# BlueFisher/Advanced-Soft-Actor-Critic

Hardware: AMD Instinct MI355X
Metric: SAC train steps/sec (PER sample + grad step), batch 256 (higher is better)
Workload: dtype f32; 1 GPU; cfg2: TEST vector obs(6) c_action(2) stock MLP, PER capacity 524288, n_step=4 V-trace; per_gpu_batch=256, global_batch=256, rows_resident=262144, replay_capacity=524288, n_step=4, burn_in_step=0, parallelism=single, ranks=1, hipgraph=True

## Files before the change

### advanced-soft-actor-critic_amd/algorithm/fused_mlp.py

```python
import contextlib
import os
import weakref

import torch
from torch import nn

from asac_amd import native

from .nn_models.layers.linear_layers import LinearLayers, ResBlock

__all__ = ['StockMLP', 'describe_q', 'describe_policy', 'describe_dense', 'fused_dense', 'gauss_head']

MAX_WIDTH, MAX_HEAD = 64, 16
MAX_INPUT = 128
FUSED_DENSE = True

_direct_depth = 0
_direct_only = []


@contextlib.contextmanager
def direct_param_grads(only=None):
    global _direct_depth
    if _direct_depth == 0:
# ... 340 lines not shown
        self._anchor = torch.zeros(1, device=device, requires_grad=True)
        self.accumulate = True
        self._workspace = None
        self._start, self._deferred_rows = start, None
        self.device = device

    @staticmethod
    def _rows(x, width):
        assert x.shape[-1] == width
        if x.dim() == 2 and x.stride(-1) == 1:
            return x
        return x.reshape(-1, width) if x.is_contiguous() else x.contiguous().view(-1, width)

    @staticmethod
    def _rows_in_place(x, width):
        assert x.shape[-1] == width
        if x.dim() == 3 and not x.is_contiguous() and x.stride(2) == 1 and x.stride(0) != x.stride(1) * x.shape[1]:
            return native.WindowRows(x)
        return StockMLP._rows(x, width)

    def _launch_forward(self, x0, x1, out=None):
        if isinstance(x0, native.WindowRows):
            job, out = self.job(x0, x1, out)
            native.mlp_forward_multi([job])
            return out
        N = x0.shape[-2]
        if out is None:
            out = torch.empty((self.E, N, self.out_cols), dtype=torch.float32, device=self.device)
        assert out.shape == (self.E, N, self.out_cols) and out.is_contiguous()
        native.mlp_forward(self.desc, self.params, self.member_stride, self.E, x0, x1, N, out)
        return out

    def _workspace_for(self, N):
        need = native.mlp_backward_workspace(self.member_stride, self.E, N)
        if self._workspace is None or self._workspace.numel() < need:
            self._workspace = torch.zeros(need, dtype=torch.float32, device=self.device)
        return self._workspace

    def _reduce_mode(self, defer):
        if defer:
            return native.MLP_REDUCE_DEFER
        return native.MLP_REDUCE_ACCUMULATE if self.accumulate else native.MLP_REDUCE_OVERWRITE

    def backward_qloss(self, x0, x1, target_q, y, weights, clip_eps, loss_out, defer=False, state_grads=False):
        N = x0.shape[-2]
        g0 = torch.empty((self.E, N, self.in0), dtype=torch.float32, device=self.device) if state_grads else None
        native.mlp_backward_qloss(self.desc, self.params, self.member_stride, self.E, x0, x1, N, target_q, y, weights,
                                  clip_eps, loss_out, self.grad_params, self._workspace_for(N), self._reduce_mode(defer),
                                  grad_x0=g0)
        self._deferred_rows = N if defer else None
        return g0

    def backward_qloss_return_ok(self, N: int, ret) -> bool:
        return native.mlp_backward_qloss_return_ok(self.desc, self.params, self.member_stride, self.E, N, ret)

    def backward_qloss_return(self, x0, x1, target_q, ret, weights, clip_eps, loss_out, defer=False, state_grads=False):
        N = x0.shape[-2]
        g0 = torch.empty((self.E, N, self.in0), dtype=torch.float32, device=self.device) if state_grads else None
        native.mlp_backward_qloss_return(self.desc, self.params, self.member_stride, self.E, x0, x1, N, target_q, ret,
                                         weights, clip_eps, loss_out, self.grad_params, self._workspace_for(N),
                                         self._reduce_mode(defer), grad_x0=g0)
        self._deferred_rows = N if defer else None
        return g0

    def backward_policy_q(self, x0, x1, q_table, subset, E_sample):
        N = x0.shape[-2]
        g1 = torch.empty((self.E, N, self.in1), dtype=torch.float32, device=self.device)
        native.mlp_backward_policy_q(self.desc, self.params, self.member_stride, self.E, x0, x1, N, q_table, subset,
                                     E_sample, g1)
        return g1

    def backward_policy_sample(self, x0, eps, grad_a, log_alpha, defer=False):
        N = x0.shape[-2]
        native.mlp_backward_policy_sample(self.desc, self.params, self.member_stride, x0, N, eps, grad_a, log_alpha,
                                          self.grad_params, self._workspace_for(N), self._reduce_mode(defer))
        self._deferred_rows = N if defer else None

    def policy_step_fused_ok(self, critics: 'StockMLP', N: int) -> bool:
        return (self.E == 1 and critics.E >= 2 and self.grad_params is not None and
                native.policy_step_fused_ok(critics.desc, critics.params, critics.member_stride, self.desc, self.params,
                                            self.member_stride, N))

    def policy_step_fused(self, critics: 'StockMLP', x0, action, eps, log_alpha, q_out=None, defer=False, subset=None,
                          sample_out=None):
        N = x0.shape[-2]
        assert subset is not None or critics.E == 2
        a_out, logp_out, ls_out = sample_out if action is None else (None, None, None)
        native.policy_step_fused(critics.desc, critics.params, critics.member_stride, self.desc, self.params,
                                 self.member_stride, x0, N, action, eps, log_alpha, q_out, self.grad_params,
                                 self._workspace_for(N), self._reduce_mode(defer), subset=subset, a_out=a_out,
                                 logp_out=logp_out, ls_out=ls_out)
        self._deferred_rows = N if defer else None

    def adam_partials(self, opt, loss_out=None):
        N = self._deferred_rows
        assert N is not None, 'no deferred backward pending'
        tiles = native.mlp_backward_tiles(N, self.E)
        s0 = self._start
        s1 = s0 + self.E * self.member_stride
        native.adam_step_partials(self.params, self.grad_params, opt.exp_avg[s0:s1], opt.exp_avg_sq[s0:s1], opt.lr,
                                  opt.betas[0], opt.betas[1], opt.eps, opt.steps_done, self._workspace, tiles,
                                  self.E, self.member_stride, native.mlp_param_extent(self.desc),
                                  self.accumulate, loss_out, N if loss_out is not None else 0)
        self._deferred_rows = None

    def job(self, x0, x1, out=None):
        N = x0.shape[0] if isinstance(x0, native.WindowRows) else x0.shape[-2]
        if self.wide and isinstance(x0, native.WindowRows):
            x0 = x0.t.reshape(N, x0.t.shape[-1])
        if out is None:
            out = torch.empty((self.E, N, self.out_cols), dtype=torch.float32, device=self.device)
        assert out.shape == (self.E, N, self.out_cols) and out.is_contiguous()
        return native.mlp_job(self.desc, self.params, self.member_stride, self.E, x0, x1, N, out), out

    def _launch_backward(self, x0, x1, grad_out, need0, need1, param_grads, reduce_members=True, defer=False,
                         grad_target=None, later=None):
        N = x0.shape[-2]
        E = self.E
        g0 = torch.empty((E, N, self.in0), dtype=torch.float32, device=self.device) if need0 else None
        g1 = torch.empty((E, N, self.in1), dtype=torch.float32, device=self.device) if need1 else None
        gp = ws = None
        mode = self._reduce_mode(defer and param_grads)
        if param_grads:
            gp = self.grad_params
            self._deferred_rows = N if defer else None
            if grad_target is not None:
                assert not defer
                gp, mode = grad_target, native.MLP_REDUCE_OVERWRITE
            if later is None or defer:
                ws = self._workspace_for(N)
            if later is not None and not defer:
                ws = torch.empty(native.mlp_backward_workspace(self.member_stride, E, N), dtype=torch.float32,
                                 device=self.device)
                tiles, used = native.mlp_backward_tiles(N, E), native.mlp_param_extent(self.desc)
                for e in range(E):
                    later.add(ws[e * self.member_stride:], tiles, 16 if tiles >= 64 else 1, E * self.member_stride, used,
                              gp[e * self.member_stride:], accumulate=mode == native.MLP_REDUCE_ACCUMULATE)
                mode = native.MLP_REDUCE_DEFER
        native.mlp_backward(self.desc, self.params, self.member_stride, E, x0, x1, N, grad_out, g0, g1, gp, ws,
                            reduce_mode=mode)
        if reduce_members:
            if g0 is not None and x0.dim() == 2:
                g0 = g0.sum(0) if E > 1 else g0[0]
            if g1 is not None and x1.dim() == 2:
                g1 = g1.sum(0) if E > 1 else g1[0]
        return g0, g1

    def call_select(self, base, t, x1=None, param_grads=True):
        if torch.is_grad_enabled() and (param_grads or base.requires_grad or (x1 is not None and x1.requires_grad)):
            pg = param_grads and self.grad_params is not None
            return _MlpSelectFn.apply(self._anchor, base, t, x1, self, pg, *(self.param_tensors if pg else ()))
        return self._launch_forward(base[:, t], x1)

    def __call__(self, x0, x1=None, param_grads=True):
        if isinstance(x0, native.WindowRows):
            assert not (torch.is_grad_enabled() and (param_grads or x0.t.requires_grad))
            return self._launch_forward(x0, x1)
        if torch.is_grad_enabled() and (param_grads or x0.requires_grad or (x1 is not None and x1.requires_grad)):
            pg = param_grads and self.grad_params is not None
            return _MlpFn.apply(self._anchor, x0, x1, self, pg, *(self.param_tensors if pg else ()))
        return self._launch_forward(x0, x1)


class _GaussHeadFn(torch.autograd.Function):
    @staticmethod
    def forward(ctx, raw, A):
        raw = raw.contiguous()
        loc = torch.empty((*raw.shape[:-1], A), dtype=raw.dtype, device=raw.device)
        scale = torch.empty_like(loc)
        native.gauss_head_fwd(raw, A, loc, scale)
        ctx.save_for_backward(raw)
        ctx.A = A
        return loc, scale

# ... 12 lines not shown
```

### advanced-soft-actor-critic_amd/algorithm/oc/option_base.py

```python
import inspect
import logging
import os

import torch
from torch.nn import functional

from asac_amd import native

from ..fused import FlatParamGroup
from ..fused_mlp import DeferredPartialSums, direct_param_grads
from ..imitation_base import SpanAdam
from ..sac_base import SAC_Base
from ..utils.enums import SEQ_ENCODER
from ..utils.operators import get_last_false_indexes

_UNSUPPORTED = "OptionBase does not support {what}: {why}"


def _reject_unsupported(args, kwargs) -> None:
    bound = inspect.signature(SAC_Base.__init__).bind_partial(None, *args, **kwargs).arguments
    if bound.get('siamese') is not None:
        raise ValueError(_UNSUPPORTED.format(
            what='siamese', why='the siamese representation loss inside compute_rep_q_grads is not built for an option'))
    if bound.get('use_prediction'):
# ... 212 lines not shown

    def _target_terminations(self, nx_target_states, nx_target_obses_list):
        with torch.no_grad():
            beta = self.model_target_termination(nx_target_states[:, :-1], [o[:, :-1] for o in nx_target_obses_list])
        return beta.squeeze(-1)

    def compute_rep_q_grads(self, next_n_vs_over_options, n_indexes, n_last_masks, n_padding_masks, nx_obses_list,
                            nx_target_obses_list, nx_states, nx_target_states, n_actions, n_pre_actions, n_rewards,
                            n_dones, n_mu_probs, n_pre_seq_hidden_states, priority_is=None):
        self._check_batch(n_rewards.shape[0])
        E, dsum = self.ensemble_q_num, self.d_action_summed_size
        n_target_terminations = self._target_terminations(nx_target_states, nx_target_obses_list)
        obs_list = [o[:, 0] for o in nx_obses_list]
        state, action = nx_states[:, 0], n_actions[:, 0]
        d_action, c_action = action[..., :dsum], action[..., dsum:]
        B = state.shape[0]
        q_list = None
        if self.d_action_sizes:
            q_list = [q(state, c_action, obs_list) for q in self.model_q_list]
            c_q = torch.stack([q[1] for q in q_list]).squeeze(-1) if self.c_action_size else None
        else:
            c_q = self._c_q_values(False, state, c_action, obs_list)
        d_y, c_y = self._get_y(next_n_vs_over_options, n_target_terminations, n_last_masks, n_padding_masks,
                               nx_target_obses_list, nx_target_states.detach(), n_actions, n_rewards, n_dones,
                               n_mu_probs if self.use_n_step_is else None,
                               eps_buf=self._eps_y, subset_prefix='y')

        start, stop = self._params.span('rep', f'q_{E - 1}')
        self._params.grad[start:stop].zero_()
        losses = roots = None
        if self.d_action_sizes:
            qs = torch.stack([torch.sum(d_action * q[0], dim=-1, keepdim=True) / self.d_action_branch_size
                              for q in q_list])
            losses = functional.mse_loss(qs, d_y.expand_as(qs), reduction='none')
        if self.c_action_size:
            yv = c_y.reshape(1, -1)
            if self.clip_epsilon > 0:
                with torch.no_grad():
                    t_q = self._c_q_values(True, state.detach(), c_action, obs_list)
                if losses is None and B == self._grad_q.shape[1]:
                    w = priority_is.reshape(-1).contiguous() if priority_is is not None else None
                    native.q_loss_fwd_bwd(c_q.detach().contiguous(), t_q.contiguous(), c_y.reshape(-1), w,
                                          self.clip_epsilon, self._loss_q_e, self._grad_q)
                    roots = ([c_q], [self._grad_q])
                else:
                    clipped = t_q + torch.clamp(c_q - t_q, -self.clip_epsilon, self.clip_epsilon)
                    c_loss = torch.maximum((clipped - yv) ** 2, (c_q - yv) ** 2).unsqueeze(-1)
            else:
                c_loss = functional.mse_loss(c_q, yv.expand_as(c_q), reduction='none').unsqueeze(-1)
            if roots is None:
                losses = c_loss if losses is None else losses + c_loss
        if roots is None:
            if priority_is is not None:
                losses = losses * priority_is.unsqueeze(0)
            loss_q_list = losses.mean(dim=(1, 2))
            self._loss_q_e.copy_(loss_q_list.detach())
            roots = ([loss_q_list.sum()], [None])
        with direct_param_grads(), DeferredPartialSums() as sums_later:
            torch.autograd.backward(*roots, retain_graph=True)
        sums_later.flush()
        self._write_option_summary({'loss/q': self._stats['loss_q']})
        return d_y, c_y

    def train_rep_q(self):
        start, stop = self._params.span('rep', f'q_{self.ensemble_q_num - 1}')
        if self.fix_policy or self.optimizer_rep is None:
            start = self._params.span('q_0')[0]
        self.optimizer_q_list[0].step(start, stop)
        self._steps_rep_q.add_(1)

    def train_policy_alpha(self, n_padding_masks, n_obses_list, nx_states, n_actions, n_mu_probs) -> None:
        if self.fix_policy:
            return
        self._check_batch(n_actions.shape[0])
        obs_list = [o[:, 0] for o in n_obses_list]
        n_states = nx_states[:, :-1]
        state, action = n_states[:, 0], n_actions[:, 0]
        mu_d_policy_probs = n_mu_probs[:, 0, :self.d_action_summed_size]
        for name in ('policy', 'alpha', 'curiosity', 'rnd'):
            if name in self._params.segments:
                s, e = self._params.span(name)
                self._params.grad[s:e].zero_()
        self._counter_advanced = False
        self._pi_sampled = False
        self._train_policy(obs_list=obs_list, state=state, action=action, mu_d_policy_probs=mu_d_policy_probs)
        if self._auto_alpha():
            self._train_alpha(obs_list, state)
        if self.curiosity is not None:
            self._train_curiosity(n_padding_masks=n_padding_masks, nx_states=nx_states, n_actions=n_actions)
        if self.use_rnd:
            self._train_rnd(n_padding_masks=n_padding_masks, n_states=n_states, n_actions=n_actions)
        if not self._counter_advanced:
            self._steps_pi.add_(1)
        if self._summary_due():
            self._refresh_policy_stats()
            tags = {}
            if self.d_action_sizes and not self.discrete_dqn_like:
                tags['loss/d_entropy'] = self._stats['d_entropy']
                if self.use_auto_alpha:
                    tags['loss/d_alpha'] = torch.exp(self.log_d_alpha.detach())
            if self.c_action_size:
                tags['loss/c_entropy'] = self._stats['c_entropy']
                if self.use_auto_alpha:
                    tags['loss/c_alpha'] = torch.exp(self.log_c_alpha.detach())
            if self.curiosity is not None:
                tags['loss/curiosity'] = self._stats['loss_curiosity']
            self._write_option_summary(tags)

    def compute_termination_grads(self, terminal_entropy, obs_list, state, y, v_over_options, done, priority_is):
        termination = self.model_termination(state.detach(), obs_list)
        B = termination.shape[0]
        dbeta = torch.empty(B, dtype=torch.float32, device=self.device)
        with torch.no_grad():
            native.termination_loss_grad(termination.detach(), y.detach(), v_over_options, done.contiguous(),
                                         priority_is, terminal_entropy, self._loss_termination, dbeta,
                                         workspace=self._termination_ws)
        self.optimizer_termination.zero_grad()
        with direct_param_grads(), DeferredPartialSums() as sums_later:
            torch.autograd.backward([termination], [dbeta.view_as(termination)])
        sums_later.flush()
        if self._summary_due():
            self._stats['termination'].copy_(torch.mean(termination.detach()))
            self._write_option_summary({'loss/termination': self._stats['loss_termination'],
                                        'metric/termination': self._stats['termination']})

    def train_termination(self):
        self.optimizer_termination.step()

    @torch.no_grad()
    def _get_td_error(self, next_n_vs_over_options, n_last_masks, n_padding_masks, nx_obses_list, nx_target_obses_list,
                      state, nx_target_states, n_actions, n_rewards, n_dones, n_mu_probs):
        self._check_batch(n_rewards.shape[0])
        dsum = self.d_action_summed_size
        n_target_terminations = self._target_terminations(nx_target_states, nx_target_obses_list)
        obs_list = [o[:, 0] for o in nx_obses_list]
        action = n_actions[:, 0]
        d_action, c_action = action[..., :dsum], action[..., dsum:]
        B = state.shape[0]
        q_list = None
        if self.d_action_sizes:
            q_list = [q(state, c_action, obs_list) for q in self.model_q_list]
            c_q = torch.stack([q[1] for q in q_list]).squeeze(-1).contiguous() if self.c_action_size else None
        else:
            c_q = self._c_q_values(False, state, c_action, obs_list).contiguous()
        fused_td = bool(self.c_action_size) and not self.d_action_sizes
        td = torch.empty(B, dtype=torch.float32, device=self.device)
        d_y, c_y = self._get_y(next_n_vs_over_options, n_target_terminations, n_last_masks, n_padding_masks,
                               nx_obses_list, nx_target_states, n_actions, n_rewards, n_dones,
                               n_mu_probs if self.use_n_step_is else None,
                               eps_buf=self._eps_td, subset_prefix='td',
                               q_online=c_q if fused_td else None, td_out=td)
        if fused_td:
            return td.unsqueeze(-1)
        err = torch.zeros((self.ensemble_q_num, B, 1), device=self.device)
        if self.d_action_sizes:
            d_q = torch.stack([torch.sum(d_action * q[0], dim=-1, keepdim=True) / self.d_action_branch_size
                               for q in q_list])
            err = err + torch.abs(d_q - d_y)
        if self.c_action_size:
            err = err + torch.abs(c_q.unsqueeze(-1) - c_y)
        return err.mean(dim=0)

    def _check_batch(self, rows: int) -> None:
        if rows != self.batch_size:
            raise ValueError(f'OptionBase was built with batch_size={self.batch_size} and takes batches of that size, '
                             f'got {rows} rows')

# ... 12 lines not shown
```

### advanced-soft-actor-critic_amd/algorithm/sac_base.py

```python
import contextlib
import logging
import random
from collections import defaultdict, namedtuple
from pathlib import Path

import numpy as np
import torch
from torch import distributions, nn
from torch.nn import functional

from asac_amd import native

from . import fused_gru, fused_linear
from .fused import DeviceNoise, FlatAdam, FlatParamGroup, squash_sample, squash_sample_ls, time_slice
from .fused_mlp import DeferredPartialSums, StockMLP, describe_policy, describe_q, direct_param_grads
from .nn_models import *
from .nn_models.layers.seq_layers import step_mask_cache
from .nn_models.representation import ModelSimpleRep
from .batch_buffer import BatchBuffer
from .captured_step import CapturedStep
from .replay_buffer import PrioritizedReplayBuffer
from .sac_aux import AuxHeadsMixin
from .utils import *
from .utils.enums import CURIOSITY, SEQ_ENCODER, SIAMESE
# ... 347 lines not shown
        tnamed += [(f'q_{i}', list(q.parameters())) for i, q in enumerate(self.model_target_q_list)]
        self._target_params = FlatParamGroup(tnamed, dev, with_grad=False)
        self._polyak_len = self._params.span('rep', f'q_{self.ensemble_q_num - 1}')[1]
        assert self._polyak_len == self._target_params.numel
        if self._dist is not None:
            self._dist.broadcast_(self._params.flat)

        self._opt_steps = torch.zeros(1, dtype=torch.int64, device=dev)
        self._exp_avg = torch.zeros_like(self._params.flat)
        self._exp_avg_sq = torch.zeros_like(self._params.flat)

        def adam(names):
            if all(len(self._params.params[n]) == 0 for n in names):
                return None
            return FlatAdam(self._params, names, learning_rate, self._opt_steps, self._exp_avg, self._exp_avg_sq)

        self.optimizer_rep = adam(['rep'])
        self.optimizer_q_list = [adam([f'q_{i}']) for i in range(self.ensemble_q_num)]
        self.optimizer_policy = adam(['policy'])
        if self.use_auto_alpha:
            self.optimizer_alpha = adam(['alpha'])
        if cur is not None:
            self.optimizer_curiosity = adam(['curiosity'])
        if self.siamese is not None:
            self.optimizer_siamese = adam(['siamese'])
        if self.use_prediction:
            self.optimizer_prediction = adam(['prediction'])
        if self.use_rnd:
            self.optimizer_rnd = adam(['rnd'])

        self._fq = self._ftq = self._fpi = None
        if self._use_fused_mlp and self.c_action_size and not self.d_action_sizes:
            dq = [describe_q(q) for q in self.model_q_list + self.model_target_q_list]
            seg = self._params.segments
            stride = seg['q_0'][1] - seg['q_0'][0]
            consecutive = all(seg[f'q_{i}'][0] == seg['q_0'][0] + i * stride for i in range(self.ensemble_q_num))
            if all(d is not None for d in dq) and consecutive:
                tseg = self._target_params.segments
                self._fq = StockMLP(dq[0], self._params.flat, self._params.grad, seg['q_0'][0], stride,
                                    self.ensemble_q_num, dev, [p for q in self.model_q_list for p in q.parameters()])
                self._ftq = StockMLP(dq[0], self._target_params.flat, None, tseg['q_0'][0], stride,
                                     self.ensemble_q_num, dev)
            dp = describe_policy(self.model_policy)
            if dp is not None:
                self._fpi = StockMLP(dp, self._params.flat, self._params.grad, seg['policy'][0],
                                     seg['policy'][1] - seg['policy'][0], 1, dev, list(self.model_policy.parameters()))
        self._wide_critics = self._fq is not None and self._fq.wide
        if self._wide_critics:
            self._la_gather_sidecar = False
        self._logger.info(f'fused stock MLP path: Q={self._fq is not None} policy={self._fpi is not None}')
        stock_only = {f'q_{i}' for i in range(self.ensemble_q_num)} | {'policy', 'alpha'}
        self._grads_overwrite = (self._fq is not None and self._fpi is not None and not self.offline_enabled
                                 and all(stop == start or name in stock_only
                                         for name, (start, stop) in self._params.segments.items()))
        if self._grads_overwrite:
            self._fq.accumulate = self._fpi.accumulate = False

        n, A, E, Es = self.n_step, self.c_action_size, self.ensemble_q_num, self.ensemble_q_sample
        f32 = dict(dtype=torch.float32, device=dev)
        A1 = max(A, 1)
        sizes = [B * (n + 1) * A1, B * A1, B * A1, B * (n + 1) * A1]
        self._eps_all = torch.zeros(sum(sizes), **f32)
        o = np.cumsum([0] + sizes)
        self._eps_y = self._eps_all[o[0]:o[1]].view(B, n + 1, A1)
        self._eps_pi = self._eps_all[o[1]:o[2]].view(B, A1)
        self._eps_alpha = self._eps_all[o[2]:o[3]].view(B, A1)
        self._eps_td = self._eps_all[o[3]:o[4]].view(B, n + 1, A1)
        names = ('y_dn', 'y_dnext', 'y_cn', 'y_cnext', 'pi_d', 'pi_c', 'td_dn', 'td_dnext', 'td_cn', 'td_cnext')
        self._subsets_all = torch.arange(Es, dtype=torch.int32, device=dev).repeat(len(names), 1).contiguous()
        self._subsets = {k: self._subsets_all[i] for i, k in enumerate(names)}
        self._y_buf = torch.zeros(B, **f32)
        self._y_td_buf = torch.zeros(B, **f32)
        self._td_error = torch.zeros(B, **f32)
        self._stats = {k: torch.zeros((), **f32) for k in ('d_entropy', 'c_entropy', 'loss_curiosity', 'loss_policy')}
        self._loss_q_e = torch.zeros(E, **f32)
        self._stats['loss_q'] = self._loss_q_e[0]
        self._grad_q = torch.zeros(E, B, **f32)
        self._mse_big_ws = torch.zeros(native.mse_mean_grad_workspace(), **f32) if self.use_prediction else None
        self._grad_logp = torch.zeros(B, **f32)
        self._ls_y = None
        self._cq_buf, self._tq_buf, self._cq_td_buf = (torch.zeros(E, B, 1, **f32) for _ in range(3))
        self._pi_q, self._pi_stats_src = torch.zeros(E, B, 1, **f32), None
        self._pi_a, self._pi_logp, self._pi_sampled = torch.zeros(B, A1, **f32), torch.zeros(B, **f32), False
        self._rep_twin = None
        if self._twin_rep and type(self.model_rep) is not ModelSimpleRep:
            from .fused_gru import TwinPass
            self._rep_twin = TwinPass(self.model_rep, self.model_target_rep)

    def _build_ckpt(self) -> None:
        ck = self.ckpt_dict = {'global_step': self.global_step}
        if self.optimizer_rep is not None:
            ck['model_rep'], ck['model_target_rep'], ck['optimizer_rep'] = \
                self.model_rep, self.model_target_rep, self.optimizer_rep
        for i in range(self.ensemble_q_num):
            ck[f'model_q_{i}'] = self.model_q_list[i]
            ck[f'model_target_q_{i}'] = self.model_target_q_list[i]
            ck[f'optimizer_q_{i}'] = self.optimizer_q_list[i]
        ck['model_policy'], ck['optimizer_policy'] = self.model_policy, self.optimizer_policy
        ck['log_d_alpha'], ck['log_c_alpha'] = self.log_d_alpha, self.log_c_alpha
        if self.use_auto_alpha:
            ck['optimizer_alpha'] = self.optimizer_alpha
        if self.curiosity == CURIOSITY.FORWARD:
            ck['model_forward_dynamic'] = self.model_forward_dynamic
        elif self.curiosity == CURIOSITY.INVERSE:
            ck['model_inverse_dynamic'] = self.model_inverse_dynamic
        if self.curiosity is not None:
            ck['optimizer_curiosity'] = self.optimizer_curiosity
        self._aux_ckpt(ck)
        total = sum(p.numel() for m in ck.values() if isinstance(m, nn.Module) for p in m.parameters())
        self._logger.info(f'Parameters: {total}')

    def _init_or_restore(self, last_ckpt: int | None) -> None:
        self.ckpt_dir = None
        if not self.model_abs_dir:
            self._update_target_variables()
            return
        self.ckpt_dir = ckpt_dir = Path(self.model_abs_dir).joinpath('model')
        ckpts = sorted(int(p.stem) for p in ckpt_dir.glob('*.pth')) if ckpt_dir.exists() else []
        ckpt_dir.mkdir(parents=True, exist_ok=True)
        if not ckpts:
            self._logger.info('Initializing from scratch')
            self._update_target_variables()
            return
        if last_ckpt is None or last_ckpt not in ckpts:
            if last_ckpt is not None:
                self._logger.warning(f'{last_ckpt} NOT IN {ckpts}, using {ckpts[-1]}')
            last_ckpt = ckpts[-1]
        path = ckpt_dir.joinpath(f'{last_ckpt}.pth')
        restored = torch.load(path, map_location=self.device, weights_only=True)
        failed = False
        for name, obj in self.ckpt_dict.items():
            if name not in restored:
                self._logger.warning(f'{name} not in {last_ckpt}.pth')
                continue
            if isinstance(obj, torch.Tensor):
                if name == 'global_step':
                    self.global_step.copy_(restored[name].to('cpu'))
                else:
                    with torch.no_grad():
                        obj.copy_(restored[name])
                continue
            try:
                if failed and name.startswith('optimizer'):
                    continue
                obj.load_state_dict(restored[name])
            except RuntimeError as e:
                failed = True
                self._logger.error(e)
            if isinstance(obj, nn.Module):
                obj.train(self.train_mode)
        self._params.rebind()
        self._target_params.rebind()
        self._logger.info(f'Restored from {path}')
        if self.train_mode and self.use_replay_buffer:
            self.replay_buffer.load(ckpt_dir, last_ckpt)
            self._logger.info('Replay buffer restored')

    def _init_replay_buffer(self, replay_config: dict | None = None) -> None:
        if not self.train_mode:
            return
        if not self.use_replay_buffer:
            self.batch_buffer = BatchBuffer(burn_in_step=self.burn_in_step,
                                            n_step=self.n_step,
                                            padding_action=self._padding_action,
                                            batch_size=self.batch_size,
                                            device=self.device,
# ... 265 lines not shown
        return bnx_indexes, bnx_padding_masks, gen_n_pre_actions(bn_actions, keep_last_action=True)

    def get_l_states(self, l_indexes, l_padding_masks, l_obses_list, l_pre_actions, l_pre_seq_hidden_states,
                     is_target=False):
        rep = self.model_target_rep if is_target else self.model_rep
        if self.seq_encoder == SEQ_ENCODER.ATTN:
            st, attn, _ = rep(l_indexes.shape[1], l_indexes, l_obses_list, l_pre_actions,
                              l_pre_seq_hidden_states[:, :1], is_prev_hidden_state=True,
                              padding_mask=l_padding_masks)
            return _real(st), _real(attn)
        out = rep(l_obses_list, l_pre_actions, l_pre_seq_hidden_states, padding_mask=l_padding_masks)
        return tuple(_real(o) for o in out) if isinstance(out, tuple) else _real(out)

    def _c_q_values(self, target: bool, state, c_action, obs_list, param_grads=True, select=None):
        fused = self._ftq if target else self._fq
        if fused is not None:
            lead = state.shape[:-1]
            a_rows = StockMLP._rows(c_action, self.c_action_size)
            if select is not None and not target and select[0].dim() == 3 and select[0].is_contiguous():
                out = fused.call_select(select[0], select[1], a_rows, param_grads=param_grads)
            else:
                rows = StockMLP._rows if torch.is_grad_enabled() else StockMLP._rows_in_place
                out = fused(rows(state, self.state_size), a_rows, param_grads=param_grads and not target)
            return out.view(self.ensemble_q_num, *lead)
        models = self.model_target_q_list if target else self.model_q_list
        return torch.stack([q(state, c_action, obs_list)[1] for q in models]).squeeze(-1)

    def _policy(self, state, obs_list):
        if self._fpi is not None:
            lead, A = state.shape[:-1], self.c_action_size
            rows = StockMLP._rows if torch.is_grad_enabled() else StockMLP._rows_in_place
            self._ls = self._fpi(rows(state, self.state_size))[0].view(*lead, 2 * A)
            return None, None, self._ls[..., :A], self._ls[..., A:], True
        self._ls = None
        d_policy, c_policy = self.model_policy(state, obs_list)
        if c_policy is None:
            return d_policy, None, None, None, False
        plain = type(c_policy) is distributions.Normal
        return d_policy, c_policy, c_policy.loc, c_policy.scale, plain

    @staticmethod
    def _rsample(c_policy, eps):
        if hasattr(c_policy, 'padding_mask'):
            keep = ~c_policy.padding_mask
            return c_policy.loc * keep + eps * (c_policy.scale * keep)
        return c_policy.loc + eps * c_policy.scale

    @torch.no_grad()
    def get_l_probs(self, l_obses_list, l_states, l_actions):
        d_policy, c_policy, loc, scale, plain = self._policy(l_states, l_obses_list)
        A_all = self.d_action_summed_size + self.c_action_size
        probs = torch.empty((*l_states.shape[:2], A_all), dtype=torch.float32, device=self.device)
        if self.d_action_sizes:
            probs[..., :self.d_action_summed_size] = d_policy.probs
        if self.c_action_size:
            if plain and l_actions.stride(-1) == 1:
                native.squash_prob(loc, scale, l_actions, self.d_action_summed_size, probs,
                                   self.d_action_summed_size)
            else:
                c_act = l_actions[..., self.d_action_summed_size:]
                probs[..., self.d_action_summed_size:] = squash_correction_prob(
                    c_policy, torch.atanh(torch.clamp(c_act, -0.999, 0.999)))
        return probs

    def _return_sample_epilogue(self, jobs, k, ls, nx_actions, eps_buf, policy_sample):
        A = self.c_action_size
        if not (native.SAMPLE_EPILOGUE and A and 2 * A <= 16 and ls.dim() == 3 and nx_actions.stride(-1) == 1):
            return None
        f32 = dict(dtype=torch.float32, device=self.device)
        a_tanh, logp = torch.empty((*ls.shape[:2], A), **f32), torch.empty(ls.shape[:2], **f32)
        c_pi = torch.empty((*ls.shape[:2], A), **f32) if self.use_n_step_is else None
        epis = [native.sample_epilogue() for _ in jobs]
        epis[k] = native.sample_epilogue(jobs[k], eps_buf, a_tanh, logp, ls.shape[1],
                                         action=nx_actions if self.use_n_step_is else None,
                                         action_offset=self.d_action_summed_size, prob_out=c_pi,
                                         eps2=self._eps_pi if policy_sample else None, t2=0,
                                         a2_out=self._pi_a if policy_sample else None,
                                         logp2_out=self._pi_logp if policy_sample else None)
        if not native.mlp_forward_multi_sampled_ok(jobs, epis):
            return None
        self.noise.normal_(eps_buf)
        if policy_sample:
            self.noise.normal_(self._eps_pi)
            self._pi_sampled = True
        native.mlp_forward_multi_sampled(jobs, epis)
        return (a_tanh, logp), c_pi

    def _vtrace_args(self, n_rewards, n_dones, n_last, n_pad, y_out):
        a = native.VtraceArgs()
        a.reward, a.reward_stride = n_rewards.data_ptr(), n_rewards.stride(0)
        a.done, a.last_mask, a.padding_mask = n_dones.data_ptr(), n_last.data_ptr(), n_pad.data_ptr()
        assert n_dones.stride(0) == n_last.stride(0) == n_pad.stride(0)
        a.mask_stride = n_dones.stride(0)
        a.gamma_ratio, a.lambda_ratio = self._gamma_ratio.data_ptr(), self._lambda_ratio.data_ptr()
        a.gamma, a.v_rho, a.v_c = self.gamma, self._v_rho_f, self._v_c_f
        a.use_n_step_is, a.B, a.n = int(self.use_n_step_is), n_rewards.shape[0], self.n_step
        a.y_out = y_out.data_ptr()
        return a

    def _window_sample(self, loc, scale, plain, c_policy, eps_buf, nx_actions, t0_ls=None):
        dsum, A = self.d_action_summed_size, self.c_action_size
        self.noise.normal_(eps_buf)
        if not plain:
            sampled = self._rsample(c_policy, eps_buf)
            c_pi = None
            if self.use_n_step_is:
                c_pi = squash_correction_prob(
                    c_policy, torch.atanh(torch.clamp(nx_actions[..., dsum:], -0.999, 0.999))).contiguous()
            return torch.tanh(sampled), sum_log_prob(squash_correction_log_prob(c_policy, sampled)), c_pi
        f32 = dict(dtype=torch.float32, device=self.device)
        a_tanh, logp = torch.empty(loc.shape, **f32), torch.empty(loc.shape[:-1], **f32)
        c_pi = torch.empty(loc.shape, **f32) if self.use_n_step_is else None
        stored = dict(action=nx_actions, action_offset=dsum, prob_out=c_pi) if self.use_n_step_is else {}
        if t0_ls is not None:
            self.noise.normal_(self._eps_pi)
            native.squash_multi([
                native.squash_job(loc, scale, eps_buf, a_tanh, logp, **stored),
                native.squash_job(t0_ls[:, 0, :A], t0_ls[:, 0, A:], self._eps_pi, self._pi_a, self._pi_logp)])
            self._pi_sampled = True
        else:
            native.squash_sample_fwd(loc, scale, eps_buf, a_tanh, logp, **stored)
        return a_tanh, logp, c_pi

    def _stored_action_ratios(self, d_policy, n_mu_probs, nx_actions):
        dsum = self.d_action_summed_size
        mu = n_mu_probs[..., :dsum] * nx_actions[:, :-1, :dsum]
        mu = torch.where(mu == 0., torch.ones_like(mu), mu).prod(-1).contiguous()
        pi = torch.exp(d_policy.log_prob(nx_actions[..., :dsum]).sum(-1))[:, :-1].contiguous()
        return pi, mu

    def _c_return(self, q_tab, logp, c_pi, n_mu_probs, sub_n, sub_next, n_rewards, n_dones, n_last, n_pad, y_out,
                  q_online=None, td_out=None):
        E, Es = self.ensemble_q_num, self.ensemble_q_sample
        args = self._vtrace_args(n_rewards, n_dones, n_last, n_pad, y_out)
        args.q = q_tab.data_ptr()
        args.q_stride_e, args.q_stride_b, args.q_stride_t = q_tab.stride(0), q_tab.stride(1), q_tab.stride(2)
        args.subset_n, args.subset_next, args.E_sample = (sub_n.data_ptr(), sub_next.data_ptr(), Es) if Es != E else (None, None, Es)
        logp = logp.contiguous()
        args.logp, args.log_alpha = logp.data_ptr(), self.log_c_alpha.data_ptr()
        if self.use_n_step_is:
            args.pi_prob, args.pi_stride_b, args.pi_stride_t = c_pi.data_ptr(), c_pi.stride(0), c_pi.stride(1)
            args.mu_prob, args.mu_stride_b, args.mu_stride_t = \
                n_mu_probs.data_ptr(), n_mu_probs.stride(0), n_mu_probs.stride(1)
            args.mu_offset, args.A = self.d_action_summed_size, self.c_action_size
        if q_online is not None and not self.d_action_sizes:
            q_online = q_online.contiguous()
            args.q_online, args.E_online, args.td_error_out = q_online.data_ptr(), q_online.shape[0], td_out.data_ptr()
        return _Return(args, (q_tab, logp, c_pi, n_mu_probs, sub_n, sub_next, q_online))

    @staticmethod
    def _launch_return(ret, *, sidecars=None, pending_alpha=None, td_update=None) -> bool:
        if td_update is not None and ret.args.td_error_out:
            rb, ids = td_update
            rb.td_update(ret.args, ids, sidecars=sidecars, alpha_step=pending_alpha)
            return True
        native.vtrace_return_min(ret.args, sidecars=sidecars, pending_alpha=pending_alpha)
        return False

    @torch.no_grad()
    def _get_y(self, n_last_masks, n_padding_masks, nx_obses_list, nx_states, nx_actions, n_rewards,
               n_dones, n_mu_probs, *, eps_buf, subset_prefix, y_out, q_online=None, td_out=None, ls=None,
               sample=None, stored_pi=None, policy_sample=False, q_table=None, launch=True):
        n_actions = nx_actions[:, :-1]
        if ls is None and sample is None and self._fpi is not None and self.c_action_size and nx_states.dim() == 3:
            job_pi, ls_out = self._fpi.job(StockMLP._rows_in_place(nx_states, self.state_size), None)
            ls_try = ls_out[0].view(*nx_states.shape[:2], 2 * self.c_action_size)
            pre = self._return_sample_epilogue([job_pi], 0, ls_try, nx_actions, eps_buf, policy_sample)
            if pre is not None:
                ls, (sample, stored_pi) = ls_try, pre
        if ls is not None:
            d_policy = c_policy = None
            loc, scale, plain = ls[..., :self.c_action_size], ls[..., self.c_action_size:], True
        else:
            d_policy, c_policy, loc, scale, plain = self._policy(nx_states, nx_obses_list)
            ls = self._ls
        self._ls_y = ls

        if self.curiosity is not None:
            n_states, next_n_states = nx_states[:, :-1], nx_states[:, 1:]
            if self.curiosity == CURIOSITY.FORWARD:
                approx, actual = self.model_forward_dynamic(n_states, n_actions), next_n_states
            else:
                approx, actual = self.model_inverse_dynamic(n_states, next_n_states), n_actions
            if (self._fused_curiosity and approx.is_cuda and approx.dim() == 3 and approx.dtype == torch.float32
                    and actual.stride(-1) == 1 and n_rewards.dim() == 2 and n_rewards.dtype == torch.float32
                    and (n_rewards.stride(1) == 1 or n_rewards.shape[1] == 1) and not torch.is_grad_enabled()):
                native.curiosity_bonus(approx.contiguous(), actual, n_rewards, self.curiosity_strength)
            else:
                d = approx - actual
                bonus = torch.sum(d.mul_(d), dim=-1).mul_(0.5)
                n_rewards.add_(bonus, alpha=self.curiosity_strength)

        logp = c_pi = None
        if self.c_action_size and sample is not None:
            (a_tanh, logp), c_pi = sample, stored_pi
        elif self.c_action_size:
            a_tanh, logp, c_pi = self._window_sample(
                loc, scale, plain, c_policy, eps_buf, nx_actions,
                t0_ls=ls if plain and policy_sample and ls is not None and ls.dim() == 3 else None)
        else:
            a_tanh = torch.zeros(0, device=self.device)

# ... 13 lines not shown
            self.noise.subset_(sub_eval, E)
            d_y = self.get_dqn_like_d_y(n_last_masks, n_padding_masks, n_rewards, n_dones,
                                        eval_next.index_select(0, sub_eval.long()), target_next)
        elif self.d_action_sizes:
            sub_next, sub_n = self._subsets[subset_prefix + '_dnext'], self._subsets[subset_prefix + '_dn']
            self.noise.subset_(sub_next, E)
            self.noise.subset_(sub_n, E)
            stacked = torch.stack([q[0] for q in nx_qs])
            mean_next = stacked[:, :, 1:].index_select(0, sub_next.long()).mean(0)
            mean_n = stacked[:, :, :-1].index_select(0, sub_n.long()).mean(0)
            probs = d_policy.probs
            n_p, next_p = probs[:, :-1], probs[:, 1:]
            d_alpha = torch.exp(self.log_d_alpha)
            v_n = torch.sum(n_p * (mean_n - d_alpha * torch.log(n_p.clamp(min=1e-8))), -1) / self.d_action_branch_size
            v_next = torch.sum(next_p * (mean_next - d_alpha * torch.log(next_p.clamp(min=1e-8))), -1) \
                / self.d_action_branch_size
            pi, mu = self._stored_action_ratios(d_policy, n_mu_probs, nx_actions) if self.use_n_step_is else (None, None)
            d_y = torch.empty(n_rewards.shape[0], dtype=torch.float32, device=self.device)
            args = self._vtrace_args(n_rewards, n_dones, n_last_masks, n_padding_masks, d_y)
            native.vtrace_return_direct(args, v_n.contiguous(), v_next.contiguous(), pi, mu)
            d_y = d_y.unsqueeze(-1)

        if self.c_action_size:
            sub_n, sub_next = self._subsets[subset_prefix + '_cn'], self._subsets[subset_prefix + '_cnext']
            self.noise.subset_(sub_n, E)
            self.noise.subset_(sub_next, E)
            if q_table is not None:
                q_tab = q_table
            elif nx_qs is not None:
                q_tab = torch.stack([q[1] for q in nx_qs]).squeeze(-1)
            else:
                q_tab = self._c_q_values(True, nx_states, a_tanh, nx_obses_list)
            ret = self._c_return(q_tab, logp, c_pi, n_mu_probs, sub_n, sub_next, n_rewards, n_dones, n_last_masks,
                                 n_padding_masks, y_out, q_online, td_out)
            if launch:
                self._launch_return(ret)
            c_y = y_out.unsqueeze(-1)
        return (d_y, c_y) if launch else (d_y, c_y, ret)

    def _stock_q_targets(self, job_tq, job_pi, ls, window, policy_sample):
        nx_states, nx_actions = window[3], window[4]
        ls = ls[0].view(*nx_states.shape[:2], 2 * self.c_action_size)
        pre = self._return_sample_epilogue([job_tq, job_pi], 1, ls, nx_actions, self._eps_y, policy_sample)
        if pre is None:
            native.mlp_forward_multi([job_tq, job_pi])
        sample, stored_pi = pre or (None, None)
        _, c_y, ret = self._get_y(*window, eps_buf=self._eps_y, subset_prefix='y', y_out=self._y_buf, ls=ls,
                                  sample=sample, stored_pi=stored_pi, policy_sample=policy_sample and pre is None,
                                  launch=False)
        return c_y, ret

    def _stock_q_backward(self, x0, a0, ret, c_y, priority_is, fold, fused_return, state_grads=False):
        w = priority_is.reshape(-1).contiguous() if priority_is is not None else None
        t_q = self._tq_buf.view(self.ensemble_q_num, -1)
        if fused_return and self._fq.backward_qloss_return_ok(x0.shape[-2], ret.args):
            g0 = self._fq.backward_qloss_return(x0, a0, t_q, ret.args, w, self.clip_epsilon, self._loss_q_e,
                                                defer=fold, state_grads=state_grads)
        else:
            self._launch_return(ret)
            g0 = self._fq.backward_qloss(x0, a0, t_q, c_y.reshape(-1), w, self.clip_epsilon, self._loss_q_e,
                                         defer=fold, state_grads=state_grads)
        if fold:
            self._fq.adam_partials(self.optimizer_q_list[0], loss_out=self._loss_q_e)
        return g0

    @torch.no_grad()
    def _train_rep_q_stock(self, n_last_masks, n_padding_masks, nx_obses_list, nx_states, nx_actions, n_rewards,
                           n_dones, n_mu_probs, priority_is, policy_sample):
        E, B = self.ensemble_q_num, nx_states.shape[0]
        x0 = StockMLP._rows(nx_states[:, 0], self.state_size)
        a0 = StockMLP._rows(nx_actions[:, 0], self.c_action_size)
        xs = StockMLP._rows(nx_states, self.state_size)
        job_tq, _ = self._ftq.job(x0, a0, out=self._tq_buf)
        job_pi, ls = self._fpi.job(xs, None)
        T, A = nx_states.shape[1], self.c_action_size
        window = (n_last_masks, n_padding_masks, nx_obses_list, nx_states, nx_actions, n_rewards, n_dones,
                  n_mu_probs if self.use_n_step_is else None)
        fused = None
        if self._fused_forward_chain and self.curiosity is None:
            f32 = dict(dtype=torch.float32, device=self.device)
            a_y, logp_y = torch.empty((B, T, A), **f32), torch.empty((B, T), **f32)
            c_pi = torch.empty((B, T, A), **f32) if self.use_n_step_is else None
            job_q, q_tab = self._ftq.job(xs, a_y.view(-1, A))
            fused = native.pi_q_job(job_pi, job_q, self._eps_y, a_y, logp_y, T,
                                    action=nx_actions if self.use_n_step_is else None,
                                    action_offset=self.d_action_summed_size, prob_out=c_pi,
                                    eps2=self._eps_pi if policy_sample else None, t2=0,
                                    a2_out=self._pi_a, logp2_out=self._pi_logp)
            if not native.policy_sample_q_forward_ok(fused):
                fused = None
        if fused is not None:
            self.noise.normal_(self._eps_y)
            if policy_sample:
                self.noise.normal_(self._eps_pi)
                self._pi_sampled = True
            native.policy_sample_q_forward(fused, [job_tq], sidecars=self._take_la_gather())
            _, c_y, ret = self._get_y(*window, eps_buf=self._eps_y, subset_prefix='y', y_out=self._y_buf,
                                      ls=ls[0].view(B, T, 2 * A), sample=(a_y, logp_y), stored_pi=c_pi,
                                      q_table=q_tab.view(E, B, T), launch=False)
        else:
            c_y, ret = self._stock_q_targets(job_tq, job_pi, ls, window, policy_sample)
        opt = self.optimizer_q_list[0]
        fold = self._dist is None and opt.start == self._fq._start and self._params.span('rep')[0] == self._params.span('rep')[1]
        self._stock_q_backward(x0, a0, ret, c_y, priority_is, fold, fused_return=fused is not None and self._fused_q_return)
        if not fold:
            self._finish_rep_q(None, None)

    def _train_rep_q(self, n_last_masks, n_padding_masks, nx_obses_list, nx_states, nx_actions, n_rewards,
                     n_dones, n_mu_probs, priority_is, aux=None, policy_sample=False, state_base=None):
        if (self._stock_c_only() and aux is None and self.clip_epsilon > 0 and not nx_states.requires_grad
                and self.optimizer_rep is None):
            return self._train_rep_q_stock(n_last_masks, n_padding_masks, nx_obses_list, nx_states, nx_actions,
                                           n_rewards, n_dones, n_mu_probs, priority_is, policy_sample)
        dsum = self.d_action_summed_size
        obs_list = [o[:, 0] for o in nx_obses_list]
        state, action = nx_states[:, 0], nx_actions[:, 0]
        if state_base is not None and not nx_states.requires_grad:
            state = state_base[0][:, state_base[1]]
        d_action, c_action = action[..., :dsum], action[..., dsum:]

        if (self._fused_q_state_grads and self._fq is not None and self._ftq is not None and not self.d_action_sizes
                and self.c_action_size and self.clip_epsilon > 0 and aux is None and state_base is not None
                and state_base[0].dim() == 3 and state.requires_grad):
            base, t = state_base
            with torch.no_grad():
                x0 = StockMLP._rows(base.detach()[:, t], self.state_size)
                a0 = StockMLP._rows(c_action, self.c_action_size)
                states_y = nx_states.detach()
                job_tq, _ = self._ftq.job(x0, a0, out=self._tq_buf)
                job_pi, ls_y = self._fpi.job(StockMLP._rows_in_place(states_y, self.state_size), None)
                c_y, ret = self._stock_q_targets(
                    job_tq, job_pi, ls_y, (n_last_masks, n_padding_masks, nx_obses_list, states_y, nx_actions, n_rewards,
                                           n_dones, n_mu_probs if self.use_n_step_is else None), policy_sample)
                fold = self._dist is None and self._fold_rep_q_adam and self._rep_q_adam_alike()
                g0 = self._stock_q_backward(x0, a0, ret, c_y, priority_is, fold, fused_return=self._fused_q_return,
                                            state_grads=True)
                g_base = self._g_state_base
                if g_base is None or g_base.shape != base.shape:
                    g_base = self._g_state_base = torch.zeros_like(base)
                at_position = self._gru_backward_at and fused_gru.is_fused_top(base)
                from_head = not at_position and self._head_sums_members and fused_linear.is_fused_head_output(base)
                if not (at_position or from_head):
                    torch.sum(g0, dim=0, out=g_base[:, t])
            rep_stepped = False
            with direct_param_grads(), DeferredPartialSums() as sums_later:
                if at_position:
                    rep_stepped = fused_gru.backward_from_position(base, g0, t, g_base,
                                                                   adam=self._rep_adam_epilogue() if fold else None)
                elif from_head:
                    fused_linear.backward_from_members(base, g0, t, g_base)
                else:
                    torch.autograd.backward([base], [g_base])
            sums_later.flush()
            if fold:
                if not rep_stepped:
                    self.optimizer_q_list[0].step(*self._params.span('rep'))
                return
            return self._finish_rep_q(None, None)
        q_list = None
        if self.d_action_sizes:
            q_list = [q(state, c_action, obs_list) for q in self.model_q_list]
            c_q = torch.stack([q[1] for q in q_list]).squeeze(-1) if self.c_action_size else None
        else:
            c_q = self._c_q_values(False, state, c_action, obs_list, select=state_base)
        d_y, c_y = self._get_y(n_last_masks, n_padding_masks, nx_obses_list, nx_states.detach(), nx_actions,
                               n_rewards, n_dones, n_mu_probs if self.use_n_step_is else None,
                               eps_buf=self._eps_y, subset_prefix='y', y_out=self._y_buf,
                               policy_sample=policy_sample)

        losses = None
        if self.d_action_sizes:
            qs = torch.stack([torch.sum(d_action * q[0], dim=-1, keepdim=True) / self.d_action_branch_size
                              for q in q_list])
            losses = functional.mse_loss(qs, d_y.expand_as(qs), reduction='none')
        if self.c_action_size:
            if self.clip_epsilon > 0:
                with torch.no_grad():
                    t_q = self._c_q_values(True, state.detach(), c_action, obs_list)
# ... 4 lines not shown
                    with direct_param_grads(), DeferredPartialSums() as sums_later:
                        torch.autograd.backward([c_q], [self._grad_q],
                                                retain_graph=aux is not None and self.use_prediction)
                    sums_later.flush()
                    if aux is None:
                        return self._finish_rep_q(None, None)
                    return self._finish_rep_q(None, None, aux,
                                              dict(n_padding_masks=n_padding_masks, nx_obses_list=nx_obses_list,
                                                   nx_states=nx_states, nx_actions=nx_actions, n_rewards=n_rewards))
                clipped = t_q + torch.clamp(c_q - t_q, -self.clip_epsilon, self.clip_epsilon)
                yv = c_y.reshape(1, -1)
                c_loss = torch.maximum((clipped - yv) ** 2, (c_q - yv) ** 2).unsqueeze(-1)
            else:
                c_loss = functional.mse_loss(c_q, c_y.reshape(1, -1).expand_as(c_q), reduction='none').unsqueeze(-1)
                losses = losses * 2 if losses is not None else None
            losses = c_loss if losses is None else losses + c_loss
        if priority_is is not None:
            losses = losses * priority_is.unsqueeze(0)
        loss_q_list = losses.mean(dim=(1, 2))
        return self._finish_rep_q(loss_q_list.sum(), loss_q_list[0], aux,
                                  dict(n_padding_masks=n_padding_masks, nx_obses_list=nx_obses_list,
                                       nx_states=nx_states, nx_actions=nx_actions, n_rewards=n_rewards))

    def _rep_q_adam_alike(self) -> bool:
        a, b = self.optimizer_rep, self.optimizer_q_list[0]
        return a is None or (a.lr, tuple(a.betas), a.eps) == (b.lr, tuple(b.betas), b.eps)

    def _rep_adam_epilogue(self):
        hp = (self.optimizer_rep.lr, *self.optimizer_rep.betas, self.optimizer_rep.eps) if self.optimizer_rep is not None else None
        if self._rep_epilogue is False or self._rep_epilogue_hp != hp:
            self._rep_epilogue, self._rep_epilogue_hp = None, hp
            from .nn_models.layers.seq_layers import GRU
            grus = [m for m in self.model_rep.modules() if isinstance(m, GRU)]
            opt, (s, e) = self.optimizer_q_list[0], self._params.span('rep')
            if (len(grus) == 1 and grus[0]._fusable and self.optimizer_rep is not None and e > s
                    and {id(p) for p in grus[0].parameters()} == {id(p) for p in self.model_rep.parameters()}):
                g = self._params
                self._rep_epilogue = native.adam_epilogue(g.flat[s:e], g.grad[s:e], opt.exp_avg[s:e], opt.exp_avg_sq[s:e],
                                                          self.optimizer_rep.lr, *self.optimizer_rep.betas,
                                                          self.optimizer_rep.eps, opt.steps_done)
        return self._rep_epilogue

    def _finish_rep_q(self, total_loss, loss_q0, aux=None, ctx=None):
        if total_loss is not None:
            with direct_param_grads(), DeferredPartialSums() as sums_later:
                total_loss.backward(retain_graph=aux is not None and self.use_prediction)
            sums_later.flush()
            self._stats['loss_q'].copy_(loss_q0.detach())
        start, stop = self._params.span('rep', f'q_{self.ensemble_q_num - 1}')
        if aux is None:
            if self._dist is not None:
                self._dist.all_reduce_grads(self._params.grad, start, stop)
            self.optimizer_q_list[0].step(start, stop)
            return
        grads_rep_main = [p.grad.detach() for p in self.model_rep.parameters()]
        grads_q_main = [[p.grad.detach() for p in q.parameters()] for q in self.model_q_list]
        if self.siamese is not None:
            n_obs = [o[:, :-1] for o in ctx['nx_obses_list']]
            self._train_siamese_representation_learning(grads_rep_main, grads_q_main, aux['n_indexes'],
                                                        ctx['n_padding_masks'], n_obs, aux['n_pre_actions'],
                                                        aux['n_pre_seq_hidden_states'])
        q_start = self._params.span('q_0')[0]
        if self._dist is not None:
            self._dist.all_reduce_grads(self._params.grad, q_start, stop)
        self.optimizer_q_list[0].step(q_start, stop)
        if self.use_prediction:
            self._train_rpm(grads_rep_main, ctx['nx_obses_list'], ctx['nx_states'], aux['nx_target_states'],
                            ctx['nx_actions'][:, :-1], ctx['n_rewards'])
        if self.optimizer_rep is not None:
            if self._dist is not None:
                self._dist.all_reduce_grads(self._params.grad, *self._params.span('rep'))
            self.optimizer_rep.step()

    def _stock_c_only(self) -> bool:
        return (self._fpi is not None and self._fq is not None and bool(self.c_action_size)
                and not self.d_action_sizes and not (self.offline_enabled and self.offline_loss))

    @torch.no_grad()
    def _train_policy_stock(self, state, ls=None):
        A, E = self.c_action_size, self.ensemble_q_num
        x = StockMLP._rows(state, self.state_size)
        B = x.shape[0]
        fusable = (self._fused_policy_step and self.ensemble_q_sample == 2 and self._fpi.policy_step_fused_ok(self._fq, B))
        sample_out = None
        if ls is None and not self._pi_sampled and fusable:
            f32 = dict(dtype=torch.float32, device=self.device)
            self.noise.normal_(self._eps_pi)
            sample_out = (torch.empty((B, A), **f32), torch.empty(B, **f32), torch.empty((B, 2 * A), **f32))
            a_tanh, logp, scale = sample_out[0], sample_out[1], sample_out[2][:, A:]
        else:
            if ls is None:
                ls = self._fpi._launch_forward(x, None)[0]
            loc, scale = ls[..., :A], ls[..., A:]
            if self._pi_sampled:
                a_tanh, logp, self._pi_sampled = self._pi_a, self._pi_logp, False
            else:
                self.noise.normal_(self._eps_pi)
                a_tanh = torch.empty((B, A), dtype=torch.float32, device=self.device)
                logp = torch.empty(B, dtype=torch.float32, device=self.device)
                native.squash_sample_fwd(loc, scale, self._eps_pi, a_tanh, logp)
        sub = self._subsets['pi_c']
        self.noise.subset_(sub, E)
        self._pi_stats_src = (logp, scale)
        opt = self.optimizer_policy
        fold = self._dist is None and (opt.start, opt.stop) == (self._fpi._start, self._fpi._start + self._fpi.member_stride)
        if fusable and a_tanh.is_contiguous():
            self._fpi.policy_step_fused(self._fq, x, None if sample_out is not None else a_tanh, self._eps_pi,
                                        self.log_c_alpha, q_out=self._pi_q, defer=fold, subset=sub if E != 2 else None,
                                        sample_out=sample_out)
        else:
            c_qs = self._fq._launch_forward(x, a_tanh, out=self._pi_q)
            g_a = self._fq.backward_policy_q(x, a_tanh, c_qs.view(E, B), sub if self.ensemble_q_sample != E else None,
                                             self.ensemble_q_sample)
            self._fpi.backward_policy_sample(x, self._eps_pi, g_a, self.log_c_alpha, defer=fold)
        if fold:
            self._fpi.adam_partials(opt)
            return
        if self._dist is not None:
            self._dist.all_reduce_grads(self._params.grad, *self._params.span('policy'))
        opt.step()

    def _train_policy(self, obs_list, state, action, mu_d_policy_probs, ls=None):
        if self._stock_c_only():
            return self._train_policy_stock(state, ls)
        dsum, E = self.d_action_summed_size, self.ensemble_q_num
        d_policy, c_policy, loc, scale, plain = self._policy(state, obs_list)
        loss_d = loss_c = None
        with torch.no_grad():
            d_alpha = torch.exp(self.log_d_alpha) if self.d_action_sizes else None
            c_alpha = torch.exp(self.log_c_alpha) if self.c_action_size else None

        if self.d_action_sizes and self.discrete_dqn_like and not self.c_action_size:
            with torch.no_grad():
                self._stats['d_entropy'].copy_(torch.mean(d_policy.entropy().sum(-1) / self.d_action_branch_size))
            return
        if self.d_action_sizes and not self.discrete_dqn_like:
            probs = d_policy.probs
            c_action = action[..., dsum:]
            d_qs = torch.stack([q(state, c_action, obs_list)[0] for q in self.model_q_list])
            sub = self._subsets['pi_d']
            self.noise.subset_(sub, E)
            mean_q = d_qs.index_select(0, sub.long()).mean(0)
            inner = d_alpha * torch.log(probs.clamp(min=1e-8)) - mean_q.detach()
            loss_d = torch.sum(probs * inner, dim=1, keepdim=True) / self.d_action_branch_size
            mu_ent = -torch.sum(mu_d_policy_probs * torch.log(mu_d_policy_probs.clamp(min=1e-8)), dim=-1) \
                / self.d_action_branch_size
            pi_ent = d_policy.entropy().sum(-1) / self.d_action_branch_size
            loss_d = loss_d + self.d_policy_entropy_penalty * (torch.pow(mu_ent - pi_ent, 2.) / 2.).unsqueeze(-1)

        pi_inputs = list(self.model_policy.parameters()) + ([self._fpi._anchor] if self._fpi is not None else [])
        if self.c_action_size and not self.d_action_sizes and plain and not (self.offline_enabled and self.offline_loss):
            self.noise.normal_(self._eps_pi)
            if self._ls is not None:
                a_tanh, logp = squash_sample_ls(self._ls, self._eps_pi)
            else:
                a_tanh, logp = squash_sample(loc, scale, self._eps_pi)
            c_qs = self._c_q_values(False, state, a_tanh, obs_list, param_grads=False)
            sub = self._subsets['pi_c']
            self.noise.subset_(sub, E)
            native.policy_loss_fwd_bwd(logp.detach(), c_qs.detach().contiguous(),
                                       sub if self.ensemble_q_sample != E else None, self.ensemble_q_sample,
                                       self.log_c_alpha, scale.detach(), self._stats['loss_policy'],
                                       self._grad_logp, self._grad_q, self._stats['c_entropy'])
            with direct_param_grads(only=pi_inputs):
                torch.autograd.backward([logp, c_qs], [self._grad_logp, self._grad_q], inputs=pi_inputs)
            if self._dist is not None:
                self._dist.all_reduce_grads(self._params.grad, *self._params.span('policy'))
            self.optimizer_policy.step()
            return

        if self.c_action_size:
            self.noise.normal_(self._eps_pi)
            if plain:
                a_tanh, logp = squash_sample(loc, scale, self._eps_pi)
                logp = logp.unsqueeze(-1)
            else:
                sampled = self._rsample(c_policy, self._eps_pi)
                a_tanh = torch.tanh(sampled)
                logp = sum_log_prob(squash_correction_log_prob(c_policy, sampled), keepdim=True)
            if self.d_action_sizes:
                c_qs = torch.stack([q(state, a_tanh, obs_list)[1] for q in self.model_q_list])
            else:
                c_qs = self._c_q_values(False, state, a_tanh, obs_list, param_grads=False).unsqueeze(-1)
            sub = self._subsets['pi_c']
            self.noise.subset_(sub, E)
            if self.ensemble_q_sample != E:
                c_qs = c_qs.index_select(0, sub.long())
            loss_c = c_alpha * logp - c_qs.min(dim=0)[0]
            if self.offline_enabled and self.offline_loss:
                loss_c = loss_c + functional.mse_loss(torch.atanh(a_tanh.clamp(-0.999999, 0.999999)), action[..., dsum:],
                                                      reduction='none').sum(-1, keepdim=True)

# ... 697 lines not shown
```

### advanced-soft-actor-critic_amd/csrc/mlp.hip

```cpp
#include "asac_common.h"
#include "asac_gelu.h"
#include "asac_sidecar.h"
#include "asac_squash.h"
#include "asac_vtrace.h"

#include <cmath>

namespace asac {

constexpr int kP = 66;
constexpr int kMaxW = 64;
constexpr int kMaxB = ASAC_MLP_MAX_BLOCKS;
constexpr int kHeadPad = 16;
#ifndef ASAC_PS_WAVES
#define ASAC_PS_WAVES 16
#endif
#ifndef ASAC_PIQ_WAVES
#define ASAC_PIQ_WAVES 8
#endif
constexpr int kPiQThreads = 64 * ASAC_PIQ_WAVES;
template <int TM> constexpr int threads_of() { return TM * 16; }

inline int mlp_tile_rows(int64_t N, int E) { return ((N + 15) / 16) * (int64_t)(E > 0 ? E : 1) <= 256 ? 16 : 32; }

using f32x4 = __attribute__((ext_vector_type(4))) float;

#ifdef ASAC_MLP_STAMPS
__device__ unsigned long long g_mlp_stamps[32];
#define MLP_STAMP(i)                                                                             \
    do {                                                                                         \
        if (blockIdx.x == 0 && blockIdx.y == 0 && threadIdx.x == 0) g_mlp_stamps[i] = wall_clock64(); \
    } while (0)
#else
#define MLP_STAMP(i)
#endif

__device__ __forceinline__ int round4(int v) { return (v + 3) & ~3; }

template <int THREADS>
__device__ __forceinline__ void stage_matrix(float* dst, const float* __restrict__ src, int rows, int cols) {
    if (rows == kMaxW && cols == kMaxW && (reinterpret_cast<uintptr_t>(src) & 15) == 0) {
        constexpr int U = 1024 / THREADS;
        const float4* s4 = reinterpret_cast<const float4*>(src);
        float4 v[U];
#pragma unroll
        for (int u = 0; u < U; ++u) v[u] = s4[threadIdx.x + u * THREADS];
#pragma unroll
        for (int u = 0; u < U; ++u) {
            const int q = threadIdx.x + u * THREADS;
            float2* d = reinterpret_cast<float2*>(dst + (q >> 4) * kP + ((q & 15) << 2));
            d[0] = make_float2(v[u].x, v[u].y);
            d[1] = make_float2(v[u].z, v[u].w);
        }
        return;
    }
    constexpr int U = 4096 / THREADS;
    float v[U];
#pragma unroll
    for (int u = 0; u < U; ++u) {
        const int i = threadIdx.x + u * THREADS;
        const int r = i >> 6, c = i & 63;
        v[u] = (r < rows && c < cols) ? src[r * cols + c] : 0.f;
    }
#pragma unroll
    for (int u = 0; u < U; ++u) {
        const int i = threadIdx.x + u * THREADS;
        dst[(i >> 6) * kP + (i & 63)] = v[u];
    }
}

template <int THREADS>
__device__ __forceinline__ void stage_matrix_part(float* dst, const float* __restrict__ src, int rows, int cols, int c0,
                                                  int ncols) {
    constexpr int U = 4096 / THREADS;
    float v[U];
#pragma unroll
    for (int u = 0; u < U; ++u) {
        const int i = threadIdx.x + u * THREADS;
        const int r = i >> 6, c = i & 63;
        v[u] = (r < rows && c < ncols) ? src[r * cols + c0 + c] : 0.f;
    }
#pragma unroll
    for (int u = 0; u < U; ++u) {
        const int i = threadIdx.x + u * THREADS;
        dst[(i >> 6) * kP + (i & 63)] = v[u];
    }
}

template <int THREADS>
__device__ __forceinline__ void stage_heads(const asac_mlp_desc_t& d, const float* __restrict__ P, int K,
                                            float* head, float* head_bias) {
    constexpr int U = 1024 / THREADS;
    float v[U];
#pragma unroll
    for (int u = 0; u < U; ++u) {
        const int i = threadIdx.x + u * THREADS;
        const int o = i >> 6, c = i & 63;
        float x = 0.f;
        if (c < K) {
            if (o < d.head_cols[0]) x = P[d.head_w_off[0] + o * K + c];
            else if (o < d.head_cols[0] + d.head_cols[1]) x = P[d.head_w_off[1] + (o - d.head_cols[0]) * K + c];
        }
        v[u] = x;
// ... 969 lines not shown
            }
            __syncthreads();
            if (l == 2) MLP_STAMP(16);
            if (part) {
                if (l == 0 && wide) {
                    grad_weight<TM>(L.delta, 0, L.x[0], W, kMaxW, part + a.d.w_off[0], K0);
                    grad_weight<TM>(L.delta, 0, x_hi, W, K0 - kMaxW, part + a.d.w_off[0] + kMaxW, K0);
                } else if constexpr (W8 != 0) {
                    grad_weight_tiles(L.delta, 0, L.x[l], W, Kin, part + a.d.w_off[l], wave - 4, W8 - 4);
                } else {
                    grad_weight<TM>(L.delta, 0, L.x[l], W, Kin, part + a.d.w_off[l]);
                }
                if (l == 2) MLP_STAMP(17);
                grad_bias<TM>(L.delta, 0, W, part + a.d.b_off[l]);
                if (l == 2) MLP_STAMP(18);
            }
            if (l == 0 && wide && (a.gx0 || a.gx1)) g_hi = gemm_tile_nt(L.delta, w_hi, round4(W), rt, ct);
            if (comp) {
                f32x4 gin = gemm_tile_nt(L.delta, L.w[l], fixed ? kMaxW : round4(W), rt, ct);
                if (a.d.residual[l]) gin += g;
                g = gin;
            }
            MLP_STAMP(5 + (kMaxB - 1 - l));
        }
    }
    if (comp && (a.gx0 || a.gx1)) {
#pragma unroll
        for (int r = 0; r < 4; ++r) {
            const int64_t row = row0 + rt * 16 + 4 * (lane >> 4) + r;
            if (row >= a.N) continue;
            if (col < a.d.in0) {
                if (a.gx0) a.gx0[((int64_t)e * a.N + row) * a.d.in0 + col] = g[r];
            } else if (col < K0) {
                if (a.gx1) a.gx1[((int64_t)e * a.N + row) * a.d.in1 + (col - a.d.in0)] = g[r];
            }
            const int ch = col + kMaxW;
            if (wide && ch < K0) {
                if (ch < a.d.in0) {
                    if (a.gx0) a.gx0[((int64_t)e * a.N + row) * a.d.in0 + ch] = g_hi[r];
                } else if (a.gx1) {
                    a.gx1[((int64_t)e * a.N + row) * a.d.in1 + (ch - a.d.in0)] = g_hi[r];
                }
            }
        }
    }
    MLP_STAMP(10);
}

constexpr int kPsWaves = ASAC_PS_WAVES;
constexpr int kPsThreads = 64 * kPsWaves;
constexpr int kPsSlots = 1024 / kPsThreads;
constexpr int kPsRows = 16;

struct PsQLds {
    float w[3][kMaxW * kP];
    float head[kHeadPad * kP];
    float bias[3][kMaxW];
    float head_bias[kHeadPad];
    float xs[2][kPsRows * kP];
};
struct PsPiLds {
    float w[3][kMaxW * kP];
    float head[kHeadPad * kP];
    float bias[3][kMaxW];
    float head_bias[kHeadPad];
    float x[4][kPsRows * kP];
    float delta[kPsRows * kP];
};
struct PsLds {
    PsQLds q[2];
    float ga[2][kPsRows * kHeadPad];
    float qv[2][kPsRows];
    float ls[kPsRows * 2 * kHeadPad];
    float act[kPsRows * kHeadPad];
};
static_assert(sizeof(PsPiLds) <= 2 * sizeof(PsQLds), "the policy phase reuses the critics' LDS");

struct PolicyStepArgs {
    MlpArgs q, pi;
    float* q_out;
    float* a_out;
    float* logp_out;
    float* ls_out;
};

__device__ __forceinline__ void ps_fetch_tile(const StageScalars& q, int64_t row0, float (&v)[kPsSlots]) {
    const int in0 = q.in0, in1 = q.in1;
    const rsrc_t r0 = make_rsrc(q.x0);
    const rsrc_t r1 = make_rsrc(q.x1, in1 > 0 ? 0x7fffffffu : 0u);
#pragma unroll
    for (int u = 0; u < kPsSlots; ++u) {
        const int i = threadIdx.x + u * kPsThreads;
        const int r = i >> 6, c = i & 63;
        const uint32_t row = (uint32_t)row0 + (uint32_t)r;
        const bool live = (int64_t)row0 + r < q.N;
        const unsigned o0 = (live && c < in0) ? (row * (uint32_t)q.x0_rs + (uint32_t)c) * 4u : kOob;
        const unsigned o1 = (live && c >= in0 && c < in0 + in1) ? (row * (uint32_t)q.x1_rs + (uint32_t)(c - in0)) * 4u : kOob;
        v[u] = __builtin_bit_cast(float, buf_ld(r0, o0) | buf_ld(r1, o1));
    }
}
__device__ __forceinline__ void ps_put_tile(const float (&v)[kPsSlots], float* xs) {
#pragma unroll
    for (int u = 0; u < kPsSlots; ++u) {
        const int i = threadIdx.x + u * kPsThreads;
        xs[(i >> 6) * kP + (i & 63)] = v[u];
    }
}

__global__ __launch_bounds__(kPsThreads) void k_policy_step(const PolicyStepArgs a_by_value) {
    extern __shared__ __attribute__((aligned(16))) unsigned char smem_raw[];
    const ASAC_KARG PolicyStepArgs& a = *static_cast<const ASAC_KARG PolicyStepArgs*>(kernarg_base());
    PsLds& L = *reinterpret_cast<PsLds*>(smem_raw);
    PsPiLds& P = *reinterpret_cast<PsPiLds*>(smem_raw);
    const int wave = threadIdx.x >> 6, lane = threadIdx.x & 63;
    const int m = wave >> 2, ct = wave & 3;
    const int col = ct * 16 + (lane & 15);
    const int64_t row0 = (int64_t)blockIdx.x * kPsRows;
    const int64_t N = a.pi.N;
    const int A = a.pi.d.head_cols[0];
    const int S = a.q.d.in0, K0q = a.q.d.in0 + a.q.d.in1, K0p = a.pi.d.in0;
    MLP_STAMP(0);

    const int e0 = a.q.subset ? a.q.subset[0] : 0, e1 = a.q.subset ? a.q.subset[1] : 1;
    const StageScalars s0 = stage_scalars<3>(a.q, e0), s1 = stage_scalars<3>(a.q, e1), sp = stage_scalars<3>(a.pi, 0);
    const bool sample_here = a.q.x1 == nullptr;
    float in_q[kPsSlots] = {}, in_pi[kPsSlots];
    if (!sample_here) ps_fetch_tile(s0, row0, in_q);
    ps_fetch_tile(sp, row0, in_pi);
    StagedNet<kPsThreads> r0, r1, rp;
    net_fetch_fixed<kPsThreads, 3>(s0, r0);
    net_fetch_fixed<kPsThreads, 3>(s1, r1);
    net_fetch_fixed<kPsThreads, 3>(sp, rp);
    float ev = 0.f, gl = 0.f;
    {
        const int lrow = threadIdx.x / (A > 0 ? A : 1), d = threadIdx.x - lrow * A;
        if ((int)threadIdx.x < kPsRows * A && row0 + lrow < N) ev = a.pi.eps[(row0 + lrow) * A + d];
        gl = expf(*a.pi.log_alpha) * (1.f / (float)N);
    }
    if (sample_here) {
        net_put_fixed<kPsThreads, 3>(rp, P);
        ps_put_tile(in_pi, P.x[0]);
        __syncthreads();
#pragma unroll
        for (int l = 0; l < 3; ++l) {
            if (wave < 4) {
                const float* xin = P.x[l & 1];
                float* xout = P.x[(l & 1) ^ 1];
                const f32x4 acc = l > 0 ? gemm_tile(xin, P.w[l], kMaxW, 0, wave) : gemm_tile(xin, P.w[l], round4(K0p), 0, wave);
                const int pc = wave * 16 + (lane & 15);
                const float bias = P.bias[l][pc];
                const bool res = a.pi.d.residual[l] != 0;
                f32x2_g ya, yb, unused;
                gelu_parts2((f32x2_g){acc[0] + bias, acc[1] + bias}, ya, unused);
                gelu_parts2((f32x2_g){acc[2] + bias, acc[3] + bias}, yb, unused);
                const float yv[4] = {ya.x, ya.y, yb.x, yb.y};
#pragma unroll
                for (int r = 0; r < 4; ++r) {
                    const int row = 4 * (lane >> 4) + r;
                    float y = yv[r];
                    if (res) y += xin[row * kP + pc];
                    xout[row * kP + pc] = y;
                }
            }
            __syncthreads();
        }
        if (wave < 4) {
            const f32x4 acc = gemm_tile(P.x[1], P.head, kMaxW, 0, 0);
            const int hc = lane & 15;
            const float mine = wave == 0 ? acc[0] : wave == 1 ? acc[1] : wave == 2 ? acc[2] : acc[3];
            const int lrow = 4 * (lane >> 4) + wave;
            const float v = head_value(a.pi.d, hc, mine + P.head_bias[hc]);
            L.ls[lrow * 2 * kHeadPad + hc] = v;
            if (a.ls_out && row0 + lrow < N && hc < 2 * A) a.ls_out[(row0 + lrow) * (2 * A) + hc] = v;
        }
        __syncthreads();
        if (threadIdx.x < kPsRows) {
            const int lrow = threadIdx.x;
            const int64_t r = row0 + lrow;
            float* arow = L.act + lrow * kHeadPad;
            if (r < N) {
                float lp;
                squash_sample_at(L.ls + lrow * 2 * kHeadPad, L.ls + lrow * 2 * kHeadPad + A, a.pi.eps + r * A, A, arow, &lp, nullptr);
                for (int d = 0; d < A; ++d) a.a_out[r * A + d] = arow[d];
                a.logp_out[r] = lp;
            } else {
                for (int d = 0; d < A; ++d) arow[d] = 0.f;
            }
        }
        __syncthreads();
        ps_put_tile(in_pi, L.q[0].xs[0]);
        ps_put_tile(in_pi, L.q[1].xs[0]);
    } else {
        ps_put_tile(in_q, L.q[0].xs[0]);
        ps_put_tile(in_q, L.q[1].xs[0]);
    }
    net_put_fixed<kPsThreads, 3>(r0, L.q[0]);
    net_put_fixed<kPsThreads, 3>(r1, L.q[1]);
    __syncthreads();
    if (sample_here) {
        if ((int)threadIdx.x < kPsRows * A) {
            const int lrow = threadIdx.x / A, d = threadIdx.x - lrow * A;
            const float v = L.act[lrow * kHeadPad + d];
            L.q[0].xs[0][lrow * kP + S + d] = v;
            L.q[1].xs[0][lrow * kP + S + d] = v;
        }
        __syncthreads();
    }
    MLP_STAMP(1);

    const bool qwave = wave < 8;
    PsQLds& Q = L.q[qwave ? m : 0];
    f32x4 z[3];
    int cur = 0;
#pragma unroll
    for (int l = 0; l < 3; ++l) {
        if (qwave) {
        const float* xin = Q.xs[cur];
        float* xout = Q.xs[cur ^ 1];
        const f32x4 acc = l > 0 ? gemm_tile(xin, Q.w[l], kMaxW, 0, ct) : gemm_tile(xin, Q.w[l], round4(K0q), 0, ct);
        const float bias = Q.bias[l][col];
        const bool res = a.q.d.residual[l] != 0;
        f32x2_g ya, yb, da, db;
        gelu_parts2((f32x2_g){acc[0] + bias, acc[1] + bias}, ya, da);
        gelu_parts2((f32x2_g){acc[2] + bias, acc[3] + bias}, yb, db);
        const float yv[4] = {ya.x, ya.y, yb.x, yb.y};
        z[l] = f32x4{da.x, da.y, db.x, db.y};
#pragma unroll
        for (int r = 0; r < 4; ++r) {
            const int row = 4 * (lane >> 4) + r;
            float y = yv[r];
            if (res) y += xin[row * kP + col];
            xout[row * kP + col] = y;
        }
        }
        __syncthreads();
        cur ^= 1;
    }
    MLP_STAMP(2);
    if (qwave && ct == 0) {
        const f32x4 raw = gemm_tile(Q.xs[cur], Q.head, kMaxW, 0, 0);
        if ((lane & 15) == 0) {
#pragma unroll
            for (int r = 0; r < 4; ++r) {
                const int lrow = 4 * (lane >> 4) + r;
                const float qv = raw[r] + Q.head_bias[0];
                L.qv[m][lrow] = qv;
                if (a.q_out && row0 + lrow < N) a.q_out[(int64_t)(m ? e1 : e0) * N + row0 + lrow] = qv;
            }
        }
    }
    __syncthreads();
    MLP_STAMP(3);
    float* qdelta = Q.xs[cur ^ 1];
    if (qwave) {
        const int t = threadIdx.x & 255;
        const int r = t >> 4, c = t & 15;
        float g = 0.f;
        if (c == 0 && row0 + r < N) {
            const int best = L.qv[1][r] < L.qv[0][r] ? 1 : 0;
            if (best == m) g = -1.f / (float)N;
        }
        qdelta[r * kP + c] = g;
    }
    __syncthreads();
    MLP_STAMP(4);
    f32x4 g = {0.f, 0.f, 0.f, 0.f};
    if (qwave) g = gemm_tile_nt(qdelta, Q.head, kHeadPad, 0, ct);
#pragma unroll
    for (int l = 2; l >= 0; --l) {
        __syncthreads();
        if (qwave) {
#pragma unroll
            for (int r = 0; r < 4; ++r) qdelta[(4 * (lane >> 4) + r) * kP + col] = g[r] * z[l][r];
        }
        __syncthreads();
        if (qwave) {
            f32x4 gin = gemm_tile_nt(qdelta, Q.w[l], kMaxW, 0, ct);
            if (a.q.d.residual[l]) gin += g;
            g = gin;
        }
    }
    if (qwave && col >= S && col < K0q) {
#pragma unroll
        for (int r = 0; r < 4; ++r) L.ga[m][(4 * (lane >> 4) + r) * kHeadPad + (col - S)] = g[r];
    }
    __syncthreads();
    MLP_STAMP(5);

    net_put_fixed<kPsThreads, 3>(rp, P);
    ps_put_tile(in_pi, P.x[0]);
    if (threadIdx.x < kPsRows * kHeadPad) P.delta[(threadIdx.x >> 4) * kP + (threadIdx.x & 15)] = 0.f;
    __syncthreads();
    MLP_STAMP(6);
    f32x4 zp[3];
#pragma unroll
    for (int l = 0; l < 3; ++l) {
        if (wave < 4) {
            const float* xin = P.x[l];
            float* xout = P.x[l + 1];
            const f32x4 acc = l > 0 ? gemm_tile(xin, P.w[l], kMaxW, 0, wave) : gemm_tile(xin, P.w[l], round4(K0p), 0, wave);
            const int pc = wave * 16 + (lane & 15);
            const float bias = P.bias[l][pc];
            const bool res = a.pi.d.residual[l] != 0;
            f32x2_g ya, yb, da, db;
            gelu_parts2((f32x2_g){acc[0] + bias, acc[1] + bias}, ya, da);
            gelu_parts2((f32x2_g){acc[2] + bias, acc[3] + bias}, yb, db);
            const float yv[4] = {ya.x, ya.y, yb.x, yb.y};
            zp[l] = f32x4{da.x, da.y, db.x, db.y};
#pragma unroll
            for (int r = 0; r < 4; ++r) {
                const int row = 4 * (lane >> 4) + r;
                float y = yv[r];
                if (res) y += xin[row * kP + pc];
                xout[row * kP + pc] = y;
            }
        }
        __syncthreads();
    }
    MLP_STAMP(7);
    if (wave == 0) {
        const f32x4 raw = gemm_tile(P.x[3], P.head, kMaxW, 0, 0);
        const int hc = lane & 15;
#pragma unroll
        for (int r = 0; r < 4; ++r) P.delta[(4 * (lane >> 4) + r) * kP + hc] = raw[r] + P.head_bias[hc];
    }
    __syncthreads();
    MLP_STAMP(8);
    if ((int)threadIdx.x < kPsRows * A) {
        const int lrow = threadIdx.x / A, d = threadIdx.x - lrow * A;
        const int64_t row = row0 + lrow;
        float g_loc = 0.f, g_scale = 0.f;
        const float raw_l = P.delta[lrow * kP + d], raw_s = P.delta[lrow * kP + A + d];
        if (row < N) {
            const float loc = head_value(a.pi.d, d, raw_l), sc = head_value(a.pi.d, A + d, raw_s);
            const float t = tanhf(loc + ev * sc);
            const float one_m = 1.f - t * t;
            float ga = 0.f;
            ga += L.ga[0][lrow * kHeadPad + d];
            ga += L.ga[1][lrow * kHeadPad + d];
            float gx = ga * one_m;
            if (one_m > 1e-2f) gx += gl * ((float)A * 2.f * t);
            g_loc = gx * head_deriv(a.pi.d, d, raw_l);
            g_scale = (gx * ev - gl / sc) * head_deriv(a.pi.d, A + d, raw_s);
        }
        P.delta[lrow * kP + d] = g_loc;
        P.delta[lrow * kP + A + d] = g_scale;
    }
    __syncthreads();
    MLP_STAMP(9);
    float* part = a.pi.partial + (int64_t)blockIdx.x * a.pi.member_stride;
    ps_grad_weight(P.delta, 0, P.x[3], A, kMaxW, part + a.pi.d.head_w_off[0]);
    ps_grad_weight(P.delta, A, P.x[3], A, kMaxW, part + a.pi.d.head_w_off[1], 4);
    if (wave == 7) {
        const int c = lane & 15, rq = (lane >> 4) * 4;
        float sb = 0.f;
#pragma unroll
        for (int r = 0; r < 4; ++r) sb += P.delta[(rq + r) * kP + c];
        sb += __shfl_xor(sb, 16, 64);
        sb += __shfl_xor(sb, 32, 64);
        if (lane < 16) {
            if (c < A) part[a.pi.d.head_b_off[0] + c] = sb;
            else if (c < 2 * A) part[a.pi.d.head_b_off[1] + c - A] = sb;
        }
    }
    f32x4 gp = {0.f, 0.f, 0.f, 0.f};
    if (wave < 4) gp = gemm_tile_nt(P.delta, P.head, kHeadPad, 0, wave);
    MLP_STAMP(10);
#pragma unroll
    for (int l = 2; l >= 0; --l) {
        const int Kin = l == 0 ? K0p : kMaxW;
        __syncthreads();
        if (wave < 4) {
            const int pc = wave * 16 + (lane & 15);
#pragma unroll
            for (int r = 0; r < 4; ++r) P.delta[(4 * (lane >> 4) + r) * kP + pc] = gp[r] * zp[l][r];
        }
        __syncthreads();
        ps_grad_weight(P.delta, 0, P.x[l], kMaxW, Kin, part + a.pi.d.w_off[l]);
        grad_bias<kPsRows>(P.delta, 0, kMaxW, part + a.pi.d.b_off[l]);
        if (l > 0 && wave < 4) {
            f32x4 gin = gemm_tile_nt(P.delta, P.w[l], kMaxW, 0, wave);
            if (a.pi.d.residual[l]) gin += gp;
            gp = gin;
        }
        MLP_STAMP(11 + (2 - l));
    }
}

struct StockJobArg {
    const float *P, *x0, *x1;
    float* out;
    int32_t member_stride, N, x0_rs, x0_ms, x1_rs, x1_ms, x0_sb, x0_T;
    int32_t in0, in1, h0, h1, hw0, hw1, hb0, hb1;
    int32_t w_off[3], b_off[3];
    int32_t residual_bits, head_transform;
};
static_assert(sizeof(StockJobArg) == 128, "StockJobArg");

template <typename JOB>
__device__ __forceinline__ MlpFwdArgs expand_stock(const JOB& j) {
    MlpFwdArgs a;
    a.d.in0 = j.in0, a.d.in1 = j.in1, a.d.n_blocks = 3;
#pragma unroll
    for (int l = 0; l < kMaxB; ++l) {
        a.d.width[l] = l < 3 ? kMaxW : 0;
        a.d.residual[l] = l < 3 ? (j.residual_bits >> l) & 1 : 0;
        a.d.w_off[l] = l < 3 ? j.w_off[l] : 0;
        a.d.b_off[l] = l < 3 ? j.b_off[l] : 0;
    }
    a.d.head_cols[0] = j.h0, a.d.head_cols[1] = j.h1;
    a.d.head_w_off[0] = j.hw0, a.d.head_w_off[1] = j.hw1;
    a.d.head_b_off[0] = j.hb0, a.d.head_b_off[1] = j.hb1;
    a.d.head_transform = j.head_transform, a.d.reserved_ = 0;
    a.params = j.P, a.member_stride = j.member_stride;
    a.x0 = j.x0, a.x0_rs = j.x0_rs, a.x0_ms = j.x0_ms;
    a.x1 = j.x1, a.x1_rs = j.x1_rs, a.x1_ms = j.x1_ms;
    a.x0_sb = j.x0_sb, a.x0_T = j.x0_T, a.pad_ = 0;
    a.N = j.N, a.out = j.out;
    return a;
}

struct PiQLds {
    float head[kHeadPad * kP];
    float bias[kMaxB][kMaxW];
    float head_bias[kHeadPad];
    float xs[2][16 * kP];
    float w[3][kMaxW * kP];
    float qw[3][kMaxW * kP];
    float qhead[kHeadPad * kP];
    float qbias[3][kMaxW];
    float qhead_bias[kHeadPad];
    float ls[16 * 2 * kHeadPad];
    float act[16 * kHeadPad];
};
static_assert(offsetof(PiQLds, w) == offsetof(MlpLds<16>, w), "PiQLds starts like MlpLds<16>");

struct PiQCritic {
    float (&w)[3][kMaxW * kP];
    float (&head)[kHeadPad * kP];
    float (&bias)[3][kMaxW];
    float (&head_bias)[kHeadPad];
};

struct StoredProbArg {
    const float* action;
    float* out;
    int32_t T, a_sb, a_st, a_off, p_sb, p_st, p_off, pad_;
};
struct PiQLaunch {
    StockJobArg pi, q;
    const float *eps, *eps2;
    float *a_out, *logp_out, *a2_out, *logp2_out;
    StoredProbArg sp;
    int32_t E, tile_groups, blocks, T, t2;
    int32_t x_n, x_blocks;
    int32_t x_E[ASAC_MLP_MAX_JOBS], x_first_block[ASAC_MLP_MAX_JOBS], x_tile_stride[ASAC_MLP_MAX_JOBS];
    StockJobArg x_job[ASAC_MLP_MAX_JOBS];
};


__device__ __forceinline__ StageScalars stage_scalars_stock(const ASAC_KARG StockJobArg& j, int e) {
    StageScalars q;
    q.P = j.P + e * j.member_stride;
    q.x0 = j.x0, q.x1 = j.in1 > 0 ? j.x1 : j.x0;
    q.N = j.N, q.x0_rs = j.x0_rs, q.x0_ms = j.x0_ms, q.x1_rs = j.x1_rs, q.x1_ms = j.x1_ms, q.x0_sb = j.x0_sb;
    q.in0 = j.in0, q.in1 = j.in1, q.x0_T = j.x0_T;
    q.h0 = j.h0, q.h1 = j.h1;
    q.hw0 = j.hw0, q.hw1 = j.hw1, q.hb0 = j.hb0, q.hb1 = j.hb1;
#pragma unroll
    for (int l = 0; l < 3; ++l) q.w_off[l] = j.w_off[l], q.b_off[l] = j.b_off[l];
    ASAC_PIN(q.P); ASAC_PIN(q.x0); ASAC_PIN(q.x1);
    ASAC_PIN(q.N); ASAC_PIN(q.x0_rs); ASAC_PIN(q.x0_ms); ASAC_PIN(q.x1_rs); ASAC_PIN(q.x1_ms); ASAC_PIN(q.x0_sb);
    ASAC_PIN(q.in0); ASAC_PIN(q.in1); ASAC_PIN(q.x0_T); ASAC_PIN(q.h0); ASAC_PIN(q.h1);
    ASAC_PIN(q.hw0); ASAC_PIN(q.hw1); ASAC_PIN(q.hb0); ASAC_PIN(q.hb1);
#pragma unroll
    for (int l = 0; l < 3; ++l) { ASAC_PIN(q.w_off[l]); ASAC_PIN(q.b_off[l]); }
    return q;
}

__device__ __forceinline__ StageScalars stage_scalars_stock_like(const ASAC_KARG StockJobArg& j, int e, const StageScalars& rows) {
    StageScalars q = rows;
    q.P = j.P + e * j.member_stride;
    q.in1 = j.in1;
    q.h0 = j.h0, q.h1 = j.h1;
    q.hw0 = j.hw0, q.hw1 = j.hw1, q.hb0 = j.hb0, q.hb1 = j.hb1;
#pragma unroll
    for (int l = 0; l < 3; ++l) q.w_off[l] = j.w_off[l], q.b_off[l] = j.b_off[l];
    ASAC_PIN(q.P); ASAC_PIN(q.in1); ASAC_PIN(q.h0); ASAC_PIN(q.h1);
    ASAC_PIN(q.hw0); ASAC_PIN(q.hw1); ASAC_PIN(q.hb0); ASAC_PIN(q.hb1);
#pragma unroll
    for (int l = 0; l < 3; ++l) { ASAC_PIN(q.w_off[l]); ASAC_PIN(q.b_off[l]); }
    return q;
}

__device__ __forceinline__ float gauss_head_value(bool location, float raw) {
    return location ? tanhf(raw / 5.f) * 5.f : expf(fminf(fmaxf(raw, -20.f), 0.5f));
}

template <bool WINDOW>
__device__ __forceinline__ void pi_q_tiles(const ASAC_KARG PiQLaunch& a, PiQLds& L) {
    constexpr int THREADS = kPiQThreads;
    constexpr int SLOTS = 1024 / kPiQThreads;
    const bool comp = (threadIdx.x >> 6) < 4;
    const int e = (int)blockIdx.x % a.E, group = (int)blockIdx.x / a.E;
    const int wave = threadIdx.x >> 6, lane = threadIdx.x & 63;
    const int col = wave * 16 + (lane & 15);
    const int A = a.pi.h0, S = a.q.in0;
    const int K0p = a.pi.in0, K0q = a.q.in0 + a.q.in1;
    const int N = a.pi.N;
    const int n_tiles = (int)((N + 15) / 16);
    const bool writer = e == 0;
    MLP_STAMP(0);

    const StageScalars sp = stage_scalars_stock(a.pi, 0);
    const StageScalars sq = stage_scalars_stock_like(a.q, e, sp);
    float in_lo[SLOTS];
    fetch_input_tile_fixed<THREADS, WINDOW, SLOTS>(sp, 0, (int64_t)group * 16, in_lo);
    StagedNet<THREADS> rp, rq;
    net_fetch_fixed<THREADS, 3>(sp, rp);
    net_fetch_fixed<THREADS, 3>(sq, rq);
    put_input_tile<THREADS, SLOTS>(in_lo, L.xs[0]);
    net_put_fixed<THREADS, 3>(rp, L);
    PiQCritic C{L.qw, L.qhead, L.qbias, L.qhead_bias};
    __syncthreads();
    MLP_STAMP(1);

    for (int tile = group; tile < n_tiles; tile += a.tile_groups) {
        const int row0 = tile * 16;
        if (tile != group) {
            fetch_input_tile_fixed<THREADS, WINDOW, SLOTS>(sp, 0, row0, in_lo);
            __syncthreads();
            put_input_tile<THREADS, SLOTS>(in_lo, L.xs[0]);
            __syncthreads();
        }
        int cur = 0;
#pragma unroll
        for (int l = 0; l < 3; ++l) {
            if (comp) {
                const float* xin = L.xs[cur];
                float* xout = L.xs[cur ^ 1];
                const f32x4 acc = l > 0 ? gemm_tile(xin, L.w[l], kMaxW, 0, wave) : gemm_tile(xin, L.w[l], round4(K0p), 0, wave);
                const float bias = L.bias[l][col];
                const bool res = (a.pi.residual_bits >> l) & 1;
                f32x2_g ya, yb, unused;
                gelu_parts2((f32x2_g){acc[0] + bias, acc[1] + bias}, ya, unused);
                gelu_parts2((f32x2_g){acc[2] + bias, acc[3] + bias}, yb, unused);
                const float yv[4] = {ya.x, ya.y, yb.x, yb.y};
#pragma unroll
                for (int r = 0; r < 4; ++r) {
                    const int row = 4 * (lane >> 4) + r;
                    float y = yv[r];
                    if (res) y += xin[row * kP + col];
                    xout[row * kP + col] = y;
                }
            }
            __syncthreads();
            cur ^= 1;
        }
        MLP_STAMP(2);
        if (comp) {
            const f32x4 acc = gemm_tile(L.xs[cur], L.head, kMaxW, 0, 0);
            const int hc = lane & 15;
            const float mine = wave == 0 ? acc[0] : wave == 1 ? acc[1] : wave == 2 ? acc[2] : acc[3];
            const int lrow = 4 * (lane >> 4) + wave;
            const float v = gauss_head_value(hc < A, mine + L.head_bias[hc]);
            L.ls[lrow * 2 * kHeadPad + hc] = v;
            if (writer && a.pi.out && row0 + lrow < N && hc < 2 * A) a.pi.out[(row0 + lrow) * (2 * A) + hc] = v;
        }
        __syncthreads();
        MLP_STAMP(3);
        {
            float* scr = L.xs[1];
            const int job = wave;
            const bool job_on = job == 0 || (writer && ((job == 1 && a.sp.action) || (job == 2 && a.eps2)));
            float* s0 = scr + job * 256;
            float* s1 = s0 + 128;
            if (job < 3 && job_on) {
                for (int it = lane; it < 16 * A; it += 64) {
                    const int lrow = it / A, d = it - lrow * A;
                    const int r = row0 + lrow;
                    if (r >= N) continue;
                    const float l = L.ls[lrow * 2 * kHeadPad + d], sc = L.ls[lrow * 2 * kHeadPad + A + d];
                    if (job == 1) {
                        const int spT = a.sp.T;
                        const int sb = (int)((unsigned)r / (unsigned)spT), st = r - sb * spT;
                        const float av = a.sp.action[sb * a.sp.a_sb + st * a.sp.a_st + a.sp.a_off + d];
                        const float x = atanhf(fminf(fmaxf(av, -0.999f), 0.999f));
                        s0[lrow * 8 + d] = squash_jac(x);
                        s1[lrow * 8 + d] = expf(normal_log_prob(x, l, sc));
                    } else {
                        float ev;
                        const int smp = (int)((unsigned)r / (unsigned)a.T);
                        if (job == 0) {
                            ev = a.eps[r * A + d];
                        } else {
                            if (r - smp * a.T != a.t2) continue;
                            ev = a.eps2[smp * A + d];
                        }
                        const float x = l + ev * sc;
                        const float t = tanhf(x);
                        s0[lrow * 8 + d] = logf(fmaxf(1.f - t * t, kSquashFloor));
                        s1[lrow * 8 + d] = normal_log_prob(x, l, sc);
                        if (job == 0) {
                            L.act[lrow * kHeadPad + d] = t;
                            if (writer) a.a_out[r * A + d] = t;
                        } else {
                            a.a2_out[smp * A + d] = t;
                        }
                    }
                }
                __builtin_amdgcn_fence(__ATOMIC_RELEASE, "wavefront");
                __builtin_amdgcn_wave_barrier();
                __builtin_amdgcn_fence(__ATOMIC_ACQUIRE, "wavefront");
                if (lane < 16) {
                    const int lrow = lane;
                    const int r = row0 + lrow;
                    if (r < N) {
                        if (job == 1) {
                            float jac = 1.f;
                            for (int d = 0; d < A; ++d) jac *= s0[lrow * 8 + d];
                            const int spT = a.sp.T;
                            const int sb = (int)((unsigned)r / (unsigned)spT), st = r - sb * spT;
                            float* out = a.sp.out + (sb * a.sp.p_sb + st * a.sp.p_st + a.sp.p_off);
                            for (int d = 0; d < A; ++d) out[d] = s1[lrow * 8 + d] / jac;
                        } else {
                            const int smp = (int)((unsigned)r / (unsigned)a.T);
                            if (job == 0 || r - smp * a.T == a.t2) {
                                float corr = 0.f;
                                for (int d = 0; d < A; ++d) corr += s0[lrow * 8 + d];
                                float lp = 0.f;
                                for (int d = 0; d < A; ++d) {
                                    float v = s1[lrow * 8 + d] - corr;
                                    if (v == INFINITY) v = 0.f;
                                    lp += v;
                                }
                                if (job == 2) a.logp2_out[smp] = lp;
                                else if (writer) a.logp_out[r] = lp;
                            }
                        }
                    }
                }
            }
            if (job == 0 && lane < 16 && row0 + lane >= N)
                for (int d = 0; d < A; ++d) L.act[lane * kHeadPad + d] = 0.f;
        }
        if (tile == group) net_put_fixed<THREADS, 3>(rq, C);
        put_input_tile<THREADS, SLOTS>(in_lo, L.xs[0]);
        __syncthreads();
// ... 469 lines not shown
        const int64_t be = desc->b_off[l] + desc->width[l];
        used = we > used ? we : used;
        used = be > used ? be : used;
    }
    for (int h = 0; h < 2; ++h) {
        if (desc->head_cols[h] <= 0) continue;
        const int64_t we = desc->head_w_off[h] + (int64_t)desc->head_cols[h] * H;
        const int64_t be = desc->head_b_off[h] + desc->head_cols[h];
        used = we > used ? we : used;
        used = be > used ? be : used;
    }
    return used;
}

int asac_mlp_backward(const asac_mlp_desc_t* desc, const float* params, int64_t member_stride, int E,
                      const float* x0, int64_t x0_row_stride, int64_t x0_member_stride,
                      const float* x1, int64_t x1_row_stride, int64_t x1_member_stride, int64_t N,
                      const float* grad_out, float* grad_x0, float* grad_x1, float* grad_params,
                      float* workspace, int reduce_mode, void* stream) {
    if (!desc || !desc_ok(*desc) || E <= 0 || N <= 0 || !x0 || (desc->in1 > 0 && !x1) || !grad_out)
        return bad_arg("asac_mlp_backward");
    if (grad_params && !workspace) return bad_arg("asac_mlp_backward: workspace");
    MlpArgs a = make_args(desc, params, member_stride, x0, x0_row_stride, x0_member_stride, x1, x1_row_stride,
                          x1_member_stride, N);
    a.gout = grad_out;
    a.gx0 = grad_x0;
    a.gx1 = grad_x1;
    return mlp_backward_common("asac_mlp_backward", desc, a, E, N, member_stride, grad_params, workspace,
                               reduce_mode, nullptr, as_stream(stream));
}

int asac_mlp_backward_policy_q(const asac_mlp_desc_t* desc, const float* params, int64_t member_stride, int E,
                               const float* x0, int64_t x0_row_stride, int64_t x0_member_stride,
                               const float* x1, int64_t x1_row_stride, int64_t x1_member_stride, int64_t N,
                               const float* q_table, const int32_t* subset, int E_sample, float* grad_x1,
                               void* stream) {
    if (!desc || !desc_ok(*desc) || E <= 0 || N <= 0 || !x0 || desc->in1 <= 0 || !x1 || !q_table || !grad_x1 ||
        E_sample < 1 || E_sample > E)
        return bad_arg("asac_mlp_backward_policy_q");
    if (desc->head_cols[0] != 1 || desc->head_cols[1] != 0 || desc->head_transform != 0)
        return bad_arg("asac_mlp_backward_policy_q: not a scalar-head network");
    MlpArgs a = make_args(desc, params, member_stride, x0, x0_row_stride, x0_member_stride, x1, x1_row_stride,
                          x1_member_stride, N);
    a.q_table = q_table;
    a.subset = subset;
    a.E_sample = E_sample;
    a.gx1 = grad_x1;
    return mlp_backward_common("asac_mlp_backward_policy_q", desc, a, E, N, member_stride, nullptr, nullptr,
                               ASAC_MLP_REDUCE_OVERWRITE, nullptr, as_stream(stream));
}

int asac_mlp_backward_policy_sample(const asac_mlp_desc_t* desc, const float* params, int64_t member_stride,
                                    const float* x0, int64_t x0_row_stride, int64_t N, const float* eps,
                                    const float* grad_a, int grad_a_members, const float* log_alpha,
                                    float* grad_params, float* workspace, int reduce_mode, void* stream) {
    if (!desc || !desc_ok(*desc) || N <= 0 || !x0 || desc->in1 != 0 || !eps || !grad_a || grad_a_members < 1 ||
        !log_alpha || !grad_params || !workspace)
        return bad_arg("asac_mlp_backward_policy_sample");
    if (desc->head_transform != 1 || desc->head_cols[0] != desc->head_cols[1] || desc->head_cols[0] > 16)
        return bad_arg("asac_mlp_backward_policy_sample: not a Gaussian-head policy");
    MlpArgs a = make_args(desc, params, member_stride, x0, x0_row_stride, 0, nullptr, 0, 0, N);
    a.eps = eps;
    a.grad_a = grad_a;
    a.grad_a_members = grad_a_members;
    a.log_alpha = log_alpha;
    return mlp_backward_common("asac_mlp_backward_policy_sample", desc, a, 1, N, member_stride, grad_params,
                               workspace, reduce_mode, nullptr, as_stream(stream));
}

int asac_policy_step_fused_ok(const asac_mlp_desc_t* q_desc, const float* q_params, int64_t q_member_stride,
                              const asac_mlp_desc_t* pi_desc, const float* pi_params, int64_t pi_member_stride, int64_t N) {
    if (!q_desc || !pi_desc || !desc_ok(*q_desc) || !desc_ok(*pi_desc) || N <= 0) return 0;
    if (!stock3(*q_desc, q_params, q_member_stride) || !stock3(*pi_desc, pi_params, pi_member_stride)) return 0;
    if (q_desc->head_cols[0] != 1 || q_desc->head_cols[1] != 0 || q_desc->head_transform != 0) return 0;
    if (pi_desc->head_transform != 1 || pi_desc->head_cols[0] != pi_desc->head_cols[1] || pi_desc->in1 != 0) return 0;
    if (q_desc->in0 != pi_desc->in0 || q_desc->in1 != pi_desc->head_cols[0] || 2 * pi_desc->head_cols[0] > kHeadPad) return 0;
    return mlp_tile_rows(N, 1) == kPsRows ? 1 : 0;
}

int asac_policy_step_fused(const asac_mlp_desc_t* q_desc, const float* q_params, int64_t q_member_stride,
                           const asac_mlp_desc_t* pi_desc, const float* pi_params, int64_t pi_member_stride,
                           const float* x, int64_t x_row_stride, int64_t N, const float* action, const float* eps,
                           const float* log_alpha, const int32_t* subset, float* q_out, float* a_tanh_out,
                           float* logp_out, float* ls_out, float* pi_grad_params, float* workspace, int reduce_mode,
                           void* stream) {
    if (!asac_policy_step_fused_ok(q_desc, q_params, q_member_stride, pi_desc, pi_params, pi_member_stride, N) ||
        !x || !eps || !log_alpha || !pi_grad_params || !workspace || (!action && (!a_tanh_out || !logp_out)))
        return bad_arg("asac_policy_step_fused");
    PolicyStepArgs a{};
    const int A = pi_desc->head_cols[0];
    a.q = make_args(q_desc, q_params, q_member_stride, x, x_row_stride, 0, action, A, 0, N);
    a.pi = make_args(pi_desc, pi_params, pi_member_stride, x, x_row_stride, 0, nullptr, 0, 0, N);
    if (!offsets32(a.q) || !offsets32(a.pi)) return bad_arg("asac_policy_step_fused: offsets");
    a.q.subset = subset;
    a.a_out = a_tanh_out;
    a.logp_out = logp_out;
    a.ls_out = ls_out;
    a.pi.eps = eps;
    a.pi.log_alpha = log_alpha;
    a.pi.partial = workspace;
    a.q_out = q_out;
    static bool attr_done = false;
    if (int rc = set_lds_limit(reinterpret_cast<const void*>(k_policy_step), sizeof(PsLds), attr_done,
                               "asac_policy_step_fused: hipFuncSetAttribute"))
        return rc;
    const int tiles = (int)((N + kPsRows - 1) / kPsRows);
    hipStream_t s = as_stream(stream);
    ASAC_LAUNCH(k_policy_step, dim3((unsigned)tiles), dim3(kPsThreads), sizeof(PsLds), s, a);
    if (reduce_mode != ASAC_MLP_REDUCE_DEFER) {
        const int64_t used = asac_mlp_param_extent(pi_desc);
        if (tiles >= kSlicedFrom)
            hipLaunchKernelGGL(k_mlp_reduce_partials_sliced, dim3((unsigned)((used + 63) / 64), 1u), dim3(64 * kReduceSlices),
                               0, s, workspace, tiles, 1, pi_member_stride, used, pi_grad_params,
                               reduce_mode == ASAC_MLP_REDUCE_ACCUMULATE ? 1 : 0, nullptr, nullptr, 0.f);
        else
            hipLaunchKernelGGL(k_mlp_reduce_partials, dim3((unsigned)((used + 255) / 256), 1u), dim3(256), 0, s, workspace,
                               tiles, 1, pi_member_stride, used, pi_grad_params,
                               reduce_mode == ASAC_MLP_REDUCE_ACCUMULATE ? 1 : 0, nullptr, nullptr, 0.f);
    }
    return finish_launch("asac_policy_step_fused");
}

static bool fits32(int64_t v) { return v >= 0 && v < 0x1fffffffLL; }

static StockJobArg stock_job_arg(const asac_mlp_desc_t* d, const float* params, int64_t member_stride, const float* x0,
                                 int64_t x0_rs, int64_t x0_ms, const float* x1, int64_t x1_rs, int64_t x1_ms, int64_t N,
                                 int64_t x0_T, int64_t x0_sb, float* out) {
    StockJobArg j{};
    j.P = params, j.x0 = x0, j.x1 = x1, j.out = out;
    j.member_stride = (int32_t)member_stride, j.N = (int32_t)N;
    j.x0_rs = (int32_t)x0_rs, j.x0_ms = (int32_t)x0_ms, j.x1_rs = (int32_t)x1_rs, j.x1_ms = (int32_t)x1_ms;
    j.x0_sb = (int32_t)x0_sb, j.x0_T = (int32_t)x0_T;
    j.in0 = d->in0, j.in1 = d->in1, j.h0 = d->head_cols[0], j.h1 = d->head_cols[1];
    j.hw0 = (int32_t)d->head_w_off[0], j.hw1 = (int32_t)d->head_w_off[1];
    j.hb0 = (int32_t)d->head_b_off[0], j.hb1 = (int32_t)d->head_b_off[1];
    for (int l = 0; l < 3; ++l) {
        j.w_off[l] = (int32_t)d->w_off[l], j.b_off[l] = (int32_t)d->b_off[l];
        j.residual_bits |= (d->residual[l] ? 1 : 0) << l;
    }
    j.head_transform = d->head_transform;
    return j;
}

static bool pi_q_job_ok(const asac_pi_q_job_t& j) {
    const asac_mlp_job_t &p = j.pi, &q = j.q;
    if (!p.desc || !q.desc || !desc_ok(*p.desc) || !desc_ok(*q.desc) || p.N <= 0 || q.N != p.N || p.E != 1 || q.E < 1) return false;
    if (!stock3(*p.desc, p.params, p.member_stride) || !stock3(*q.desc, q.params, q.member_stride)) return false;
    if (q.desc->head_cols[0] != 1 || q.desc->head_cols[1] != 0 || q.desc->head_transform != 0) return false;
    if (p.desc->head_transform != 1 || p.desc->head_cols[0] != p.desc->head_cols[1] || p.desc->in1 != 0) return false;
    const int A = p.desc->head_cols[0];
    if (q.desc->in0 != p.desc->in0 || q.desc->in1 != A || 2 * A > kHeadPad || A > 8) return false;
    if (!p.x0 || q.x0 != p.x0 || q.x0_row_stride != p.x0_row_stride || q.x0_window_T != p.x0_window_T ||
        q.x0_sample_stride != p.x0_sample_stride || p.x0_member_stride != 0 || q.x0_member_stride != 0 || !q.out)
        return false;
    const asac_squash_job_t& s = j.sample;
    if (!s.eps || !s.a_tanh_out || !s.logp_out || s.A != A || s.rows != p.N) return false;
    if (s.action && (!s.prob_out || s.T <= 0)) return false;
    if (j.eps2 && (!j.a2_out || !j.logp2_out || s.T <= 0 || j.t2 < 0 || j.t2 >= s.T)) return false;
    if (!fits32(p.member_stride) || !fits32(q.member_stride * q.E)) return false;
    if (s.action && (!fits32((p.N / s.T + 1) * s.action_stride_b) || !fits32((p.N / s.T + 1) * s.prob_stride_b) ||
                     !fits32(s.T * s.action_stride_t) || !fits32(s.T * s.prob_stride_t)))
        return false;
    return p.N * (p.x0_row_stride + 1) < 0x1fffffffLL &&
           (p.x0_window_T == 0 || (p.N / p.x0_window_T + 1) * p.x0_sample_stride < 0x1fffffffLL);
}

int asac_policy_sample_q_forward_ok(const asac_pi_q_job_t* job) { return job && pi_q_job_ok(*job) ? 1 : 0; }

int asac_policy_sample_q_forward(const asac_pi_q_job_t* job, const asac_mlp_job_t* extra_jobs, int n_extra,
                                 const asac_sidecar_t* sidecars_host, int n_sidecars, void* stream) {
    if (!job || !pi_q_job_ok(*job) || n_extra < 0 || n_extra > ASAC_MLP_MAX_JOBS || (n_extra > 0 && !extra_jobs))
        return bad_arg("asac_policy_sample_q_forward");
    SidecarsDev sc{};
    if (sidecars_prepare(sidecars_host, n_sidecars, sc)) return bad_arg("asac_policy_sample_q_forward: sidecar");
    PiQLaunch m{};
    const asac_mlp_job_t &p = job->pi, &q = job->q;
    m.pi = stock_job_arg(p.desc, p.params, p.member_stride, p.x0, p.x0_row_stride, 0, nullptr, 0, 0, p.N, p.x0_window_T,
                         p.x0_sample_stride, p.out);
    m.q = stock_job_arg(q.desc, q.params, q.member_stride, p.x0, p.x0_row_stride, 0, p.x0, 0, 0, p.N, p.x0_window_T,
                        p.x0_sample_stride, q.out);
    m.E = q.E;
    const int tiles = (int)((p.N + 15) / 16);
    const int cap = 256 / q.E > 0 ? 256 / q.E : 1;
    m.tile_groups = tiles <= cap ? tiles : cap;
    m.blocks = m.tile_groups * q.E;
    const asac_squash_job_t& sj = job->sample;
    m.eps = sj.eps;
    m.a_out = sj.a_tanh_out;
    m.logp_out = sj.logp_out;
    m.sp = StoredProbArg{sj.action, sj.prob_out, sj.T, (int32_t)sj.action_stride_b, (int32_t)sj.action_stride_t, sj.action_offset,
                         (int32_t)sj.prob_stride_b, (int32_t)sj.prob_stride_t, sj.prob_offset, 0};
    m.eps2 = job->eps2;
    m.T = sj.T > 0 ? sj.T : 1;
    m.t2 = job->t2;
    m.a2_out = job->a2_out;
    m.logp2_out = job->logp2_out;
    m.x_n = n_extra;
    int blocks = 0;
    for (int k = 0; k < n_extra; ++k) {
        const asac_mlp_job_t& j = extra_jobs[k];
        if (!j.desc || !desc_ok(*j.desc) || !stock3(*j.desc, j.params, j.member_stride) || j.E <= 0 || j.N <= 0 || !j.x0 ||
            (j.desc->in1 > 0 && !j.x1) || !j.out || j.x0_window_T < 0 ||
            j.N * (j.x0_row_stride + j.x1_row_stride + 1) >= 0x1fffffffLL ||
            (j.x0_window_T > 0 && (j.N / j.x0_window_T + 1) * j.x0_sample_stride >= 0x1fffffffLL) ||
            !fits32(j.member_stride) || !fits32(j.x0_member_stride) || !fits32(j.x1_member_stride))
            return bad_arg("asac_policy_sample_q_forward: extra job");
        m.x_job[k] = stock_job_arg(j.desc, j.params, j.member_stride, j.x0, j.x0_row_stride, j.x0_member_stride, j.x1,
                                   j.x1_row_stride, j.x1_member_stride, j.N, j.x0_window_T, j.x0_sample_stride, j.out);
        m.x_E[k] = j.E;
        m.x_first_block[k] = blocks;
        m.x_tile_stride[k] = mlp_tile_groups(j.N, j.E, 1, 16);
        blocks += m.x_tile_stride[k] * j.E;
    }
    m.x_blocks = blocks;
    static bool attr_done = false;
    static bool attr_done1 = false;
    if (int rc = set_lds_limit(reinterpret_cast<const void*>(k_pi_sample_q<ASAC_MAX_SIDECARS>), sizeof(PiQLds), attr_done,
                               "asac_policy_sample_q_forward: hipFuncSetAttribute"))
        return rc;
    if (int rc = set_lds_limit(reinterpret_cast<const void*>(k_pi_sample_q<1>), sizeof(PiQLds), attr_done1,
                               "asac_policy_sample_q_forward: hipFuncSetAttribute"))
        return rc;
    const SidecarsDev none{};
    for (int rep = 0; rep < g_launch_repeat; ++rep) {
        const bool last = rep == g_launch_repeat - 1;
        const dim3 grid((unsigned)(m.blocks + blocks + (last ? sc.blocks : 0)));
        if (sc.n <= 1)
            hipLaunchKernelGGL(k_pi_sample_q<1>, grid, dim3(kPiQThreads), sizeof(PiQLds), as_stream(stream), m,
                               sidecars_first<1>(last ? sc : none));
        else
            hipLaunchKernelGGL(k_pi_sample_q<ASAC_MAX_SIDECARS>, grid, dim3(kPiQThreads), sizeof(PiQLds), as_stream(stream), m,
                               last ? sc : none);
    }
    return finish_launch("asac_policy_sample_q_forward");
}

int asac_mlp_backward_qloss(const asac_mlp_desc_t* desc, const float* params, int64_t member_stride, int E,
                            const float* x0, int64_t x0_row_stride, int64_t x0_member_stride,
                            const float* x1, int64_t x1_row_stride, int64_t x1_member_stride, int64_t N,
                            const float* target_q, const float* y, const float* weights, float clip_eps,
                            float* loss_out, float* grad_params, float* workspace, int reduce_mode,
                            void* stream) {
    return asac_mlp_backward_qloss_gx(desc, params, member_stride, E, x0, x0_row_stride, x0_member_stride, x1, x1_row_stride,
                                      x1_member_stride, N, target_q, y, weights, clip_eps, loss_out, nullptr, grad_params,
                                      workspace, reduce_mode, stream);
}

int asac_mlp_backward_qloss_return_ok(const asac_mlp_desc_t* desc, const float* params, int64_t member_stride, int E,
                                      int64_t N, const asac_vtrace_args_t* ret) {
    if (!desc || !desc_ok(*desc) || !ret || E <= 0 || N <= 0 || ret->B != N || ret->n <= 0 || !ret->q || !ret->y_out ||
        ret->E_sample <= 0 || ret->E_sample > ASAC_MAX_ENSEMBLE || ret->td_error_out)
        return 0;
    if (desc->in0 + desc->in1 > kMaxW || !stock3(*desc, params, member_stride)) return 0;
    const int tm = mlp_tile_rows(N, E);
    const size_t lds = (tm == 16 ? sizeof(MlpBwdLds<16>) : sizeof(MlpBwdLds<32>)) +
                       (size_t)(2 * ((ret->n + 1) | 1) + 2) * tm * sizeof(float);
    const int threads = tm == 16 ? 64 * ASAC_BWD_WAVES : 32 * 16;
    return tm * ret->n <= threads && lds <= 128 * 1024;
}

int asac_mlp_backward_qloss_return(const asac_mlp_desc_t* desc, const float* params, int64_t member_stride, int E,
                                   const float* x0, int64_t x0_row_stride, int64_t x0_member_stride,
                                   const float* x1, int64_t x1_row_stride, int64_t x1_member_stride, int64_t N,
                                   const float* target_q, const asac_vtrace_args_t* ret, const float* weights,
                                   float clip_eps, float* loss_out, float* grad_x0, float* grad_params, float* workspace,
                                   int reduce_mode, void* stream) {
    if (!desc || !desc_ok(*desc) || E <= 0 || N <= 0 || !x0 || (desc->in1 > 0 && !x1) || !target_q || !ret ||
        !grad_params || !workspace || clip_eps <= 0.f)
        return bad_arg("asac_mlp_backward_qloss_return");
    if (desc->head_cols[0] != 1 || desc->head_cols[1] != 0 || desc->head_transform != 0)
        return bad_arg("asac_mlp_backward_qloss_return: not a scalar-head network");
    if (reduce_mode != ASAC_MLP_REDUCE_DEFER && !loss_out) return bad_arg("asac_mlp_backward_qloss_return: loss_out");
    if (!asac_mlp_backward_qloss_return_ok(desc, params, member_stride, E, N, ret) ||
        (ret->use_n_step_is && (!ret->mu_prob || !ret->pi_prob || ret->A <= 0)))
        return bad_arg("asac_mlp_backward_qloss_return: return arguments");
    MlpArgs a = make_args(desc, params, member_stride, x0, x0_row_stride, x0_member_stride, x1, x1_row_stride,
                          x1_member_stride, N);
    if (!offsets32(a)) return bad_arg("asac_mlp_backward_qloss_return: offsets");
    a.tq = target_q;
// ... 34 lines not shown
```

### advanced-soft-actor-critic_amd/native.py

```python
import ctypes as C
from pathlib import Path

import torch

PKG_DIR = Path(__file__).resolve().parent
import os as _os

LIB_PATH = Path(_os.environ.get('ASAC_HIP_LIB', PKG_DIR / 'lib' / 'libasac_hip.so'))
ABI_VERSION = 84

MAX_GATHER_KEYS = 16
PAD_KEEP, PAD_WORD, PAD_BYTE, PAD_ROW, PAD_EMIT_MASK = 0, 1, 2, 3, 4
CVT_NONE, CVT_U8_TO_F32_UNIT, CVT_BOOL_TO_F32 = 0, 1, 2


class AsacNativeError(RuntimeError):
    pass


class GatherKey(C.Structure):
    _fields_ = [('src', C.c_void_p), ('dst', C.c_void_p), ('pad_row', C.c_void_p),
                ('row_bytes', C.c_int32), ('pad_mode', C.c_int32), ('pad_word', C.c_uint32),
                ('convert', C.c_int32), ('dst_row_pitch', C.c_int32), ('derive', C.c_int32)]


class AdamEpilogue(C.Structure):
    _fields_ = [('param_base', C.c_void_p), ('grad_base', C.c_void_p), ('exp_avg_base', C.c_void_p),
                ('exp_avg_sq_base', C.c_void_p), ('lr', C.c_float), ('beta1', C.c_float), ('beta2', C.c_float),
                ('eps', C.c_float), ('steps_done', C.c_void_p)]


def adam_epilogue(param_flat, grad_flat, exp_avg, exp_avg_sq, lr, beta1, beta2, eps, steps_done) -> AdamEpilogue:
    for t in (param_flat, grad_flat, exp_avg, exp_avg_sq):
        assert t.is_cuda and t.is_contiguous() and t.dtype == torch.float32 and t.numel() == param_flat.numel()
    assert steps_done.dtype == torch.int64 and steps_done.is_cuda
    ep = AdamEpilogue(param_flat.data_ptr(), grad_flat.data_ptr(), exp_avg.data_ptr(), exp_avg_sq.data_ptr(),
                      float(lr), float(beta1), float(beta2), float(eps), steps_done.data_ptr())
    ep._keep = (param_flat, grad_flat, exp_avg, exp_avg_sq, steps_done)
    ep._span = (grad_flat.data_ptr(), grad_flat.data_ptr() + 4 * grad_flat.numel())
    return ep


ROW_ITEM, ROW_SLOT, ROW_SLOT_ROW, ROW_BROADCAST = 0, 1, 2, 3
DERIVE_NONE, DERIVE_PREVIOUS, DERIVE_HOLD_LAST, DERIVE_HOLD_LAST_NEXT = 0, 1, 2, 3


class RowMove(C.Structure):
    _fields_ = [('src', C.c_void_p), ('dst', C.c_void_p),
                ('src_stride0', C.c_int64), ('src_stride1', C.c_int64),
                ('dst_stride0', C.c_int64), ('dst_stride1', C.c_int64),
                ('row_bytes', C.c_int32), ('src_mode', C.c_int32), ('dst_mode', C.c_int32),
                ('src_row_offset', C.c_int32), ('pad_word', C.c_uint32), ('reserved_', C.c_int32)]


class BatchPutKey(C.Structure):
    _fields_ = [('src', C.c_void_p), ('pool', C.c_void_p), ('pad_row', C.c_void_p), ('src_stride', C.c_int64),
                ('row_bytes', C.c_int32), ('pad_mode', C.c_int32), ('pad_word', C.c_uint32), ('reserved_', C.c_int32)]


class BatchGatherKey(C.Structure):
    _fields_ = [('pool', C.c_void_p), ('dst', C.c_void_p), ('row_bytes', C.c_int32), ('convert', C.c_int32)]


class VtraceArgs(C.Structure):
    _fields_ = [
        ('q', C.c_void_p), ('q_stride_e', C.c_int64), ('q_stride_b', C.c_int64), ('q_stride_t', C.c_int64),
        ('subset_n', C.c_void_p), ('subset_next', C.c_void_p), ('E_sample', C.c_int32),
        ('logp', C.c_void_p), ('log_alpha', C.c_void_p),
        ('reward', C.c_void_p), ('reward_stride', C.c_int64),
        ('done', C.c_void_p), ('last_mask', C.c_void_p), ('padding_mask', C.c_void_p), ('mask_stride', C.c_int64),
        ('mu_prob', C.c_void_p), ('mu_stride_b', C.c_int64), ('mu_stride_t', C.c_int64), ('mu_offset', C.c_int32),
        ('pi_prob', C.c_void_p), ('pi_stride_b', C.c_int64), ('pi_stride_t', C.c_int64), ('A', C.c_int32),
        ('gamma_ratio', C.c_void_p), ('lambda_ratio', C.c_void_p),
        ('gamma', C.c_float), ('v_rho', C.c_float), ('v_c', C.c_float),
        ('use_n_step_is', C.c_int32), ('B', C.c_int32), ('n', C.c_int32),
        ('q_online', C.c_void_p), ('E_online', C.c_int32),
        ('td_error_out', C.c_void_p), ('y_out', C.c_void_p)]


class MlpDesc(C.Structure):
    _fields_ = [('in0', C.c_int32), ('in1', C.c_int32), ('n_blocks', C.c_int32),
                ('width', C.c_int32 * 4), ('residual', C.c_int32 * 4), ('head_cols', C.c_int32 * 2),
                ('w_off', C.c_int64 * 4), ('b_off', C.c_int64 * 4),
                ('head_w_off', C.c_int64 * 2), ('head_b_off', C.c_int64 * 2),
                ('head_transform', C.c_int32), ('reserved_', C.c_int32)]


class MlpJob(C.Structure):
    _fields_ = [('desc', C.POINTER(MlpDesc)), ('params', C.c_void_p), ('member_stride', C.c_int64),
                ('x0', C.c_void_p), ('x0_row_stride', C.c_int64), ('x0_member_stride', C.c_int64),
                ('x1', C.c_void_p), ('x1_row_stride', C.c_int64), ('x1_member_stride', C.c_int64),
                ('N', C.c_int64), ('out', C.c_void_p), ('E', C.c_int32), ('x0_window_T', C.c_int32),
                ('x0_sample_stride', C.c_int64)]


MLP_MAX_JOBS = 2
SAMPLE_EPILOGUE = _os.environ.get('ASAC_SAMPLE_EPILOGUE', '1') != '0'


class Sidecar(C.Structure):
    _fields_ = [('kind', C.c_int32),
                ('logp', C.c_void_p), ('B', C.c_int32), ('target', C.c_float), ('slot', C.c_int32),
                ('param', C.c_void_p), ('grad', C.c_void_p), ('exp_avg', C.c_void_p), ('exp_avg_sq', C.c_void_p),
                ('n', C.c_int32), ('lr', C.c_float), ('beta1', C.c_float), ('beta2', C.c_float), ('eps', C.c_float),
                ('steps_done', C.c_void_p), ('advance_counter', C.c_int32),
                ('ring', C.c_void_p), ('row_bytes', C.c_int32), ('capacity', C.c_int32), ('ids', C.c_void_p),
                ('batch', C.c_int32), ('first_off', C.c_int32), ('count', C.c_int32), ('slot_ids', C.c_void_p),
                ('padding_mask', C.c_void_p), ('mask_sample_stride', C.c_int32), ('rows', C.c_void_p),
                ('rows_sample_stride_bytes', C.c_int64), ('rows_row_stride_bytes', C.c_int64), ('winner', C.c_void_p),
                ('gather_plan', C.c_void_p), ('gather_blocks', C.c_int32)]


SIDECAR_ALPHA_ADAM, SIDECAR_SCATTER_ELECT, SIDECAR_SCATTER_WRITE, SIDECAR_WINDOW_GATHER, MAX_SIDECARS = 1, 2, 3, 4, 4


class SquashJob(C.Structure):
    _fields_ = [('loc', C.c_void_p), ('scale', C.c_void_p), ('ls_row_stride', C.c_int64), ('eps', C.c_void_p),
                ('rows', C.c_int64), ('A', C.c_int32), ('T', C.c_int32), ('a_tanh_out', C.c_void_p),
                ('logp_out', C.c_void_p), ('x_out', C.c_void_p), ('action', C.c_void_p),
                ('action_stride_b', C.c_int64), ('action_stride_t', C.c_int64), ('prob_out', C.c_void_p),
                ('prob_stride_b', C.c_int64), ('prob_stride_t', C.c_int64), ('action_offset', C.c_int32),
                ('prob_offset', C.c_int32)]


SQUASH_MAX_JOBS = 4


class PiQJob(C.Structure):
    _fields_ = [('pi', MlpJob), ('sample', SquashJob), ('eps2', C.c_void_p), ('t2', C.c_int32), ('reserved_', C.c_int32),
                ('a2_out', C.c_void_p), ('logp2_out', C.c_void_p), ('q', MlpJob)]


class SampleEpilogue(C.Structure):
    _fields_ = [('sample', SquashJob), ('eps2', C.c_void_p), ('t2', C.c_int32), ('reserved_', C.c_int32),
                ('a2_out', C.c_void_p), ('logp2_out', C.c_void_p)]


class PartialSum(C.Structure):
    _fields_ = [('partial', C.c_void_p), ('out', C.c_void_p), ('slab_stride', C.c_int64), ('n', C.c_int64),
                ('slabs', C.c_int32), ('slices', C.c_int32), ('accumulate', C.c_int32), ('pad_', C.c_int32)]


class GruDesc(C.Structure):
    _fields_ = [('input', C.c_int32), ('hidden', C.c_int32), ('hidden_pow2', C.c_int32), ('layers', C.c_int32)]


class Conv2Desc(C.Structure):
    _fields_ = [(n, C.c_int32) for n in ('channels', 'height', 'width', 'out1', 'kernel1', 'stride1',
                                         'out2', 'kernel2', 'stride2')]


GRU_MAX_LAYERS, GRU_MAX_DIM = 2, 16
_PtrArray = C.c_void_p * GRU_MAX_LAYERS

class ObsDecoderParams(C.Structure):
    _fields_ = [(n, C.c_void_p) for n in ('dense1_w', 'dense1_b', 'dense2_w', 'dense2_b', 'ct1_w', 'ct1_b', 'ct2_w',
                                          'ct2_b', 'ct3_w', 'ct3_b')]


_SIGNATURES = {
    'asac_version': (C.c_int, []),
    'asac_last_error': (C.c_char_p, []),
    'asac_set_launch_repeat': (C.c_int, [C.c_int]),
    'asac_sumtree_sample': (C.c_int, [C.c_void_p, C.c_int, C.c_int, C.c_void_p, C.c_void_p, C.c_void_p,
                                      C.c_double, C.c_void_p, C.c_void_p, C.c_void_p, C.c_void_p,
                                      C.c_void_p, C.c_void_p]),
    'asac_per_is_weights': (C.c_int, [C.c_void_p, C.c_int, C.c_void_p, C.c_void_p, C.c_void_p, C.c_double,
                                      C.c_void_p, C.c_void_p]),
    'asac_sumtree_update': (C.c_int, [C.c_void_p, C.c_int, C.c_int, C.c_void_p, C.c_void_p, C.c_void_p,
                                      C.c_float, C.c_float, C.c_float, C.c_int, C.c_void_p, C.c_void_p,
                                      C.c_void_p]),
    'asac_per_add': (C.c_int, [C.c_void_p, C.c_int, C.c_int64, C.c_int, C.c_int, C.c_void_p, C.c_float,
                               C.c_void_p, C.c_void_p]),
    'asac_sumtree_leaf_max': (C.c_int, [C.c_void_p, C.c_int, C.c_void_p, C.c_void_p]),
    'asac_sumtree_check': (C.c_int, [C.c_void_p, C.c_int, C.c_void_p, C.c_void_p]),
    'asac_gelu_eval': (C.c_int, [C.c_void_p, C.c_void_p, C.c_void_p, C.c_int64, C.c_void_p]),
    'asac_sumtree_plan_top': (C.c_int, [C.c_void_p, C.c_int, C.c_int, C.c_void_p, C.c_void_p, C.c_void_p, C.c_void_p, C.c_void_p]),
    'asac_sumtree_descend_owned': (C.c_int, [C.c_void_p, C.c_int, C.c_int, C.c_void_p, C.c_void_p, C.c_int, C.c_void_p,
                                             C.c_void_p, C.c_void_p, C.c_void_p, C.c_void_p]),
    'asac_per_is_weights_slice': (C.c_int, [C.c_void_p, C.c_int, C.c_int, C.c_int, C.c_void_p, C.c_void_p, C.c_double,
                                            C.c_void_p, C.c_void_p]),
    'asac_window_gather_pad': (C.c_int, [C.POINTER(GatherKey), C.c_int, C.c_void_p, C.c_int, C.c_int,
                                         C.c_int, C.c_int, C.c_void_p, C.c_void_p]),
    'asac_window_gather_plan_bytes': (C.c_int64, []),
    'asac_window_gather_plan': (C.c_int, [C.POINTER(GatherKey), C.c_int, C.c_void_p, C.c_int, C.c_int, C.c_int, C.c_int,
                                          C.c_void_p, C.c_void_p, C.POINTER(C.c_int)]),
    'asac_sumtree_descend': (C.c_int, [C.c_void_p, C.c_int, C.c_int, C.c_void_p, C.c_void_p, C.c_void_p, C.c_void_p,
                                       C.c_void_p, C.c_void_p]),
    'asac_gather_rows': (C.c_int, [C.POINTER(GatherKey), C.c_int, C.c_void_p, C.c_int, C.c_int, C.c_void_p]),
    'asac_rows_move': (C.c_int, [C.POINTER(RowMove), C.c_int, C.c_void_p, C.c_void_p, C.c_void_p, C.c_int,
                                 C.c_void_p]),
    'asac_batch_put': (C.c_int, [C.POINTER(BatchPutKey), C.c_int, C.c_int, C.c_int, C.c_int, C.c_void_p, C.c_void_p,
                                 C.c_int, C.c_int, C.c_void_p, C.c_void_p, C.c_int, C.c_int, C.c_void_p, C.c_int,
                                 C.c_void_p, C.c_int32, C.c_void_p]),
    'asac_batch_pop_gather': (C.c_int, [C.POINTER(BatchGatherKey), C.c_int, C.c_void_p, C.c_void_p, C.c_int, C.c_int,
                                        C.c_int, C.c_int, C.c_void_p]),
    'asac_window_aux': (C.c_int, [C.c_void_p, C.c_int64, C.c_void_p, C.c_int64, C.c_void_p, C.c_int64, C.c_int64,
                                  C.c_int, C.c_int, C.c_int, C.c_void_p, C.c_void_p, C.c_void_p, C.c_int64, C.c_void_p]),
    'asac_scatter_rows_if_id_match': (C.c_int, [C.c_void_p, C.c_int, C.c_int, C.c_void_p, C.c_int, C.c_int,
                                                C.c_int, C.c_void_p, C.c_void_p, C.c_int, C.c_void_p,
                                                C.c_int64, C.c_int64, C.c_void_p, C.c_void_p]),
    'asac_squash_sample_fwd': (C.c_int, [C.c_void_p, C.c_void_p, C.c_int64, C.c_void_p, C.c_int64, C.c_int,
                                         C.c_void_p, C.c_void_p, C.c_void_p,
                                         C.c_void_p, C.c_int, C.c_int64, C.c_int64, C.c_int,
                                         C.c_void_p, C.c_int64, C.c_int64, C.c_int, C.c_void_p]),
    'asac_squash_sample_bwd': (C.c_int, [C.c_void_p, C.c_void_p, C.c_int64, C.c_void_p, C.c_void_p, C.c_int,
                                         C.c_int64, C.c_void_p, C.c_void_p, C.c_int64, C.c_int, C.c_void_p,
                                         C.c_void_p, C.c_int64, C.c_void_p]),
    'asac_squash_multi': (C.c_int, [C.POINTER(SquashJob), C.c_int, C.POINTER(Sidecar), C.c_int, C.c_void_p]),
    'asac_squash_prob': (C.c_int, [C.c_void_p, C.c_void_p, C.c_int64, C.c_void_p, C.c_int, C.c_int64, C.c_int64,
                                   C.c_int, C.c_int64, C.c_int, C.c_void_p, C.c_int64, C.c_int64, C.c_int,
                                   C.c_void_p]),
    'asac_vtrace_return_min': (C.c_int, [C.POINTER(VtraceArgs), C.c_void_p]),
    'asac_vtrace_return_min_sc': (C.c_int, [C.POINTER(VtraceArgs), C.POINTER(Sidecar), C.c_int, C.POINTER(Sidecar),
                                            C.c_void_p]),
    'asac_td_update': (C.c_int, [C.POINTER(VtraceArgs), C.c_void_p, C.c_int, C.c_void_p, C.c_void_p, C.c_float, C.c_float,
                                 C.c_float, C.c_void_p, C.c_void_p, C.POINTER(Sidecar), C.c_int, C.POINTER(Sidecar),
                                 C.c_void_p]),
    'asac_sumtree_update_sc': (C.c_int, [C.c_void_p, C.c_int, C.c_int, C.c_void_p, C.c_void_p, C.c_void_p, C.c_float,
                                         C.c_float, C.c_float, C.c_int, C.c_void_p, C.c_void_p, C.POINTER(Sidecar), C.c_int,
                                         C.c_void_p]),
    'asac_vtrace_return_direct': (C.c_int, [C.POINTER(VtraceArgs), C.c_void_p, C.c_void_p, C.c_void_p,
                                            C.c_void_p, C.c_void_p]),
    'asac_q_loss_fwd_bwd': (C.c_int, [C.c_void_p, C.c_void_p, C.c_void_p, C.c_void_p, C.c_int, C.c_int,
                                      C.c_float, C.c_void_p, C.c_void_p, C.c_void_p]),
    'asac_mlp_forward': (C.c_int, [C.POINTER(MlpDesc), C.c_void_p, C.c_int64, C.c_int, C.c_void_p, C.c_int64,
                                   C.c_int64, C.c_void_p, C.c_int64, C.c_int64, C.c_int64, C.c_void_p, C.c_void_p]),
    'asac_mlp_forward_multi': (C.c_int, [C.POINTER(MlpJob), C.c_int, C.POINTER(Sidecar), C.c_int, C.c_void_p]),
    'asac_mlp_forward_multi_sampled_ok': (C.c_int, [C.POINTER(MlpJob), C.c_int, C.POINTER(SampleEpilogue)]),
    'asac_mlp_forward_multi_sampled': (C.c_int, [C.POINTER(MlpJob), C.c_int, C.POINTER(SampleEpilogue), C.POINTER(Sidecar),
                                                 C.c_int, C.c_void_p]),
    'asac_mlp_backward_workspace': (C.c_int64, [C.c_int64, C.c_int, C.c_int64]),
    'asac_mlp_backward_tiles': (C.c_int64, [C.c_int64, C.c_int]),
    'asac_mlp_backward': (C.c_int, [C.POINTER(MlpDesc), C.c_void_p, C.c_int64, C.c_int, C.c_void_p, C.c_int64,
                                    C.c_int64, C.c_void_p, C.c_int64, C.c_int64, C.c_int64, C.c_void_p, C.c_void_p,
                                    C.c_void_p, C.c_void_p, C.c_void_p, C.c_int, C.c_void_p]),
    'asac_mlp_backward_qloss': (C.c_int, [C.POINTER(MlpDesc), C.c_void_p, C.c_int64, C.c_int, C.c_void_p, C.c_int64,
                                          C.c_int64, C.c_void_p, C.c_int64, C.c_int64, C.c_int64, C.c_void_p,
                                          C.c_void_p, C.c_void_p, C.c_float, C.c_void_p, C.c_void_p, C.c_void_p,
                                          C.c_int, C.c_void_p]),
    'asac_mlp_backward_qloss_gx': (C.c_int, [C.POINTER(MlpDesc), C.c_void_p, C.c_int64, C.c_int, C.c_void_p, C.c_int64,
                                             C.c_int64, C.c_void_p, C.c_int64, C.c_int64, C.c_int64, C.c_void_p,
                                             C.c_void_p, C.c_void_p, C.c_float, C.c_void_p, C.c_void_p, C.c_void_p,
                                             C.c_void_p, C.c_int, C.c_void_p]),
    'asac_mlp_backward_qloss_return_ok': (C.c_int, [C.POINTER(MlpDesc), C.c_void_p, C.c_int64, C.c_int, C.c_int64,
                                                    C.POINTER(VtraceArgs)]),
    'asac_mlp_backward_qloss_return': (C.c_int, [C.POINTER(MlpDesc), C.c_void_p, C.c_int64, C.c_int, C.c_void_p, C.c_int64,
                                                 C.c_int64, C.c_void_p, C.c_int64, C.c_int64, C.c_int64, C.c_void_p,
                                                 C.POINTER(VtraceArgs), C.c_void_p, C.c_float, C.c_void_p, C.c_void_p,
                                                 C.c_void_p, C.c_void_p, C.c_int, C.c_void_p]),
    'asac_mlp_backward_policy_q': (C.c_int, [C.POINTER(MlpDesc), C.c_void_p, C.c_int64, C.c_int, C.c_void_p, C.c_int64,
                                             C.c_int64, C.c_void_p, C.c_int64, C.c_int64, C.c_int64, C.c_void_p,
                                             C.c_void_p, C.c_int, C.c_void_p, C.c_void_p]),
    'asac_mlp_backward_policy_sample': (C.c_int, [C.POINTER(MlpDesc), C.c_void_p, C.c_int64, C.c_void_p, C.c_int64,
                                                  C.c_int64, C.c_void_p, C.c_void_p, C.c_int, C.c_void_p,
                                                  C.c_void_p, C.c_void_p, C.c_int, C.c_void_p]),
    'asac_struct_size': (C.c_int64, [C.c_char_p]),
    'asac_policy_sample_q_forward_ok': (C.c_int, [C.POINTER(PiQJob)]),
    'asac_policy_sample_q_forward': (C.c_int, [C.POINTER(PiQJob), C.POINTER(MlpJob), C.c_int, C.POINTER(Sidecar), C.c_int,
                                               C.c_void_p]),
    'asac_policy_step_fused_ok': (C.c_int, [C.POINTER(MlpDesc), C.c_void_p, C.c_int64, C.POINTER(MlpDesc), C.c_void_p,
                                            C.c_int64, C.c_int64]),
    'asac_policy_step_fused': (C.c_int, [C.POINTER(MlpDesc), C.c_void_p, C.c_int64, C.POINTER(MlpDesc), C.c_void_p,
                                         C.c_int64, C.c_void_p, C.c_int64, C.c_int64, C.c_void_p, C.c_void_p,
                                         C.c_void_p, C.c_void_p, C.c_void_p, C.c_void_p, C.c_void_p, C.c_void_p,
                                         C.c_void_p, C.c_void_p, C.c_int, C.c_void_p]),
    'asac_mlp_param_extent': (C.c_int64, [C.POINTER(MlpDesc)]),
    'asac_adam_step_partials': (C.c_int, [C.c_void_p, C.c_void_p, C.c_void_p, C.c_void_p, C.c_float, C.c_float,
                                          C.c_float, C.c_float, C.c_void_p, C.c_void_p, C.c_int64, C.c_int,
                                          C.c_int64, C.c_int64, C.c_int, C.c_void_p, C.c_int64, C.c_void_p]),
    'asac_gauss_head_fwd': (C.c_int, [C.c_void_p, C.c_int64, C.c_int, C.c_void_p, C.c_void_p, C.c_void_p]),
    'asac_gauss_head_bwd': (C.c_int, [C.c_void_p, C.c_void_p, C.c_void_p, C.c_int64, C.c_int, C.c_void_p,
                                      C.c_void_p]),
    'asac_attention_supported': (C.c_int, [C.c_int, C.c_int, C.c_int]),
    'asac_attention_forward': (C.c_int, [C.c_void_p, C.c_void_p, C.c_void_p, C.c_void_p, C.c_int64, C.c_int64, C.c_int64,
                                         C.c_int, C.c_int, C.c_int, C.c_int, C.c_void_p, C.c_void_p, C.c_void_p,
                                         C.c_void_p]),
    'asac_attention_backward': (C.c_int, [C.c_void_p, C.c_void_p, C.c_void_p, C.c_void_p, C.c_void_p, C.c_void_p, C.c_int,
                                          C.c_int, C.c_int, C.c_int, C.c_void_p, C.c_void_p, C.c_void_p, C.c_void_p]),
    'asac_attention_proj_workspace': (C.c_int64, [C.c_int, C.c_int, C.c_int, C.c_int]),
    'asac_attention_proj_forward': (C.c_int, [C.c_void_p, C.c_int64, C.c_int64, C.c_void_p, C.c_int64, C.c_int64,
                                              C.c_void_p * 8, C.c_void_p, C.c_int64, C.c_int64, C.c_int64, C.c_int,
                                              C.c_int, C.c_int, C.c_int, C.c_void_p, C.c_void_p, C.c_void_p, C.c_void_p,
                                              C.c_void_p, C.c_int64, C.c_int64, C.c_void_p]),
    'asac_attention_proj_backward': (C.c_int, [C.c_void_p, C.c_int64, C.c_int64, C.c_void_p, C.c_int64, C.c_int64,
                                               C.c_void_p * 8, C.c_void_p, C.c_void_p, C.c_void_p, C.c_void_p, C.c_int64,
                                               C.c_int64, C.c_void_p, C.c_void_p, C.c_int64, C.c_int64,
                                               C.c_int, C.c_int, C.c_int, C.c_int, C.c_void_p, C.c_void_p, C.c_void_p,
                                               C.c_int, C.c_void_p, C.c_void_p]),
    'asac_linear_tanh_workspace': (C.c_int64, [C.c_int64, C.c_int, C.c_int]),
    'asac_linear_tanh_forward': (C.c_int, [C.c_void_p, C.c_int64, C.c_void_p, C.c_void_p, C.c_int64, C.c_int, C.c_int,
                                           C.c_void_p, C.c_void_p]),
    'asac_linear_tanh_backward': (C.c_int, [C.c_void_p, C.c_int64, C.c_void_p, C.c_void_p, C.c_void_p, C.c_int64, C.c_int,
                                            C.c_int, C.c_void_p, C.c_void_p, C.c_int, C.c_void_p, C.c_void_p]),
    'asac_linear_tanh_forward2': (C.c_int, [C.c_void_p, C.c_int64, C.c_int, C.c_void_p, C.c_int64, C.c_int, C.c_void_p,
                                            C.c_void_p, C.c_int64, C.c_int, C.c_void_p, C.c_void_p]),
    'asac_linear_tanh_forward2w': (C.c_int, [C.c_void_p, C.c_int64, C.c_int, C.c_int64, C.c_int, C.c_void_p, C.c_int64,
                                             C.c_int, C.c_void_p, C.c_void_p, C.c_int64, C.c_int, C.c_void_p, C.c_void_p]),
    'asac_linear_tanh_backward2w': (C.c_int, [C.c_void_p, C.c_int64, C.c_int, C.c_int64, C.c_int, C.c_void_p, C.c_int64,
                                              C.c_int, C.c_void_p, C.c_void_p, C.c_void_p, C.c_int, C.c_int, C.c_int,
                                              C.c_int64, C.c_int, C.c_void_p, C.c_void_p, C.c_void_p, C.c_int, C.c_void_p,
                                              C.c_void_p]),
    'asac_linear_tanh_backward2': (C.c_int, [C.c_void_p, C.c_int64, C.c_int, C.c_void_p, C.c_int64, C.c_int, C.c_void_p,
                                             C.c_void_p, C.c_void_p, C.c_int, C.c_int, C.c_int, C.c_int64, C.c_int,
                                             C.c_void_p, C.c_void_p, C.c_void_p, C.c_int, C.c_void_p, C.c_void_p]),
    'asac_curiosity_bonus': (C.c_int, [C.c_void_p, C.c_void_p, C.c_int64, C.c_int64, C.c_void_p, C.c_int64, C.c_int,
                                       C.c_int, C.c_int, C.c_float, C.c_void_p]),
    'asac_masked_mse': (C.c_int, [C.c_void_p, C.c_void_p, C.c_int64, C.c_int64, C.c_void_p, C.c_int64, C.c_int, C.c_int,
                                  C.c_int, C.c_void_p, C.c_void_p, C.c_void_p, C.c_void_p]),
    'asac_mse_mean_grad_workspace': (C.c_int64, []),
    'asac_mse_mean_grad': (C.c_int, [C.c_void_p, C.c_void_p, C.c_int64, C.c_int64, C.c_int, C.c_int, C.c_int, C.c_float,
                                     C.c_void_p, C.c_void_p, C.c_void_p, C.c_void_p]),
    'asac_masked_mse_workspace': (C.c_int64, [C.c_int64]),
    'asac_normal_nll_kl_workspace': (C.c_int64, [C.c_int64]),
    'asac_normal_nll_kl': (C.c_int, [C.c_void_p, C.c_int64, C.c_int64, C.c_void_p, C.c_int64, C.c_int64, C.c_void_p,
                                     C.c_int64, C.c_int64, C.c_int, C.c_int, C.c_int, C.c_float, C.c_void_p, C.c_void_p,
                                     C.c_void_p, C.c_void_p, C.c_void_p]),
    'asac_normal_nll_kl_logstd': (C.c_int, [C.c_void_p, C.c_int64, C.c_int64, C.c_float, C.c_float, C.c_void_p, C.c_int64,
                                            C.c_int64, C.c_int, C.c_int, C.c_int, C.c_float, C.c_void_p, C.c_void_p,
                                            C.c_void_p, C.c_void_p]),
    'asac_sum_partials_multi': (C.c_int, [C.c_int, C.POINTER(PartialSum), C.c_void_p]),
    'asac_rows_wide_supported': (C.c_int, [C.c_int64, C.c_int, C.c_int]),
    'asac_rows_wide_workspace': (C.c_int64, [C.c_int64, C.c_int, C.c_int]),
    'asac_rows_wide_forward': (C.c_int, [C.c_void_p, C.c_int64, C.c_int64, C.c_int, C.c_void_p, C.c_void_p, C.c_int, C.c_int,
                                         C.c_void_p, C.c_void_p, C.c_void_p, C.c_void_p]),
    'asac_rows_wide_backward_input': (C.c_int, [C.c_void_p, C.c_void_p, C.c_int, C.c_int64, C.c_int, C.c_void_p, C.c_int,
                                                C.c_void_p, C.c_void_p, C.c_int64, C.c_void_p]),
    'asac_rows_wide_backward_params': (C.c_int, [C.c_void_p, C.c_void_p, C.c_int64, C.c_int64, C.c_int, C.c_int, C.c_void_p,
                                                 C.c_void_p, C.c_int, C.c_void_p, C.c_void_p]),
    'asac_xty_supported': (C.c_int, [C.c_int64, C.c_int, C.c_int]),
    'asac_xty_workspace': (C.c_int64, [C.c_int64, C.c_int, C.c_int]),
    'asac_xty': (C.c_int, [C.c_void_p, C.c_int64, C.c_int, C.c_void_p, C.c_int64, C.c_int, C.c_int64, C.c_void_p, C.c_void_p,
                           C.c_int, C.c_void_p, C.c_void_p]),
    'asac_xty_multi_workspace': (C.c_int64, [C.c_int, C.c_void_p, C.c_void_p, C.c_void_p]),
    'asac_xty_multi': (C.c_int, [C.c_int, C.c_void_p, C.c_void_p, C.c_void_p, C.c_void_p, C.c_void_p, C.c_void_p, C.c_void_p,
                                 C.c_void_p, C.c_void_p, C.c_int, C.c_void_p, C.c_void_p]),
    'asac_conv2_tiles': (C.c_int, [C.POINTER(Conv2Desc)]),
    'asac_conv2_z1_floats': (C.c_int64, [C.POINTER(Conv2Desc), C.c_int64]),
    'asac_conv2_supported': (C.c_int, [C.POINTER(Conv2Desc)]),
    'asac_conv2_group_frames': (C.c_int, [C.POINTER(Conv2Desc)]),
    'asac_conv2_backward_windows': (C.c_int, [C.POINTER(Conv2Desc), C.c_void_p, C.c_int64, C.c_int, C.c_int64, C.c_void_p,
                                              C.c_void_p, C.c_void_p, C.c_void_p, C.c_void_p, C.c_int, C.c_void_p,
                                              C.c_void_p]),
    'asac_conv2_backward_multi_max': (C.c_int, [C.POINTER(Conv2Desc)]),
    'asac_conv2_backward_slabs': (C.c_int, [C.POINTER(Conv2Desc), C.c_int64, C.c_int]),
    'asac_conv2_backward_multi': (C.c_int, [C.POINTER(Conv2Desc), C.c_void_p, C.c_int64, C.c_int, C.c_int64, C.c_void_p,
                                            C.c_void_p, C.c_void_p, C.POINTER(C.c_void_p), C.c_int, C.c_void_p, C.c_int,
                                            C.c_void_p, C.c_void_p]),
    'asac_conv2_forward_windows': (C.c_int, [C.POINTER(Conv2Desc), C.c_void_p, C.c_int64, C.c_int, C.c_int64, C.c_void_p,
# ... 577 lines not shown
                                   N, _p(out), _stream()), 'asac_mlp_forward')


class WindowRows:

    def __init__(self, t: torch.Tensor):
        self.t = t
        self.shape = (t.shape[0] * t.shape[1], t.shape[2])


def mlp_job(desc, params, member_stride, E, x0, x1, N, out) -> MlpJob:
    j = MlpJob()
    j.desc, j.params, j.member_stride, j.E, j.N = C.pointer(desc), params.data_ptr(), member_stride, E, N
    if isinstance(x0, WindowRows):
        t = x0.t
        assert t.dim() == 3 and t.stride(2) == 1 and t.shape[0] * t.shape[1] == N
        p0, j.x0_row_stride, j.x0_member_stride = _p(t), t.stride(1), 0
        j.x0_window_T, j.x0_sample_stride = t.shape[1], t.stride(0)
    else:
        p0, j.x0_row_stride, j.x0_member_stride = _rows_view(x0)
    p1, j.x1_row_stride, j.x1_member_stride = _rows_view(x1)
    j.x0, j.x1 = p0.value if p0 is not None else None, p1.value if p1 is not None else None
    assert out.is_cuda and out.is_contiguous()
    j.out = out.data_ptr()
    return j


@_profiled
def mlp_forward_multi(jobs, sidecars=None):
    global _last_work
    _last_work = sum(mlp_flops(j.desc.contents, j.E, j.N) for j in jobs)
    assert 1 <= len(jobs) <= MLP_MAX_JOBS
    arr = (MlpJob * len(jobs))(*jobs)
    sc, n_sc = _sidecar_array(sidecars)
    _check(load().asac_mlp_forward_multi(arr, len(jobs), sc, n_sc, _stream()), 'asac_mlp_forward_multi')


def sample_epilogue(job: MlpJob | None = None, eps=None, a_out=None, logp_out=None, T=0, action=None, action_offset=0,
                    prob_out=None, prob_offset=0, eps2=None, t2=0, a2_out=None, logp2_out=None) -> SampleEpilogue:
    e = SampleEpilogue()
    if job is None:
        return e
    A, N = job.desc.contents.head_cols[0], job.N
    s = e.sample
    s.rows, s.A, s.T = N, A, T
    if eps is not None:
        assert eps.is_contiguous() and a_out.is_contiguous() and eps.numel() == N * A and logp_out.numel() == N
        assert logp_out.is_contiguous()
        s.eps, s.a_tanh_out, s.logp_out = eps.data_ptr(), a_out.data_ptr(), logp_out.data_ptr()
    if action is not None:
        assert action.dim() == 3 and prob_out.dim() == 3 and action.stride(-1) == 1 and prob_out.stride(-1) == 1
        assert action.shape[0] * action.shape[1] == N and prob_out.shape[:2] == action.shape[:2]
        s.T = action.shape[1]
        assert T in (0, s.T)
        s.action, s.action_stride_b, s.action_stride_t, s.action_offset = \
            action.data_ptr(), action.stride(0), action.stride(1), action_offset
        s.prob_out, s.prob_stride_b, s.prob_stride_t, s.prob_offset = \
            prob_out.data_ptr(), prob_out.stride(0), prob_out.stride(1), prob_offset
    if eps2 is not None:
        assert s.T > 0 and eps2.is_contiguous() and a2_out.is_contiguous() and eps2.numel() == (N // s.T) * A
        assert logp2_out.is_contiguous() and logp2_out.numel() == N // s.T
        e.eps2, e.t2, e.a2_out, e.logp2_out = eps2.data_ptr(), t2, a2_out.data_ptr(), logp2_out.data_ptr()
    return e


def mlp_forward_multi_sampled_ok(jobs, epilogues) -> bool:
    assert len(jobs) == len(epilogues) and 1 <= len(jobs) <= MLP_MAX_JOBS
    return bool(load().asac_mlp_forward_multi_sampled_ok((MlpJob * len(jobs))(*jobs), len(jobs),
                                                         (SampleEpilogue * len(jobs))(*epilogues)))


@_profiled
def mlp_forward_multi_sampled(jobs, epilogues, sidecars=None):
    global _last_work
    _last_work = sum(mlp_flops(j.desc.contents, j.E, j.N) for j in jobs)
    assert len(jobs) == len(epilogues) and 1 <= len(jobs) <= MLP_MAX_JOBS
    arr = (MlpJob * len(jobs))(*jobs)
    epi = (SampleEpilogue * len(jobs))(*epilogues)
    sc, n_sc = _sidecar_array(sidecars)
    _check(load().asac_mlp_forward_multi_sampled(arr, len(jobs), epi, sc, n_sc, _stream()), 'asac_mlp_forward_multi_sampled')


def pi_q_job(pi_job: MlpJob, q_job: MlpJob, eps, a_out, logp_out, T, action=None, action_offset=0, prob_out=None,
             prob_offset=0, eps2=None, t2=0, a2_out=None, logp2_out=None) -> PiQJob:
    j = PiQJob()
    j.pi, j.q = pi_job, q_job
    A = pi_job.desc.contents.head_cols[0]
    N = pi_job.N
    assert eps.is_contiguous() and a_out.is_contiguous() and eps.numel() == N * A and logp_out.numel() == N
    s = j.sample
    s.eps, s.a_tanh_out, s.logp_out, s.rows, s.A, s.T = eps.data_ptr(), a_out.data_ptr(), logp_out.data_ptr(), N, A, T
    if action is not None:
        assert action.dim() == 3 and prob_out.dim() == 3 and action.stride(-1) == 1 and prob_out.stride(-1) == 1
        assert action.shape[0] * action.shape[1] == N and action.shape[1] == T and prob_out.shape[:2] == action.shape[:2]
        s.action, s.action_stride_b, s.action_stride_t, s.action_offset = \
            action.data_ptr(), action.stride(0), action.stride(1), action_offset
        s.prob_out, s.prob_stride_b, s.prob_stride_t, s.prob_offset = \
            prob_out.data_ptr(), prob_out.stride(0), prob_out.stride(1), prob_offset
    if eps2 is not None:
        assert eps2.is_contiguous() and a2_out.is_contiguous() and eps2.numel() == (N // T) * A
        j.eps2, j.t2, j.a2_out, j.logp2_out = eps2.data_ptr(), t2, a2_out.data_ptr(), logp2_out.data_ptr()
    return j


def policy_sample_q_forward_ok(job: PiQJob) -> bool:
    return bool(load().asac_policy_sample_q_forward_ok(C.byref(job)))


@_profiled
def policy_sample_q_forward(job: PiQJob, extra_jobs=(), sidecars=None):
    global _last_work
    _last_work = (mlp_flops(job.pi.desc.contents, 1, job.pi.N) + mlp_flops(job.q.desc.contents, job.q.E, job.q.N)
                  + sum(mlp_flops(j.desc.contents, j.E, j.N) for j in extra_jobs))
    extra_jobs = list(extra_jobs)
    assert len(extra_jobs) <= MLP_MAX_JOBS
    arr = (MlpJob * len(extra_jobs))(*extra_jobs) if extra_jobs else None
    sc, n_sc = _sidecar_array(sidecars)
    _check(load().asac_policy_sample_q_forward(C.byref(job), arr, len(extra_jobs), sc, n_sc, _stream()),
           'asac_policy_sample_q_forward')


def mlp_backward_workspace(member_stride, E, N) -> int:
    return int(load().asac_mlp_backward_workspace(member_stride, E, N))


def mlp_backward_tiles(N, E) -> int:
    return int(load().asac_mlp_backward_tiles(N, E))


MLP_REDUCE_OVERWRITE, MLP_REDUCE_ACCUMULATE, MLP_REDUCE_DEFER = 0, 1, 2


def mlp_param_extent(desc) -> int:
    return int(load().asac_mlp_param_extent(C.byref(desc)))


@_profiled
def mlp_backward_qloss(desc, params, member_stride, E, x0, x1, N, target_q, y, weights, clip_eps, loss_out,
                       grad_params, workspace, reduce_mode, grad_x0=None):
    global _last_work
    _last_work = mlp_flops(desc, E, N, backward=True, param_grads=True)
    p0, rs0, ms0 = _rows_view(x0)
    p1, rs1, ms1 = _rows_view(x1)
    assert target_q.is_contiguous() and target_q.numel() == E * N and y.is_contiguous() and y.numel() == N
    assert grad_x0 is None or (grad_x0.is_contiguous() and grad_x0.numel() == E * N * desc.in0)
    _check(load().asac_mlp_backward_qloss_gx(C.byref(desc), _p(params), member_stride, E, p0, rs0, ms0, p1, rs1, ms1, N,
                                             _p(target_q), _p(y), _p(weights), float(clip_eps), _p(loss_out), _p(grad_x0),
                                             _p(grad_params), _p(workspace), int(reduce_mode), _stream()),
           'asac_mlp_backward_qloss')


def mlp_backward_qloss_return_ok(desc, params, member_stride, E, N, ret: VtraceArgs) -> bool:
    return bool(load().asac_mlp_backward_qloss_return_ok(C.byref(desc), _p(params), member_stride, E, N, C.byref(ret)))


@_profiled
def mlp_backward_qloss_return(desc, params, member_stride, E, x0, x1, N, target_q, ret: VtraceArgs, weights, clip_eps,
                              loss_out, grad_params, workspace, reduce_mode, grad_x0=None):
    global _last_work
    _last_work = mlp_flops(desc, E, N, backward=True, param_grads=True)
    p0, rs0, ms0 = _rows_view(x0)
    p1, rs1, ms1 = _rows_view(x1)
    assert target_q.is_contiguous() and target_q.numel() == E * N
    assert grad_x0 is None or (grad_x0.is_contiguous() and grad_x0.numel() == E * N * desc.in0)
    _check(load().asac_mlp_backward_qloss_return(C.byref(desc), _p(params), member_stride, E, p0, rs0, ms0, p1, rs1, ms1,
                                                 N, _p(target_q), C.byref(ret), _p(weights), float(clip_eps),
                                                 _p(loss_out), _p(grad_x0), _p(grad_params), _p(workspace), int(reduce_mode),
                                                 _stream()), 'asac_mlp_backward_qloss_return')


@_profiled
def mlp_backward_policy_q(desc, params, member_stride, E, x0, x1, N, q_table, subset, E_sample, grad_x1):
    global _last_work
    _last_work = mlp_flops(desc, E, N, backward=True, param_grads=False)
    p0, rs0, ms0 = _rows_view(x0)
    p1, rs1, ms1 = _rows_view(x1)
    assert q_table.is_contiguous() and q_table.numel() == E * N and grad_x1.is_contiguous()
    _check(load().asac_mlp_backward_policy_q(C.byref(desc), _p(params), member_stride, E, p0, rs0, ms0, p1, rs1, ms1,
                                             N, _p(q_table), _p(subset), E_sample, _p(grad_x1), _stream()),
           'asac_mlp_backward_policy_q')


@_profiled
def mlp_backward_policy_sample(desc, params, member_stride, x0, N, eps, grad_a, log_alpha, grad_params, workspace,
                               reduce_mode):
    global _last_work
    _last_work = mlp_flops(desc, 1, N, backward=True, param_grads=True)
    p0, rs0, _ = _rows_view(x0)
    A = desc.head_cols[0]
    assert eps.is_contiguous() and eps.numel() == N * A and grad_a.is_contiguous() and grad_a.numel() % (N * A) == 0
    _check(load().asac_mlp_backward_policy_sample(C.byref(desc), _p(params), member_stride, p0, rs0, N, _p(eps),
                                                  _p(grad_a), grad_a.numel() // (N * A), _p(log_alpha),
                                                  _p(grad_params), _p(workspace), int(reduce_mode), _stream()),
           'asac_mlp_backward_policy_sample')


def policy_step_fused_ok(q_desc, q_params, q_member_stride, pi_desc, pi_params, pi_member_stride, N) -> bool:
    return bool(load().asac_policy_step_fused_ok(C.byref(q_desc), _p(q_params), q_member_stride, C.byref(pi_desc),
                                                 _p(pi_params), pi_member_stride, N))


@_profiled
def policy_step_fused(q_desc, q_params, q_member_stride, pi_desc, pi_params, pi_member_stride, x, N, action, eps,
                      log_alpha, q_out, pi_grad_params, workspace, reduce_mode, subset=None, a_out=None, logp_out=None,
                      ls_out=None):
    global _last_work
    _last_work = (mlp_flops(q_desc, 2, N, backward=True, param_grads=False)
                  + mlp_flops(pi_desc, 1, N, backward=True, param_grads=True))
    p0, rs0, _ = _rows_view(x)
    A = pi_desc.head_cols[0]
    assert eps.is_contiguous() and eps.numel() == N * A
    if action is not None:
        assert action.is_contiguous() and action.numel() == N * A
    else:
        assert a_out.is_contiguous() and a_out.numel() == N * A and logp_out.is_contiguous() and logp_out.numel() == N
        assert ls_out is None or (ls_out.is_contiguous() and ls_out.numel() == 2 * N * A)
    assert q_out is None or (q_out.is_contiguous() and q_out.numel() % N == 0 and q_out.numel() >= 2 * N)
    assert subset is None or (subset.dtype == torch.int32 and subset.numel() == 2)
    _check(load().asac_policy_step_fused(C.byref(q_desc), _p(q_params), q_member_stride, C.byref(pi_desc), _p(pi_params),
                                         pi_member_stride, p0, rs0, N, _p(action), _p(eps), _p(log_alpha), _p(subset),
                                         _p(q_out), _p(a_out), _p(logp_out), _p(ls_out), _p(pi_grad_params), _p(workspace),
                                         int(reduce_mode), _stream()),
           'asac_policy_step_fused')


@_profiled
def adam_step_partials(param, grad, exp_avg, exp_avg_sq, lr, beta1, beta2, eps, steps_done, workspace, tiles, E,
                       member_stride, used, accumulate, loss_out=None, loss_rows=0):
    assert param.numel() >= E * member_stride and steps_done.dtype == torch.int64
    _check(load().asac_adam_step_partials(_p(param), _p(grad), _p(exp_avg), _p(exp_avg_sq), lr, beta1, beta2, eps,
                                          _p(steps_done), _p(workspace), tiles, E, member_stride, used,
                                          int(bool(accumulate)), _p(loss_out), loss_rows, _stream()),
           'asac_adam_step_partials')


@_profiled
def mlp_backward(desc, params, member_stride, E, x0, x1, N, grad_out, grad_x0, grad_x1, grad_params, workspace,
                 reduce_mode=MLP_REDUCE_ACCUMULATE):
    global _last_work
    _last_work = mlp_flops(desc, E, N, backward=True, param_grads=grad_params is not None)
    p0, rs0, ms0 = _rows_view(x0)
    p1, rs1, ms1 = _rows_view(x1)
    _check(load().asac_mlp_backward(C.byref(desc), _p(params), member_stride, E, p0, rs0, ms0, p1, rs1, ms1, N,
                                    _p(grad_out), _p(grad_x0), _p(grad_x1), _p(grad_params), _p(workspace),
                                    int(reduce_mode), _stream()), 'asac_mlp_backward')


def attention_supported(Lq: int, Lk: int, D: int) -> bool:
    return bool(load().asac_attention_supported(int(Lq), int(Lk), int(D)))


@_profiled
def attention_forward(q, k, v, mask, out, weights, keep):
    _dense_f32(q, k, v, out, weights, keep)
    B, Lq, D = q.shape
    sb = si = sj = 0
    if mask is not None:
        assert mask.element_size() == 1 and mask.dim() == 3
        sb, si, sj = (0 if mask.shape[d] == 1 else mask.stride(d) for d in range(3))
    _check(load().asac_attention_forward(_p(q), _p(k), _p(v), _p(mask), sb, si, sj, B, Lq, k.shape[1], D, _p(out),
                                         _p(weights), _p(keep), _stream()), 'asac_attention_forward')


@_profiled
def attention_backward(q, k, v, weights, grad_out, grad_weights, grad_q, grad_k, grad_v):
    _dense_f32(q, k, v, weights, grad_out, grad_weights, grad_q, grad_k, grad_v)
    B, Lq, D = q.shape
    _check(load().asac_attention_backward(_p(q), _p(k), _p(v), _p(weights), _p(grad_out), _p(grad_weights), B, Lq,
                                          k.shape[1], D, _p(grad_q), _p(grad_k), _p(grad_v), _stream()),
           'asac_attention_backward')


def _proj_ptrs(params):
    assert len(params) in (6, 8)
    arr = (C.c_void_p * 8)()
    for i, t in enumerate(params):
        assert t.is_cuda and t.is_contiguous() and t.dtype == torch.float32
        arr[i] = t.data_ptr()
    return arr


def _rows3(x):
    assert x.dim() == 3 and x.stride(2) == 1 and x.dtype == torch.float32 and x.is_cuda
    return _p(x), x.stride(0), x.stride(1)


def attention_proj_workspace(B, Lq, Lk, E) -> int:
    return int(load().asac_attention_proj_workspace(B, Lq, Lk, E))


def _row_mask(row_zero):
    if row_zero is None:
        return None, 0, 0
    assert row_zero.dim() == 2 and row_zero.element_size() == 1 and row_zero.is_cuda
    return _p(row_zero), row_zero.stride(0), row_zero.stride(1)


@_profiled
def attention_proj_forward(xq, xk, params, mask, out, weights, keep, attn_out=None, row_zero=None):
    _dense_f32(out, weights, keep, attn_out)
    pq, qsb, qsr = _rows3(xq)
    pk, ksb, ksr = _rows3(xk)
    sb = si = sj = 0
    if mask is not None:
# ... 1035 lines not shown
```

### include/asac_hip.h

```cpp
#ifndef ASAC_HIP_H
#define ASAC_HIP_H

#include <stdint.h>

#ifdef __cplusplus
extern "C" {
#endif

#define ASAC_ABI_VERSION 84
#define ASAC_MAX_GATHER_KEYS 16
#define ASAC_MAX_ENSEMBLE 16
#define ASAC_MAX_ACTION 64
#define ASAC_MLP_MAX_BLOCKS 4

int asac_version(void);
int64_t asac_struct_size(const char* name);
const char* asac_last_error(void);

int asac_set_launch_repeat(int repeat);


int asac_sumtree_sample(const float* tree, int capacity, int batch, const double* u,
                        const int64_t* slot_ids, double* beta_state, double beta_increment,
                        int32_t* leaf_out, float* p_out, int64_t* ids_out, float* is_weights_out,
                        float* min_p_out, void* stream);

int asac_sumtree_descend(const float* tree, int capacity, int n, const double* values, const int64_t* slot_ids,
                         int32_t* leaf_out, float* p_out, int64_t* ids_out, void* stream);

int asac_sumtree_plan_top(const float* shard_roots, int n_shards, int batch, const double* u, int32_t* owner_out,
                          double* value_out, float* total_out, void* stream);
int asac_sumtree_descend_owned(const float* tree, int capacity, int n, const double* values, const int32_t* owner,
                               int rank, const int64_t* slot_ids, int32_t* leaf_out, float* p_out, int64_t* ids_out,
                               void* stream);
int asac_per_is_weights_slice(const float* p_all, int n_all, int first, int count, const float* total, double* beta_state,
                              double beta_increment, float* is_weights_out, void* stream);

int asac_per_is_weights(const float* p, int batch, const float* total, const float* min_ratio,
                        double* beta_state, double beta_increment, float* is_weights_out,
                        void* stream);

int asac_sumtree_update(float* tree, int capacity, int k, const int64_t* ids,
                        const int64_t* slot_ids, const float* td_error, float alpha, float td_min,
                        float td_max, int mode, int32_t* winner, int32_t* nan_flag, void* stream);

int asac_per_add(float* tree, int capacity, int64_t first_id, int count, int ignore_size,
                 const float* max_p_dev, float max_p_host, int64_t* slot_ids, void* stream);

int asac_sumtree_leaf_max(const float* tree, int capacity, float* out, void* stream);

int asac_sumtree_check(const float* tree, int capacity, int32_t* out, void* stream);

int asac_gelu_eval(const float* z, float* value, float* deriv, int64_t n, void* stream);

enum {
    ASAC_PAD_KEEP = 0,
    ASAC_PAD_WORD = 1,
    ASAC_PAD_BYTE = 2,
    ASAC_PAD_ROW = 3,
    ASAC_PAD_EMIT_MASK = 4
};
enum {
    ASAC_CVT_NONE = 0,
    ASAC_CVT_U8_TO_F32_UNIT = 1,
    ASAC_CVT_BOOL_TO_F32 = 2
};
enum { ASAC_DERIVE_NONE = 0, ASAC_DERIVE_PREVIOUS = 1, ASAC_DERIVE_HOLD_LAST = 2, ASAC_DERIVE_HOLD_LAST_NEXT = 3 };
typedef struct {
    const void* src;
    void* dst;
    const void* pad_row;
    int32_t row_bytes;
    int32_t pad_mode;
    uint32_t pad_word;
    int32_t convert;
    int32_t dst_row_pitch;
    int32_t derive;
} asac_gather_key_t;

int asac_window_gather_pad(const asac_gather_key_t* keys_host, int n_keys, const int64_t* ids,
                           int batch, int prev_n, int post_n, int capacity,
                           const int32_t* index_ring, void* stream);

int64_t asac_window_gather_plan_bytes(void);
int asac_window_gather_plan(const asac_gather_key_t* keys_host, int n_keys, const int64_t* ids, int batch, int prev_n,
                            int post_n, int capacity, const int32_t* index_ring, void* plan_dev, int* blocks_out);

int asac_gather_rows(const asac_gather_key_t* keys_host, int n_keys, const int64_t* ids, int n_rows, int capacity,
                     void* stream);

enum { ASAC_ROW_ITEM = 0, ASAC_ROW_SLOT = 1, ASAC_ROW_SLOT_ROW = 2, ASAC_ROW_BROADCAST = 3 };
typedef struct {
// ... 112 lines not shown
    int32_t A;
    const float* gamma_ratio;
    const float* lambda_ratio;
    float gamma, v_rho, v_c;
    int32_t use_n_step_is;
    int32_t B, n;
    const float* q_online;
    int32_t E_online;
    float* td_error_out;
    float* y_out;
} asac_vtrace_args_t;

int asac_vtrace_return_min(const asac_vtrace_args_t* args_host, void* stream);
int asac_vtrace_return_min_sc(const asac_vtrace_args_t* args_host, const asac_sidecar_t* sidecars_host,
                              int n_sidecars, const asac_sidecar_t* pending_alpha, void* stream);
int asac_td_update(const asac_vtrace_args_t* args_host, float* tree, int capacity, const int64_t* ids,
                   const int64_t* slot_ids, float alpha, float td_min, float td_max, int32_t* winner, int32_t* nan_flag,
                   const asac_sidecar_t* sidecars_host, int n_sidecars, const asac_sidecar_t* alpha_step, void* stream);
int asac_sumtree_update_sc(float* tree, int capacity, int k, const int64_t* ids, const int64_t* slot_ids,
                           const float* td_error, float alpha, float td_min, float td_max, int mode, int32_t* winner,
                           int32_t* nan_flag, const asac_sidecar_t* sidecars_host, int n_sidecars, void* stream);

int asac_vtrace_return_direct(const asac_vtrace_args_t* args_host, const float* v_n,
                              const float* v_next, const float* pi_prod, const float* mu_prod,
                              void* stream);

int asac_q_loss_fwd_bwd(const float* q, const float* tq, const float* y, const float* w, int E,
                        int B, float clip_eps, float* loss_out, float* grad_q_out, void* stream);

int asac_policy_loss_fwd_bwd(const float* logp, const float* q, const int32_t* subset, int E, int E_sample,
                             int B, const float* log_alpha, const float* scale, int64_t scale_row_stride, int A,
                             float* loss_out, float* grad_logp, float* grad_q, float* entropy_out, void* stream);

int asac_alpha_grad(const float* logp, int B, float target, float* grad_slot, void* stream);

typedef struct {
    int32_t in0, in1;
    int32_t n_blocks;
    int32_t width[ASAC_MLP_MAX_BLOCKS];
    int32_t residual[ASAC_MLP_MAX_BLOCKS];
    int32_t head_cols[2];
    int64_t w_off[ASAC_MLP_MAX_BLOCKS];
    int64_t b_off[ASAC_MLP_MAX_BLOCKS];
    int64_t head_w_off[2], head_b_off[2];
    int32_t head_transform;
    int32_t reserved_;
} asac_mlp_desc_t;

int asac_mlp_forward(const asac_mlp_desc_t* desc_host, const float* params, int64_t member_stride,
                     int E, const float* x0, int64_t x0_row_stride, int64_t x0_member_stride,
                     const float* x1, int64_t x1_row_stride, int64_t x1_member_stride, int64_t N,
                     float* out, void* stream);

#define ASAC_MLP_MAX_JOBS 2
typedef struct {
    const asac_mlp_desc_t* desc;
    const float* params;
    int64_t member_stride;
    const float* x0;
    int64_t x0_row_stride, x0_member_stride;
    const float* x1;
    int64_t x1_row_stride, x1_member_stride;
    int64_t N;
    float* out;
    int32_t E;
    int32_t x0_window_T;
    int64_t x0_sample_stride;
} asac_mlp_job_t;
int asac_mlp_forward_multi(const asac_mlp_job_t* jobs_host, int n_jobs, const asac_sidecar_t* sidecars_host,
                           int n_sidecars, void* stream);

typedef struct {
    asac_squash_job_t sample;
    const float* eps2;
    int32_t t2;
    int32_t reserved_;
    float* a2_out;
    float* logp2_out;
} asac_mlp_sample_epilogue_t;
int asac_mlp_forward_multi_sampled_ok(const asac_mlp_job_t* jobs_host, int n_jobs, const asac_mlp_sample_epilogue_t* epilogues);
int asac_mlp_forward_multi_sampled(const asac_mlp_job_t* jobs_host, int n_jobs, const asac_mlp_sample_epilogue_t* epilogues,
                                   const asac_sidecar_t* sidecars_host, int n_sidecars, void* stream);

typedef struct {
    asac_mlp_job_t pi;
    asac_squash_job_t sample;
    const float* eps2;
    int32_t t2;
    int32_t reserved_;
    float* a2_out;
    float* logp2_out;
    asac_mlp_job_t q;
} asac_pi_q_job_t;
int asac_policy_sample_q_forward_ok(const asac_pi_q_job_t* job);
int asac_policy_sample_q_forward(const asac_pi_q_job_t* job, const asac_mlp_job_t* extra_jobs, int n_extra,
                                 const asac_sidecar_t* sidecars_host, int n_sidecars, void* stream);

#define ASAC_MLP_REDUCE_OVERWRITE 0
#define ASAC_MLP_REDUCE_ACCUMULATE 1
#define ASAC_MLP_REDUCE_DEFER 2
int64_t asac_mlp_backward_workspace(int64_t member_stride, int E, int64_t N);
int64_t asac_mlp_backward_tiles(int64_t N, int E);

int asac_mlp_backward(const asac_mlp_desc_t* desc_host, const float* params, int64_t member_stride,
                      int E, const float* x0, int64_t x0_row_stride, int64_t x0_member_stride,
                      const float* x1, int64_t x1_row_stride, int64_t x1_member_stride, int64_t N,
                      const float* grad_out, float* grad_x0, float* grad_x1, float* grad_params,
                      float* workspace, int reduce_mode, void* stream);

int asac_mlp_backward_qloss(const asac_mlp_desc_t* desc_host, const float* params, int64_t member_stride,
                            int E, const float* x0, int64_t x0_row_stride, int64_t x0_member_stride,
                            const float* x1, int64_t x1_row_stride, int64_t x1_member_stride, int64_t N,
                            const float* target_q, const float* y, const float* weights, float clip_eps,
                            float* loss_out, float* grad_params, float* workspace, int reduce_mode,
                            void* stream);
int asac_mlp_backward_qloss_gx(const asac_mlp_desc_t* desc_host, const float* params, int64_t member_stride, int E,
                               const float* x0, int64_t x0_row_stride, int64_t x0_member_stride,
                               const float* x1, int64_t x1_row_stride, int64_t x1_member_stride, int64_t N,
                               const float* target_q, const float* y, const float* weights, float clip_eps,
                               float* loss_out, float* grad_x0, float* grad_params, float* workspace, int reduce_mode,
                               void* stream);

int asac_mlp_backward_qloss_return_ok(const asac_mlp_desc_t* desc_host, const float* params, int64_t member_stride, int E,
                                      int64_t N, const asac_vtrace_args_t* ret);
int asac_mlp_backward_qloss_return(const asac_mlp_desc_t* desc_host, const float* params, int64_t member_stride, int E,
                                   const float* x0, int64_t x0_row_stride, int64_t x0_member_stride,
                                   const float* x1, int64_t x1_row_stride, int64_t x1_member_stride, int64_t N,
                                   const float* target_q, const asac_vtrace_args_t* ret, const float* weights,
                                   float clip_eps, float* loss_out, float* grad_x0, float* grad_params, float* workspace,
                                   int reduce_mode, void* stream);

int asac_mlp_backward_policy_q(const asac_mlp_desc_t* desc_host, const float* params, int64_t member_stride,
                               int E, const float* x0, int64_t x0_row_stride, int64_t x0_member_stride,
                               const float* x1, int64_t x1_row_stride, int64_t x1_member_stride, int64_t N,
                               const float* q_table, const int32_t* subset, int E_sample, float* grad_x1,
                               void* stream);

int asac_policy_step_fused_ok(const asac_mlp_desc_t* q_desc, const float* q_params, int64_t q_member_stride,
                              const asac_mlp_desc_t* pi_desc, const float* pi_params, int64_t pi_member_stride, int64_t N);
int asac_policy_step_fused(const asac_mlp_desc_t* q_desc, const float* q_params, int64_t q_member_stride,
                           const asac_mlp_desc_t* pi_desc, const float* pi_params, int64_t pi_member_stride,
                           const float* x, int64_t x_row_stride, int64_t N, const float* action, const float* eps,
                           const float* log_alpha, const int32_t* subset, float* q_out, float* a_tanh_out,
                           float* logp_out, float* ls_out, float* pi_grad_params, float* workspace, int reduce_mode,
                           void* stream);

int asac_mlp_backward_policy_sample(const asac_mlp_desc_t* desc_host, const float* params, int64_t member_stride,
                                    const float* x0, int64_t x0_row_stride, int64_t N, const float* eps,
                                    const float* grad_a, int grad_a_members, const float* log_alpha,
                                    float* grad_params, float* workspace, int reduce_mode, void* stream);

int64_t asac_mlp_param_extent(const asac_mlp_desc_t* desc_host);

int asac_gauss_head_fwd(const float* raw, int64_t rows, int A, float* loc, float* scale, void* stream);
int asac_gauss_head_bwd(const float* raw, const float* grad_loc, const float* grad_scale,
                        int64_t rows, int A, float* grad_raw, void* stream);

#define ASAC_GRU_MAX_LAYERS 2
#define ASAC_GRU_MAX_DIM 16
typedef struct {
    int32_t input, hidden, hidden_pow2, layers;
} asac_gru_desc_t;

int64_t asac_gru_param_count(const asac_gru_desc_t* desc_host);
int64_t asac_gru_backward_workspace(const asac_gru_desc_t* desc_host, int B);

int asac_gru_forward(const asac_gru_desc_t* desc_host, const float* const* w_ih, const float* const* w_hh,
                     const float* const* b_ih, const float* const* b_hh, const float* x,
                     int64_t x_stride_b, int64_t x_stride_t, const float* h0, int64_t h0_stride_b,
                     const uint8_t* padding_mask, int64_t mask_stride_b, int B, int L, float* hn_out,
                     float* out_top, float* gates_out, void* stream);

int asac_gru_forward_twin(const asac_gru_desc_t* desc_host, const float* const* w_ih, const float* const* w_hh,
                          const float* const* b_ih, const float* const* b_hh, const float* const* twin_w_ih,
                          const float* const* twin_w_hh, const float* const* twin_b_ih,
                          const float* const* twin_b_hh, const float* x, int64_t x_stride_b, int64_t x_stride_t,
                          const float* h0, int64_t h0_stride_b, const uint8_t* padding_mask,
                          int64_t mask_stride_b, int B, int L, float* hn_out, float* out_top, float* gates_out,
                          float* twin_hn_out, float* twin_out_top, void* stream);

int asac_gru_backward(const asac_gru_desc_t* desc_host, const float* const* w_ih, const float* const* w_hh,
                      const float* const* b_ih, const float* const* b_hh, const float* x,
                      int64_t x_stride_b, int64_t x_stride_t, const float* h0, int64_t h0_stride_b,
                      const uint8_t* padding_mask, int64_t mask_stride_b, int B, int L, const float* hn,
                      const float* gates, const float* grad_hn, const float* grad_top, float* grad_x,
                      float* grad_h0, float* grad_params, float* const* grad_param_tensors, int accumulate,
                      float* workspace, void* stream);

typedef struct {
    float* param_base;
    const float* grad_base;
    float* exp_avg_base;
    float* exp_avg_sq_base;
    float lr, beta1, beta2, eps;
    const int64_t* steps_done;
} asac_adam_epilogue_t;
int asac_gru_backward_at(const asac_gru_desc_t* desc_host, const float* const* w_ih, const float* const* w_hh,
                         const float* const* b_ih, const float* const* b_hh, const float* x,
                         int64_t x_stride_b, int64_t x_stride_t, const float* h0, int64_t h0_stride_b,
                         const uint8_t* padding_mask, int64_t mask_stride_b, int B, int L, const float* hn,
                         const float* gates, const float* grad_top_members, int members, int position,
                         float* grad_x, float* grad_h0, float* grad_params, float* const* grad_param_tensors,
                         int accumulate, const asac_adam_epilogue_t* adam, float* workspace, void* stream);

int asac_gru_wide_supported(int hidden);
int asac_gru_wide_forward(const float* gi, int64_t gi_stride_b, int64_t gi_stride_t, const float* w_hh, const float* b_hh,
                          const float* h0, int64_t h0_stride_b, const uint8_t* padding_mask, int64_t mask_stride_b, int B,
                          int L, int hidden, float* out, int64_t out_stride_b, int64_t out_stride_t, float* h_raw,
                          float* gates, void* stream);
int asac_gru_wide_forward_twin(const float* gi, int64_t gi_stride_b, int64_t gi_stride_t, const float* w_hh, const float* b_hh,
                               const float* w_hh_twin, const float* b_hh_twin, const float* h0, int64_t h0_stride_b,
                               const uint8_t* padding_mask, int64_t mask_stride_b, int B, int L, int hidden, float* out,
                               int64_t out_stride_b, int64_t out_stride_t, float* h_raw, float* gates, void* stream);
int asac_gru_wide_backward(const float* grad_out, int64_t go_stride_b, int64_t go_stride_t, const float* w_hh_t,
                           const float* gates, const float* h_raw, const float* h0, int64_t h0_stride_b,
                           const uint8_t* padding_mask, int64_t mask_stride_b, int B, int L, int hidden, float* grad_gi,
                           float* grad_gh, float* grad_h0, void* stream);

#define ASAC_CONV2_MAX_K 256
typedef struct {
    int32_t channels, height, width;
    int32_t out1, kernel1, stride1;
    int32_t out2, kernel2, stride2;
} asac_conv2_desc_t;

int asac_conv2_supported(const asac_conv2_desc_t* desc_host);
int asac_conv2_tiles(const asac_conv2_desc_t* desc_host);
int64_t asac_conv2_z1_floats(const asac_conv2_desc_t* desc_host, int64_t N);
// ... 292 lines not shown
```

Before: 11600 train_steps/s.

## Save policy forward activations in pi-q sampling kernel and reuse them in policy step

The fused pi/Q target forward now writes, for the t2 timestep rows, each policy layer's hidden outputs, GELU derivatives and raw head values into a per-sample buffer. The fused policy-step kernel loads these saved values and skips recomputing the three policy layers and the head GEMM. This trades the repeated forward compute for extra global writes (448 floats per sample) in the first kernel and extra reads in the second. It relies on the policy parameters staying unchanged between the two kernels within a step.

```diff
diff --git a/advanced-soft-actor-critic_amd/algorithm/fused_mlp.py b/advanced-soft-actor-critic_amd/algorithm/fused_mlp.py
--- a/advanced-soft-actor-critic_amd/algorithm/fused_mlp.py
+++ b/advanced-soft-actor-critic_amd/algorithm/fused_mlp.py
@@ -446,14 +446,14 @@
                                             self.member_stride, N))
 
     def policy_step_fused(self, critics: 'StockMLP', x0, action, eps, log_alpha, q_out=None, defer=False, subset=None,
-                          sample_out=None):
+                          sample_out=None, pi_saved=None):
         N = x0.shape[-2]
         assert subset is not None or critics.E == 2
         a_out, logp_out, ls_out = sample_out if action is None else (None, None, None)
         native.policy_step_fused(critics.desc, critics.params, critics.member_stride, self.desc, self.params,
                                  self.member_stride, x0, N, action, eps, log_alpha, q_out, self.grad_params,
                                  self._workspace_for(N), self._reduce_mode(defer), subset=subset, a_out=a_out,
-                                 logp_out=logp_out, ls_out=ls_out)
+                                 logp_out=logp_out, ls_out=ls_out, pi_saved=pi_saved)
         self._deferred_rows = N if defer else None
 
     def adam_partials(self, opt, loss_out=None):
diff --git a/advanced-soft-actor-critic_amd/algorithm/oc/option_base.py b/advanced-soft-actor-critic_amd/algorithm/oc/option_base.py
--- a/advanced-soft-actor-critic_amd/algorithm/oc/option_base.py
+++ b/advanced-soft-actor-critic_amd/algorithm/oc/option_base.py
@@ -318,7 +318,7 @@
                 s, e = self._params.span(name)
                 self._params.grad[s:e].zero_()
         self._counter_advanced = False
-        self._pi_sampled = False
+        self._pi_sampled = self._pi_fwd_saved = False
         self._train_policy(obs_list=obs_list, state=state, action=action, mu_d_policy_probs=mu_d_policy_probs)
         if self._auto_alpha():
             self._train_alpha(obs_list, state)
diff --git a/advanced-soft-actor-critic_amd/algorithm/sac_base.py b/advanced-soft-actor-critic_amd/algorithm/sac_base.py
--- a/advanced-soft-actor-critic_amd/algorithm/sac_base.py
+++ b/advanced-soft-actor-critic_amd/algorithm/sac_base.py
@@ -453,6 +453,7 @@
         self._cq_buf, self._tq_buf, self._cq_td_buf = (torch.zeros(E, B, 1, **f32) for _ in range(3))
         self._pi_q, self._pi_stats_src = torch.zeros(E, B, 1, **f32), None
         self._pi_a, self._pi_logp, self._pi_sampled = torch.zeros(B, A1, **f32), torch.zeros(B, **f32), False
+        self._pi_fwd, self._pi_fwd_saved = torch.zeros(B, native.PI_FWD_SAVE_FLOATS, **f32), False
         self._rep_twin = None
         if self._twin_rep and type(self.model_rep) is not ModelSimpleRep:
             from .fused_gru import TwinPass
@@ -884,7 +885,7 @@
         self.noise.normal_(eps_buf)
         if policy_sample:
             self.noise.normal_(self._eps_pi)
-            self._pi_sampled = True
+            self._pi_sampled, self._pi_fwd_saved = True, False
         native.mlp_forward_multi_sampled(jobs, epis)
         return (a_tanh, logp), c_pi
 
@@ -919,7 +920,7 @@
             native.squash_multi([
                 native.squash_job(loc, scale, eps_buf, a_tanh, logp, **stored),
                 native.squash_job(t0_ls[:, 0, :A], t0_ls[:, 0, A:], self._eps_pi, self._pi_a, self._pi_logp)])
-            self._pi_sampled = True
+            self._pi_sampled, self._pi_fwd_saved = True, False
         else:
             native.squash_sample_fwd(loc, scale, eps_buf, a_tanh, logp, **stored)
         return a_tanh, logp, c_pi
@@ -1099,18 +1100,19 @@
             a_y, logp_y = torch.empty((B, T, A), **f32), torch.empty((B, T), **f32)
             c_pi = torch.empty((B, T, A), **f32) if self.use_n_step_is else None
             job_q, q_tab = self._ftq.job(xs, a_y.view(-1, A))
+            save = self._pi_fwd if policy_sample and B == self._pi_fwd.shape[0] else None
             fused = native.pi_q_job(job_pi, job_q, self._eps_y, a_y, logp_y, T,
                                     action=nx_actions if self.use_n_step_is else None,
                                     action_offset=self.d_action_summed_size, prob_out=c_pi,
                                     eps2=self._eps_pi if policy_sample else None, t2=0,
-                                    a2_out=self._pi_a, logp2_out=self._pi_logp)
+                                    a2_out=self._pi_a, logp2_out=self._pi_logp, fwd_save=save)
             if not native.policy_sample_q_forward_ok(fused):
                 fused = None
         if fused is not None:
             self.noise.normal_(self._eps_y)
             if policy_sample:
                 self.noise.normal_(self._eps_pi)
-                self._pi_sampled = True
+                self._pi_sampled, self._pi_fwd_saved = True, save is not None
             native.policy_sample_q_forward(fused, [job_tq], sidecars=self._take_la_gather())
             _, c_y, ret = self._get_y(*window, eps_buf=self._eps_y, subset_prefix='y', y_out=self._y_buf,
                                       ls=ls[0].view(B, T, 2 * A), sample=(a_y, logp_y), stored_pi=c_pi,
@@ -1281,7 +1283,7 @@
         x = StockMLP._rows(state, self.state_size)
         B = x.shape[0]
         fusable = (self._fused_policy_step and self.ensemble_q_sample == 2 and self._fpi.policy_step_fused_ok(self._fq, B))
-        sample_out = None
+        sample_out = pi_saved = None
         if ls is None and not self._pi_sampled and fusable:
             f32 = dict(dtype=torch.float32, device=self.device)
             self.noise.normal_(self._eps_pi)
@@ -1293,11 +1295,14 @@
             loc, scale = ls[..., :A], ls[..., A:]
             if self._pi_sampled:
                 a_tanh, logp, self._pi_sampled = self._pi_a, self._pi_logp, False
+                if self._pi_fwd_saved and B == self._pi_fwd.shape[0]:
+                    pi_saved = self._pi_fwd
             else:
                 self.noise.normal_(self._eps_pi)
                 a_tanh = torch.empty((B, A), dtype=torch.float32, device=self.device)
                 logp = torch.empty(B, dtype=torch.float32, device=self.device)
                 native.squash_sample_fwd(loc, scale, self._eps_pi, a_tanh, logp)
+        self._pi_fwd_saved = False
         sub = self._subsets['pi_c']
         self.noise.subset_(sub, E)
         self._pi_stats_src = (logp, scale)
@@ -1306,7 +1311,7 @@
         if fusable and a_tanh.is_contiguous():
             self._fpi.policy_step_fused(self._fq, x, None if sample_out is not None else a_tanh, self._eps_pi,
                                         self.log_c_alpha, q_out=self._pi_q, defer=fold, subset=sub if E != 2 else None,
-                                        sample_out=sample_out)
+                                        sample_out=sample_out, pi_saved=pi_saved)
         else:
             c_qs = self._fq._launch_forward(x, a_tanh, out=self._pi_q)
             g_a = self._fq.backward_policy_q(x, a_tanh, c_qs.view(E, B), sub if self.ensemble_q_sample != E else None,
diff --git a/advanced-soft-actor-critic_amd/csrc/mlp.hip b/advanced-soft-actor-critic_amd/csrc/mlp.hip
--- a/advanced-soft-actor-critic_amd/csrc/mlp.hip
+++ b/advanced-soft-actor-critic_amd/csrc/mlp.hip
@@ -19,6 +19,12 @@
 #define ASAC_PIQ_WAVES 8
 #endif
 constexpr int kPiQThreads = 64 * ASAC_PIQ_WAVES;
+#ifndef ASAC_PS_SAVED_FWD
+#define ASAC_PS_SAVED_FWD 1
+#endif
+constexpr bool kPsSavedFwd = ASAC_PS_SAVED_FWD != 0;
+constexpr int kSaveRow = ASAC_PI_FWD_SAVE_FLOATS;
+static_assert(kSaveRow == 7 * 64, "layout of the saved policy forward");
 template <int TM> constexpr int threads_of() { return TM * 16; }
 
 inline int mlp_tile_rows(int64_t N, int E) { return ((N + 15) / 16) * (int64_t)(E > 0 ? E : 1) <= 256 ? 16 : 32; }
@@ -1154,6 +1160,7 @@
     float* a_out;
     float* logp_out;
     float* ls_out;
+    const float* pi_saved;
 };
 
 __device__ __forceinline__ void ps_fetch_tile(const StageScalars& q, int64_t row0, float (&v)[kPsSlots]) {
@@ -1268,6 +1275,33 @@
     }
     net_put_fixed<kPsThreads, 3>(r0, L.q[0]);
     net_put_fixed<kPsThreads, 3>(r1, L.q[1]);
+    const bool use_saved = kPsSavedFwd && !sample_here && a.pi_saved != nullptr;
+    float sx[3][kPsSlots] = {};
+    float sh = 0.f;
+    f32x4 zp[3] = {};
+    if (use_saved) {
+        const rsrc_t rs = make_rsrc(a.pi_saved, (unsigned)N * (unsigned)(kSaveRow * 4));
+        const uint32_t base = (uint32_t)row0 * kSaveRow;
+#pragma unroll
+        for (int k = 0; k < 3; ++k) {
+#pragma unroll
+            for (int u = 0; u < kPsSlots; ++u) {
+                const uint32_t i = threadIdx.x + u * kPsThreads;
+                sx[k][u] = __builtin_bit_cast(float, buf_ld(rs, (base + (i >> 6) * kSaveRow + k * kMaxW + (i & 63)) * 4u));
+            }
+        }
+#pragma unroll
+        for (int l = 0; l < 3; ++l) {
+#pragma unroll
+            for (int r = 0; r < 4; ++r) {
+                const uint32_t o = base + (uint32_t)(4 * (lane >> 4) + r) * kSaveRow + (3 + l) * kMaxW + (wave & 3) * 16 + (lane & 15);
+                zp[l][r] = __builtin_bit_cast(float, buf_ld(rs, wave < 4 ? o * 4u : kOob));
+            }
+        }
+        sh = __builtin_bit_cast(float, buf_ld(rs, threadIdx.x < kPsRows * kHeadPad
+                                                      ? (base + (threadIdx.x >> 4) * kSaveRow + 6 * kMaxW + (threadIdx.x & 15)) * 4u
+                                                      : kOob));
+    }
     __syncthreads();
     if (sample_here) {
         if ((int)threadIdx.x < kPsRows * A) {
@@ -1361,42 +1395,49 @@
 
     net_put_fixed<kPsThreads, 3>(rp, P);
     ps_put_tile(in_pi, P.x[0]);
-    if (threadIdx.x < kPsRows * kHeadPad) P.delta[(threadIdx.x >> 4) * kP + (threadIdx.x & 15)] = 0.f;
+    if (use_saved) {
+#pragma unroll
+        for (int k = 0; k < 3; ++k) ps_put_tile(sx[k], P.x[k + 1]);
+    }
+    if (threadIdx.x < kPsRows * kHeadPad) P.delta[(threadIdx.x >> 4) * kP + (threadIdx.x & 15)] = sh;
     __syncthreads();
     MLP_STAMP(6);
-    f32x4 zp[3];
-#pragma unroll
-    for (int l = 0; l < 3; ++l) {
-        if (wave < 4) {
-            const float* xin = P.x[l];
-            float* xout = P.x[l + 1];
-            const f32x4 acc = l > 0 ? gemm_tile(xin, P.w[l], kMaxW, 0, wave) : gemm_tile(xin, P.w[l], round4(K0p), 0, wave);
-            const int pc = wave * 16 + (lane & 15);
-            const float bias = P.bias[l][pc];
-            const bool res = a.pi.d.residual[l] != 0;
-            f32x2_g ya, yb, da, db;
-            gelu_parts2((f32x2_g){acc[0] + bias, acc[1] + bias}, ya, da);
-            gelu_parts2((f32x2_g){acc[2] + bias, acc[3] + bias}, yb, db);
-            const float yv[4] = {ya.x, ya.y, yb.x, yb.y};
-            zp[l] = f32x4{da.x, da.y, db.x, db.y};
-#pragma unroll
-            for (int r = 0; r < 4; ++r) {
-                const int row = 4 * (lane >> 4) + r;
-                float y = yv[r];
-                if (res) y += xin[row * kP + pc];
-                xout[row * kP + pc] = y;
-            }
+    if (!use_saved) {
+#pragma unroll
+        for (int l = 0; l < 3; ++l) {
+            if (wave < 4) {
+                const float* xin = P.x[l];
+                float* xout = P.x[l + 1];
+                const f32x4 acc = l > 0 ? gemm_tile(xin, P.w[l], kMaxW, 0, wave) : gemm_tile(xin, P.w[l], round4(K0p), 0, wave);
+                const int pc = wave * 16 + (lane & 15);
+                const float bias = P.bias[l][pc];
+                const bool res = a.pi.d.residual[l] != 0;
+                f32x2_g ya, yb, da, db;
+                gelu_parts2((f32x2_g){acc[0] + bias, acc[1] + bias}, ya, da);
+                gelu_parts2((f32x2_g){acc[2] + bias, acc[3] + bias}, yb, db);
+                const float yv[4] = {ya.x, ya.y, yb.x, yb.y};
+                zp[l] = f32x4{da.x, da.y, db.x, db.y};
+#pragma unroll
+                for (int r = 0; r < 4; ++r) {
+                    const int row = 4 * (lane >> 4) + r;
+                    float y = yv[r];
+                    if (res) y += xin[row * kP + pc];
+                    xout[row * kP + pc] = y;
+                }
+            }
+            __syncthreads();
+        }
+        MLP_STAMP(7);
+        if (wave == 0) {
+            const f32x4 raw = gemm_tile(P.x[3], P.head, kMaxW, 0, 0);
+            const int hc = lane & 15;
+#pragma unroll
+            for (int r = 0; r < 4; ++r) P.delta[(4 * (lane >> 4) + r) * kP + hc] = raw[r] + P.head_bias[hc];
         }
         __syncthreads();
-    }
-    MLP_STAMP(7);
-    if (wave == 0) {
-        const f32x4 raw = gemm_tile(P.x[3], P.head, kMaxW, 0, 0);
-        const int hc = lane & 15;
-#pragma unroll
-        for (int r = 0; r < 4; ++r) P.delta[(4 * (lane >> 4) + r) * kP + hc] = raw[r] + P.head_bias[hc];
-    }
-    __syncthreads();
+    } else {
+        MLP_STAMP(7);
+    }
     MLP_STAMP(8);
     if ((int)threadIdx.x < kPsRows * A) {
         const int lrow = threadIdx.x / A, d = threadIdx.x - lrow * A;
@@ -1523,6 +1564,7 @@
     StockJobArg pi, q;
     const float *eps, *eps2;
     float *a_out, *logp_out, *a2_out, *logp2_out;
+    float* save;
     StoredProbArg sp;
     int32_t E, tile_groups, blocks, T, t2;
     int32_t x_n, x_blocks;
@@ -1582,6 +1624,7 @@
     const int N = a.pi.N;
     const int n_tiles = (int)((N + 15) / 16);
     const bool writer = e == 0;
+    const bool save_on = kPsSavedFwd && writer && a.save != nullptr;
     MLP_STAMP(0);
 
     const StageScalars sp = stage_scalars_stock(a.pi, 0);
@@ -1605,6 +1648,15 @@
             put_input_tile<THREADS, SLOTS>(in_lo, L.xs[0]);
             __syncthreads();
         }
+        int soff[4] = {-1, -1, -1, -1};
+        if (save_on && comp) {
+#pragma unroll
+            for (int r = 0; r < 4; ++r) {
+                const int gr = row0 + 4 * (lane >> 4) + r;
+                const int smp = (int)((unsigned)gr / (unsigned)a.T);
+                if (gr < N && gr - smp * a.T == a.t2) soff[r] = smp * kSaveRow;
+            }
+        }
         int cur = 0;
 #pragma unroll
         for (int l = 0; l < 3; ++l) {
@@ -1614,15 +1666,20 @@
                 const f32x4 acc = l > 0 ? gemm_tile(xin, L.w[l], kMaxW, 0, wave) : gemm_tile(xin, L.w[l], round4(K0p), 0, wave);
                 const float bias = L.bias[l][col];
                 const bool res = (a.pi.residual_bits >> l) & 1;
-                f32x2_g ya, yb, unused;
-                gelu_parts2((f32x2_g){acc[0] + bias, acc[1] + bias}, ya, unused);
-                gelu_parts2((f32x2_g){acc[2] + bias, acc[3] + bias}, yb, unused);
+                f32x2_g ya, yb, da, db;
+                gelu_parts2((f32x2_g){acc[0] + bias, acc[1] + bias}, ya, da);
+                gelu_parts2((f32x2_g){acc[2] + bias, acc[3] + bias}, yb, db);
                 const float yv[4] = {ya.x, ya.y, yb.x, yb.y};
+                const float dv[4] = {da.x, da.y, db.x, db.y};
 #pragma unroll
                 for (int r = 0; r < 4; ++r) {
                     const int row = 4 * (lane >> 4) + r;
                     float y = yv[r];
                     if (res) y += xin[row * kP + col];
+                    if (save_on && soff[r] >= 0) {
+                        a.save[soff[r] + l * kMaxW + col] = y;
+                        a.save[soff[r] + (3 + l) * kMaxW + col] = dv[r];
+                    }
                     xout[row * kP + col] = y;
                 }
             }
@@ -1635,7 +1692,10 @@
             const int hc = lane & 15;
             const float mine = wave == 0 ? acc[0] : wave == 1 ? acc[1] : wave == 2 ? acc[2] : acc[3];
             const int lrow = 4 * (lane >> 4) + wave;
-            const float v = gauss_head_value(hc < A, mine + L.head_bias[hc]);
+            const float raw = mine + L.head_bias[hc];
+            const int so = wave == 0 ? soff[0] : wave == 1 ? soff[1] : wave == 2 ? soff[2] : soff[3];
+            if (save_on && so >= 0) a.save[so + 6 * kMaxW + hc] = raw;
+            const float v = gauss_head_value(hc < A, raw);
             L.ls[lrow * 2 * kHeadPad + hc] = v;
             if (writer && a.pi.out && row0 + lrow < N && hc < 2 * A) a.pi.out[(row0 + lrow) * (2 * A) + hc] = v;
         }
@@ -2271,11 +2331,13 @@
                            const asac_mlp_desc_t* pi_desc, const float* pi_params, int64_t pi_member_stride,
                            const float* x, int64_t x_row_stride, int64_t N, const float* action, const float* eps,
                            const float* log_alpha, const int32_t* subset, float* q_out, float* a_tanh_out,
-                           float* logp_out, float* ls_out, float* pi_grad_params, float* workspace, int reduce_mode,
-                           void* stream) {
+                           float* logp_out, float* ls_out, const float* pi_saved, float* pi_grad_params, float* workspace,
+                           int reduce_mode, void* stream) {
     if (!asac_policy_step_fused_ok(q_desc, q_params, q_member_stride, pi_desc, pi_params, pi_member_stride, N) ||
         !x || !eps || !log_alpha || !pi_grad_params || !workspace || (!action && (!a_tanh_out || !logp_out)))
         return bad_arg("asac_policy_step_fused");
+    if (pi_saved && (!action || N * (int64_t)(kSaveRow * 4) > 0x7fffffffLL || (reinterpret_cast<uintptr_t>(pi_saved) & 3)))
+        return bad_arg("asac_policy_step_fused: pi_saved goes with `action` (the forward of the launch that sampled it)");
     PolicyStepArgs a{};
     const int A = pi_desc->head_cols[0];
     a.q = make_args(q_desc, q_params, q_member_stride, x, x_row_stride, 0, action, A, 0, N);
@@ -2289,6 +2351,7 @@
     a.pi.log_alpha = log_alpha;
     a.pi.partial = workspace;
     a.q_out = q_out;
+    a.pi_saved = kPsSavedFwd ? pi_saved : nullptr;
     static bool attr_done = false;
     if (int rc = set_lds_limit(reinterpret_cast<const void*>(k_policy_step), sizeof(PsLds), attr_done,
                                "asac_policy_step_fused: hipFuncSetAttribute"))
@@ -2346,6 +2409,7 @@
     if (!s.eps || !s.a_tanh_out || !s.logp_out || s.A != A || s.rows != p.N) return false;
     if (s.action && (!s.prob_out || s.T <= 0)) return false;
     if (j.eps2 && (!j.a2_out || !j.logp2_out || s.T <= 0 || j.t2 < 0 || j.t2 >= s.T)) return false;
+    if (j.fwd_save && (!j.eps2 || p.N % s.T != 0 || !fits32((p.N / s.T + 1) * (int64_t)kSaveRow))) return false;
     if (!fits32(p.member_stride) || !fits32(q.member_stride * q.E)) return false;
     if (s.action && (!fits32((p.N / s.T + 1) * s.action_stride_b) || !fits32((p.N / s.T + 1) * s.prob_stride_b) ||
                      !fits32(s.T * s.action_stride_t) || !fits32(s.T * s.prob_stride_t)))
@@ -2384,6 +2448,7 @@
     m.t2 = job->t2;
     m.a2_out = job->a2_out;
     m.logp2_out = job->logp2_out;
+    m.save = kPsSavedFwd ? job->fwd_save : nullptr;
     m.x_n = n_extra;
     int blocks = 0;
     for (int k = 0; k < n_extra; ++k) {
diff --git a/advanced-soft-actor-critic_amd/native.py b/advanced-soft-actor-critic_amd/native.py
--- a/advanced-soft-actor-critic_amd/native.py
+++ b/advanced-soft-actor-critic_amd/native.py
@@ -7,7 +7,7 @@
 import os as _os
 
 LIB_PATH = Path(_os.environ.get('ASAC_HIP_LIB', PKG_DIR / 'lib' / 'libasac_hip.so'))
-ABI_VERSION = 84
+ABI_VERSION = 85
 
 MAX_GATHER_KEYS = 16
 PAD_KEEP, PAD_WORD, PAD_BYTE, PAD_ROW, PAD_EMIT_MASK = 0, 1, 2, 3, 4
@@ -124,11 +124,12 @@
 
 
 SQUASH_MAX_JOBS = 4
+PI_FWD_SAVE_FLOATS = 7 * 64
 
 
 class PiQJob(C.Structure):
     _fields_ = [('pi', MlpJob), ('sample', SquashJob), ('eps2', C.c_void_p), ('t2', C.c_int32), ('reserved_', C.c_int32),
-                ('a2_out', C.c_void_p), ('logp2_out', C.c_void_p), ('q', MlpJob)]
+                ('a2_out', C.c_void_p), ('logp2_out', C.c_void_p), ('q', MlpJob), ('fwd_save', C.c_void_p)]
 
 
 class SampleEpilogue(C.Structure):
@@ -264,7 +265,7 @@
     'asac_policy_step_fused': (C.c_int, [C.POINTER(MlpDesc), C.c_void_p, C.c_int64, C.POINTER(MlpDesc), C.c_void_p,
                                          C.c_int64, C.c_void_p, C.c_int64, C.c_int64, C.c_void_p, C.c_void_p,
                                          C.c_void_p, C.c_void_p, C.c_void_p, C.c_void_p, C.c_void_p, C.c_void_p,
-                                         C.c_void_p, C.c_void_p, C.c_int, C.c_void_p]),
+                                         C.c_void_p, C.c_void_p, C.c_void_p, C.c_int, C.c_void_p]),
     'asac_mlp_param_extent': (C.c_int64, [C.POINTER(MlpDesc)]),
     'asac_adam_step_partials': (C.c_int, [C.c_void_p, C.c_void_p, C.c_void_p, C.c_void_p, C.c_float, C.c_float,
                                           C.c_float, C.c_float, C.c_void_p, C.c_void_p, C.c_int64, C.c_int,
@@ -1008,7 +1009,7 @@
 
 
 def pi_q_job(pi_job: MlpJob, q_job: MlpJob, eps, a_out, logp_out, T, action=None, action_offset=0, prob_out=None,
-             prob_offset=0, eps2=None, t2=0, a2_out=None, logp2_out=None) -> PiQJob:
+             prob_offset=0, eps2=None, t2=0, a2_out=None, logp2_out=None, fwd_save=None) -> PiQJob:
     j = PiQJob()
     j.pi, j.q = pi_job, q_job
     A = pi_job.desc.contents.head_cols[0]
@@ -1026,6 +1027,10 @@
     if eps2 is not None:
         assert eps2.is_contiguous() and a2_out.is_contiguous() and eps2.numel() == (N // T) * A
         j.eps2, j.t2, j.a2_out, j.logp2_out = eps2.data_ptr(), t2, a2_out.data_ptr(), logp2_out.data_ptr()
+        if fwd_save is not None:
+            assert fwd_save.is_contiguous() and fwd_save.dtype == torch.float32
+            assert fwd_save.numel() == (N // T) * PI_FWD_SAVE_FLOATS
+            j.fwd_save = fwd_save.data_ptr()
     return j
 
 
@@ -1129,7 +1134,7 @@
 @_profiled
 def policy_step_fused(q_desc, q_params, q_member_stride, pi_desc, pi_params, pi_member_stride, x, N, action, eps,
                       log_alpha, q_out, pi_grad_params, workspace, reduce_mode, subset=None, a_out=None, logp_out=None,
-                      ls_out=None):
+                      ls_out=None, pi_saved=None):
     global _last_work
     _last_work = (mlp_flops(q_desc, 2, N, backward=True, param_grads=False)
                   + mlp_flops(pi_desc, 1, N, backward=True, param_grads=True))
@@ -1143,9 +1148,13 @@
         assert ls_out is None or (ls_out.is_contiguous() and ls_out.numel() == 2 * N * A)
     assert q_out is None or (q_out.is_contiguous() and q_out.numel() % N == 0 and q_out.numel() >= 2 * N)
     assert subset is None or (subset.dtype == torch.int32 and subset.numel() == 2)
+    if pi_saved is not None:
+        assert action is not None and pi_saved.is_contiguous() and pi_saved.dtype == torch.float32
+        assert pi_saved.numel() == N * PI_FWD_SAVE_FLOATS
     _check(load().asac_policy_step_fused(C.byref(q_desc), _p(q_params), q_member_stride, C.byref(pi_desc), _p(pi_params),
                                          pi_member_stride, p0, rs0, N, _p(action), _p(eps), _p(log_alpha), _p(subset),
-                                         _p(q_out), _p(a_out), _p(logp_out), _p(ls_out), _p(pi_grad_params), _p(workspace),
+                                         _p(q_out), _p(a_out), _p(logp_out), _p(ls_out), _p(pi_saved), _p(pi_grad_params),
+                                         _p(workspace),
                                          int(reduce_mode), _stream()),
            'asac_policy_step_fused')
 
diff --git a/include/asac_hip.h b/include/asac_hip.h
--- a/include/asac_hip.h
+++ b/include/asac_hip.h
@@ -7,7 +7,7 @@
 extern "C" {
 #endif
 
-#define ASAC_ABI_VERSION 84
+#define ASAC_ABI_VERSION 85
 #define ASAC_MAX_GATHER_KEYS 16
 #define ASAC_MAX_ENSEMBLE 16
 #define ASAC_MAX_ACTION 64
@@ -286,6 +286,7 @@
 int asac_mlp_forward_multi_sampled(const asac_mlp_job_t* jobs_host, int n_jobs, const asac_mlp_sample_epilogue_t* epilogues,
                                    const asac_sidecar_t* sidecars_host, int n_sidecars, void* stream);
 
+#define ASAC_PI_FWD_SAVE_FLOATS 448
 typedef struct {
     asac_mlp_job_t pi;
     asac_squash_job_t sample;
@@ -295,6 +296,7 @@
     float* a2_out;
     float* logp2_out;
     asac_mlp_job_t q;
+    float* fwd_save;
 } asac_pi_q_job_t;
 int asac_policy_sample_q_forward_ok(const asac_pi_q_job_t* job);
 int asac_policy_sample_q_forward(const asac_pi_q_job_t* job, const asac_mlp_job_t* extra_jobs, int n_extra,
@@ -346,8 +348,8 @@
                            const asac_mlp_desc_t* pi_desc, const float* pi_params, int64_t pi_member_stride,
                            const float* x, int64_t x_row_stride, int64_t N, const float* action, const float* eps,
                            const float* log_alpha, const int32_t* subset, float* q_out, float* a_tanh_out,
-                           float* logp_out, float* ls_out, float* pi_grad_params, float* workspace, int reduce_mode,
-                           void* stream);
+                           float* logp_out, float* ls_out, const float* pi_saved, float* pi_grad_params, float* workspace,
+                           int reduce_mode, void* stream);
 
 int asac_mlp_backward_policy_sample(const asac_mlp_desc_t* desc_host, const float* params, int64_t member_stride,
                                     const float* x0, int64_t x0_row_stride, int64_t N, const float* eps,
```

Result: no change. 11680 train_steps/s (median of 5 runs) (+0.7%).
